# EavnJeong/IEF-VAD

Hardware: AMD Instinct MI355X
Metric: snippets/sec at [B,T=256,d=768] (higher is better)
Workload: dtype f32 emulated: exact 3-term bf16 split of both fp32 operands, 6 bf16 MFMA products, fp32 accumulate

## Files before the change

### ief-vad_amd/csrc/iefvad.hip

```cpp
#include "../../include/iefvad.h"

#include <hip/hip_runtime.h>
#include <math.h>
#include <stdarg.h>
#include <stdio.h>
#include <stdlib.h>
#include <string.h>

#include <algorithm>
#include <exception>
#include <new>
#include <thread>
#include <vector>

#include "attention_f32.h"
#include "attention_bf16.h"
#include "attention_pbf16.h"
#include "attention_split.h"
#include "common.h"
#include "gather.h"
#include "gemm_f32.h"
#include "gemm_bf16.h"
#include "gemm_split.h"
#include "rowops.h"
#include "refine_chain_bf16.h"
#include "outproj_ln_chain_bf16.h"
#include "outproj_ln_pchain_bf16.h"
#include "inproj_chain_bf16.h"
#include "heads_chain_bf16.h"
#include "heads_pchain_bf16.h"
#include "ragged.h"
#include "resample.h"
#include "loss.h"
#include "gemm_split_tn.h"
#include "backward.h"
#include "metrics.h"
#include "similarity.h"

static thread_local char g_err[512] = "";

static int fail(const char* fmt, ...) {
    va_list ap;
    va_start(ap, fmt);
    vsnprintf(g_err, sizeof(g_err), fmt, ap);
    va_end(ap);
    return 1;
}

#define HIP_TRY(expr)                                                                            \
    do {                                                                                         \
        hipError_t e_ = (expr);                                                                  \
        if (e_ != hipSuccess) return fail("%s failed: %s (%s:%d)", #expr, hipGetErrorString(e_), \
                                          __FILE__, __LINE__);                                   \
    } while (0)

struct ProjW {
    int N;
    float* w;
    float* b;
    bf16_t* wb;
    bf16_t* ws;
    _Float16* wh;
    const float* wa;
    bf16_t* wst;
};

struct iefvad_handle {
    iefvad_config cfg;
    int D, DH;
    int device;
    bool weights_set;
    bool no_heads_fusion, no_ln_fusion;
    char* iproj_stream[2][IEFVAD_MAX_LAYERS];
    char* heads_stream;
    int chain_min_blocks;
    int rowblock_min_wgs;
    bool no_inproj_chain;
    char* oproj_stream[2][IEFVAD_MAX_LAYERS];
    bool dense_encoder;
    bool persist;
    bool train_attn_unfused;
    bool hostpipe_trace;
    bool no_chain;
    char* chain_stream;
    float* arena;
    size_t arena_floats;
    ProjW in[2][IEFVAD_MAX_LAYERS], out[2][IEFVAD_MAX_LAYERS], head[2], ref1[IEFVAD_MAX_STEPS], ref2[IEFVAD_MAX_STEPS];
    float* norm_w[2][IEFVAD_MAX_LAYERS];
    float* norm_b[2][IEFVAD_MAX_LAYERS];
    float* whiten_w[2];
    float* whiten_b[2];
    float* cls_w;
    float* cls_b;
    float* score_fold;
    bf16_t* arena_b;
    bf16_t* arena_s;
    _Float16* arena_h;
    float* amax_dev;
    struct EventPool* events;
    struct GraphCache* graphs;
    struct MetaRing* meta;
    int num_cus;
    bf16_t* arena_st; float* zero_bias; bool tplanes_valid;
    struct HostPipe* hostpipe;
    struct TrainState* train;
    const float* row_scale[2];
};
static const int kAmaxActBase = 256;
static int amax_act_tensors(int L, int K) { return 2 + 6 * L + 2 * K + 1; }
static size_t amax_words(int L, int K, int mb_chunks) {
    return (size_t)kAmaxActBase * IEF_AMAX_FLOATS + (size_t)amax_act_tensors(L, K) * mb_chunks * IEF_AMAX_PARTS;
}

static const int kDefaultMicroBatchF32 = 256;
static const int kDefaultMicroBatchBF16 = 1024;

static int micro_batch(const iefvad_handle* h) {
    if (h->cfg.micro_batch > 0) return h->cfg.micro_batch < 16384 ? h->cfg.micro_batch : 16384;
    return h->cfg.compute == IEFVAD_COMPUTE_F32 ? kDefaultMicroBatchF32 : kDefaultMicroBatchBF16;
}

template <typename F>
static int for_each_proj(iefvad_handle* h, F f) {
    for (int m = 0; m < 2; ++m) {
        for (int l = 0; l < h->cfg.num_layers; ++l) {
            if (int rc = f(h->in[m][l])) return rc;
            if (int rc = f(h->out[m][l])) return rc;
        }
        if (int rc = f(h->head[m])) return rc;
    }
    for (int k = 0; k < h->cfg.num_steps; ++k) {
        if (int rc = f(h->ref1[k])) return rc;
        if (int rc = f(h->ref2[k])) return rc;
    }
    return 0;
}
static size_t proj_elems(const iefvad_handle* h) {
    const size_t DD = (size_t)h->D * h->D;
    return 2 * (size_t)h->cfg.num_layers * (3 * DD + DD) + 2 * (2 * DD) + (size_t)h->cfg.num_steps * 2 * DD;
}

extern "C" int iefvad_abi_version(void) { return IEFVAD_ABI_VERSION; }

extern "C" const char* iefvad_last_error(void) { return g_err; }

#define IEF_D512 512

static int create_impl(const char* who, bool allow_512, const iefvad_config* cfg, iefvad_handle** out) {
    if (!cfg || !out) return fail("%s: null argument", who);
    *out = nullptr;
    if (cfg->abi_version != IEFVAD_ABI_VERSION)
        return fail("%s: abi_version %d, library is %d", who, cfg->abi_version, IEFVAD_ABI_VERSION);
    const bool d512 = allow_512 && cfg->embed_dim == IEF_D512;
    if (d512) {
        if (cfg->seq_len != IEF_T || cfg->num_heads != IEF_D512 / 64)
            return fail("%s: D=512 is built for T=256, H=8 (head dim 64) (got T=%d H=%d)", who, cfg->seq_len, cfg->num_heads);
        if (cfg->compute != IEFVAD_COMPUTE_F32)
            return fail("%s: D=512 runs in the f32 arithmetic only (compute = %d; bf16, bf16x6 and fp16x3 are built for D=768)", who,
                        cfg->compute);
    } else if (cfg->embed_dim != IEF_D || cfg->seq_len != IEF_T || cfg->num_heads != IEF_H) {
        if (allow_512)
            return fail("%s: kernels are built for D=768, T=256, H=8, or D=512, T=256, H=8 in the f32 arithmetic (got D=%d T=%d H=%d)", who,
                        cfg->embed_dim, cfg->seq_len, cfg->num_heads);
        return fail("iefvad_create: kernels are built for D=768, T=256, H=8 (got D=%d T=%d H=%d)",
                    cfg->embed_dim, cfg->seq_len, cfg->num_heads);
    }
    if (cfg->num_layers < 1 || cfg->num_layers > IEFVAD_MAX_LAYERS)
        return fail("%s: num_layers %d outside 1..%d", who, cfg->num_layers, IEFVAD_MAX_LAYERS);
    if (cfg->num_steps < 0 || cfg->num_steps > IEFVAD_MAX_STEPS)
        return fail("%s: num_steps %d outside 0..%d", who, cfg->num_steps, IEFVAD_MAX_STEPS);
    if (cfg->noise_model != IEFVAD_NOISE_GAUSSIAN && cfg->noise_model != IEFVAD_NOISE_STUDENT_T)
        return fail("Unsupported noise_model. Choose 'Gaussian' or 'StudentT'.");
    if (cfg->compute != IEFVAD_COMPUTE_F32 && cfg->compute != IEFVAD_COMPUTE_BF16 && cfg->compute != IEFVAD_COMPUTE_BF16X6 &&
        cfg->compute != IEFVAD_COMPUTE_FP16X3)
        return fail("%s: unknown compute mode %d", who, cfg->compute);
    if (cfg->noise_model == IEFVAD_NOISE_STUDENT_T && !(cfg->nu != 0.f))
        return fail("%s: nu must be non-zero for StudentT", who);
    int ndev = 0;
    HIP_TRY(hipGetDeviceCount(&ndev));
    if (ndev <= 0) return fail("%s: no HIP device", who);
    iefvad_handle* h = new (std::nothrow) iefvad_handle();
    if (!h) return fail("%s: out of host memory", who);
    memset(h, 0, sizeof(*h));
    h->cfg = *cfg;
    h->D = d512 ? IEF_D512 : IEF_D;
    h->DH = h->D / IEF_H;
    {
        const char* v = getenv("IEFVAD_ROWBLOCK_OFF");
        const int off = v ? atoi(v) : 0;
        h->no_inproj_chain = off & 1; h->no_ln_fusion = off & 2; h->no_heads_fusion = off & 4; h->no_chain = off & 8;
    }
    { const char* v = getenv("IEFVAD_ROWBLOCK_MIN_WGS"); h->rowblock_min_wgs = (v && atoi(v) > 0) ? atoi(v) : 128; }
    { const char* v = getenv("IEFVAD_CHAIN_MIN_BLOCKS"); h->chain_min_blocks = (v && atoi(v) > 0) ? atoi(v) : 4; }
    { const char* v = getenv("IEFVAD_PERSIST"); h->persist = !(v && v[0] == '0'); }
    { const char* v = getenv("IEFVAD_DENSE_ENCODER"); h->dense_encoder = v && v[0] == '1'; }
    { const char* v = getenv("IEFVAD_TRAIN_ATTN"); h->train_attn_unfused = v && v[0] == 'u'; }
    { const char* v = getenv("IEFVAD_HOSTPIPE_TRACE"); h->hostpipe_trace = v && v[0] == '1'; }
    hipError_t e = hipGetDevice(&h->device);
    if (e == hipSuccess)
        e = hipFuncSetAttribute((const void*)iefvad_gemm_bf16_kernel, hipFuncAttributeMaxDynamicSharedMemorySize,
                                GB2_LDS_BYTES);
    if (e == hipSuccess)
        e = hipFuncSetAttribute((const void*)iefvad_gemm_bf16_pipe_kernel, hipFuncAttributeMaxDynamicSharedMemorySize,
                                GB2_LDS_BYTES);
    if (e == hipSuccess)
        e = hipFuncSetAttribute((const void*)iefvad_gemm_bf16_w256_kernel, hipFuncAttributeMaxDynamicSharedMemorySize,
                                GB3_LDS_BYTES);
    if (e == hipSuccess)
        e = hipFuncSetAttribute((const void*)iefvad_refine_chain_bf16_kernel, hipFuncAttributeMaxDynamicSharedMemorySize,
                                RC_LDS_BYTES);
    if (e == hipSuccess)
        e = hipFuncSetAttribute((const void*)iefvad_outproj_ln_chain_bf16_kernel, hipFuncAttributeMaxDynamicSharedMemorySize,
                                OC_LDS_BYTES);
    if (e == hipSuccess)
        e = hipFuncSetAttribute((const void*)iefvad_outproj_ln_pchain_bf16_kernel<true, true>, hipFuncAttributeMaxDynamicSharedMemorySize,
                                OP_LDS_BYTES);
    if (e == hipSuccess)
        e = hipFuncSetAttribute((const void*)iefvad_outproj_ln_pchain_bf16_kernel<true, false>, hipFuncAttributeMaxDynamicSharedMemorySize,
                                OP_LDS_BYTES);
    if (e == hipSuccess)
        e = hipFuncSetAttribute((const void*)iefvad_outproj_ln_pchain_bf16_kernel<false, true>, hipFuncAttributeMaxDynamicSharedMemorySize,
                                OP_LDS_BYTES);
    if (e == hipSuccess)
        e = hipFuncSetAttribute((const void*)iefvad_heads_pchain_bf16_kernel, hipFuncAttributeMaxDynamicSharedMemorySize,
                                HP_LDS_BYTES);
    if (e == hipSuccess)
        e = hipFuncSetAttribute((const void*)iefvad_gemm_split_tn256_kernel, hipFuncAttributeMaxDynamicSharedMemorySize, TN_LDS_BYTES_OF(4));
    if (e == hipSuccess)
        e = hipFuncSetAttribute((const void*)iefvad_attention_pbf16_kernel, hipFuncAttributeMaxDynamicSharedMemorySize, APB_LDS_BYTES);
    if (e == hipSuccess)
        e = hipFuncSetAttribute((const void*)iefvad_attention_pbf16_rows_kernel, hipFuncAttributeMaxDynamicSharedMemorySize, APB_LDS_BYTES);
    if (e == hipSuccess) {
        hipDeviceProp_t prop;
        e = hipGetDeviceProperties(&prop, h->device);
        h->num_cus = e == hipSuccess ? prop.multiProcessorCount : 256;
        g_num_cus = h->num_cus;
    }
    if (e == hipSuccess)
        e = hipFuncSetAttribute((const void*)iefvad_gemm_f32_t256_kernel, hipFuncAttributeMaxDynamicSharedMemorySize,
                                GB2_LDS_BYTES);
    if (e == hipSuccess)
        e = hipFuncSetAttribute((const void*)iefvad_gemm_split_n128_kernel, hipFuncAttributeMaxDynamicSharedMemorySize,
                                GS_LDS_BYTES_OF(2));
    if (e == hipSuccess)
        e = hipFuncSetAttribute((const void*)iefvad_attention_split_kernel, hipFuncAttributeMaxDynamicSharedMemorySize,
                                ATS_LDS_BYTES);
    if (e == hipSuccess)
        e = hipFuncSetAttribute((const void*)iefvad_attention_split_rows_kernel, hipFuncAttributeMaxDynamicSharedMemorySize,
                                ATS_LDS_BYTES);
    if (e == hipSuccess)
        e = hipFuncSetAttribute((const void*)iefvad_attention_split_train_kernel, hipFuncAttributeMaxDynamicSharedMemorySize,
                                ATS_LDS_BYTES);
    if (e == hipSuccess)
        e = hipFuncSetAttribute((const void*)iefvad_attention_split_ds_kernel, hipFuncAttributeMaxDynamicSharedMemorySize,
                                ATS_LDS_BYTES);
    if (e == hipSuccess)
        e = hipFuncSetAttribute((const void*)iefvad_attention_split_train_mask_kernel, hipFuncAttributeMaxDynamicSharedMemorySize,
                                ATS_LDS_BYTES);
    if (e == hipSuccess)
        e = hipFuncSetAttribute((const void*)iefvad_heads_chain_bf16_kernel, hipFuncAttributeMaxDynamicSharedMemorySize,
                                HC_LDS_BYTES);
    if (e == hipSuccess)
        e = hipFuncSetAttribute((const void*)iefvad_inproj_chain_bf16_kernel, hipFuncAttributeMaxDynamicSharedMemorySize,
                                IC_LDS_BYTES);
    if (e == hipSuccess)
        e = hipFuncSetAttribute((const void*)iefvad_inproj_chain_f32in_kernel, hipFuncAttributeMaxDynamicSharedMemorySize,
                                IC_LDS_BYTES);
    if (e == hipSuccess)
        e = hipFuncSetAttribute((const void*)iefvad_attention_split_f16_kernel, hipFuncAttributeMaxDynamicSharedMemorySize,
                                ATS_LDS_BYTES);
    if (e == hipSuccess)
        e = hipFuncSetAttribute((const void*)iefvad_gemm_split_f16_n128_kernel, hipFuncAttributeMaxDynamicSharedMemorySize,
                                GS_LDS_BYTES_OF(2));
    if (e == hipSuccess && cfg->compute == IEFVAD_COMPUTE_FP16X3) e = hipMalloc((void**)&h->amax_dev, amax_words(cfg->num_layers, cfg->num_steps, micro_batch(h)) * sizeof(float));
    if (e != hipSuccess) {
        delete h;
        return fail("%s: %s", who, hipGetErrorString(e));
    }
    *out = h;
    return 0;
}

extern "C" int iefvad_create(const iefvad_config* cfg, iefvad_handle** out) { return create_impl("iefvad_create", false, cfg, out); }

extern "C" int iefvad_create_ex(const iefvad_config* cfg, iefvad_handle** out) { return create_impl("iefvad_create_ex", true, cfg, out); }

static void release_events(iefvad_handle* h);
static void release_graphs(iefvad_handle* h);
static void release_meta(iefvad_handle* h);
static void release_train(iefvad_handle* h);
static void release_hostpipe(iefvad_handle* h);

extern "C" void iefvad_destroy(iefvad_handle* h) {
    if (!h) return;
    if (h->arena) (void)hipFree(h->arena);
    if (h->arena_b) (void)hipFree(h->arena_b);
    if (h->chain_stream) (void)hipFree(h->chain_stream);
    if (h->heads_stream) (void)hipFree(h->heads_stream);
    for (int m = 0; m < 2; ++m)
        for (int l = 0; l < IEFVAD_MAX_LAYERS; ++l) {
            if (h->oproj_stream[m][l]) (void)hipFree(h->oproj_stream[m][l]);
            if (h->iproj_stream[m][l]) (void)hipFree(h->iproj_stream[m][l]);
        }
    if (h->arena_s) (void)hipFree(h->arena_s);
    if (h->arena_st) (void)hipFree(h->arena_st);
    if (h->zero_bias) (void)hipFree(h->zero_bias);
    if (h->arena_h) (void)hipFree(h->arena_h);
    if (h->amax_dev) (void)hipFree(h->amax_dev);
    release_events(h);
    release_graphs(h);
    release_meta(h);
    release_train(h);
    release_hostpipe(h);
    delete h;
}

template <typename T> struct InType { using type = T; };
template <int W> struct RowWidth { static constexpr int value = W; };
template <typename F>
static void dispatch_d(bool d512, F&& f) {
    if (d512) f(RowWidth<IEF_D512>{});
    else f(RowWidth<IEF_D>{});
}
template <typename F>
static int dispatch_in(int in_dtype, bool d512, F&& f) {
    int rc = 0;
    dispatch_d(d512, [&](auto w) {
        rc = in_dtype == IEFVAD_IN_F32 ? f(InType<float>{}, w) : in_dtype == IEFVAD_IN_F16 ? f(InType<__half>{}, w) : f(InType<__hip_bfloat16>{}, w);
    });
    return rc;
}

template <typename T>
static int launch_cast(const void* in0, const void* in1, float* o0, float* o1, bf16_t* b0, bf16_t* b1, size_t n, int nsrc,
                       hipStream_t stream) {
    size_t blocks = (n / 4 + 255) / 256;
    if (blocks > 4096) blocks = 4096;
    hipLaunchKernelGGL(iefvad_cast_kernel<T>, dim3((unsigned)blocks, nsrc), dim3(256), 0, stream, (const T*)in0,
                       (const T*)in1, o0, o1, b0, b1, n);
    HIP_TRY(hipGetLastError());
    return 0;
}

template <typename T, int W>
static int launch_cast_scaled(const void* in0, const void* in1, float* o0, float* o1, bf16_t* b0, bf16_t* b1, size_t n, const float* s0,
                              const float* s1, hipStream_t stream) {
    size_t blocks = (n / 4 + 255) / 256;
    if (blocks > 4096) blocks = 4096;
    hipLaunchKernelGGL((iefvad_cast_scaled_kernel<T, W>), dim3((unsigned)blocks, 2), dim3(256), 0, stream, (const T*)in0, (const T*)in1, o0, o1, b0, b1,
                       n, s0, s1);
    HIP_TRY(hipGetLastError());
    return 0;
}

static int launch_split_planes(const float* src, bf16_t* planes, size_t n, hipStream_t stream) {
    if (n % 4) return fail("split_bf16x3: n = %zu is not a multiple of 4", n);
    size_t blocks = (n / 4 + 255) / 256;
    if (blocks > 4096) blocks = 4096;
    hipLaunchKernelGGL(iefvad_split_planes_kernel, dim3((unsigned)blocks), dim3(256), 0, stream, src, planes, n);
    HIP_TRY(hipGetLastError());
    return 0;
}

struct SplitMany {
    SplitManyArgs a;
    hipStream_t stream;
    explicit SplitMany(hipStream_t s) : stream(s) { a.count = 0; }
    int flush() {
        if (a.count == 0) return 0;
        hipLaunchKernelGGL(iefvad_split_planes_many_kernel, dim3(96, a.count), dim3(256), 0, stream, a);
        a.count = 0;
        HIP_TRY(hipGetLastError());
        return 0;
    }
    int add(const float* src, bf16_t* dst, size_t n, int rows) {
        if (n % 4 || n > 0xffffffffu) return fail("split_bf16x3: n = %zu is not a multiple of 4 below 2^32", n);
        if (rows && (rows % 64 || (n / rows) % 32 || n % rows)) return fail("split_bf16x3: transposed split of a [%d, %zu] matrix", rows, n / rows);
        a.src[a.count] = src; a.dst[a.count] = dst; a.n[a.count] = (unsigned)n; a.rows[a.count] = rows;
        if (++a.count == SPLIT_MANY_MAX) return flush();
        return 0;
    }
};

extern "C" int iefvad_split_bf16x3_many(const float* const* src, void* const* planes, const size_t* n, const int32_t* rows, int32_t count,
                                        void* stream) {
    if (!src || !planes || !n || !rows || count < 0) return fail("iefvad_split_bf16x3_many: null argument");
    SplitMany sm((hipStream_t)stream);
    for (int i = 0; i < count; ++i) {
        if (!src[i] || !planes[i] || rows[i] < 0) return fail("iefvad_split_bf16x3_many: entry %d is null or has negative rows", i);
        if (((uintptr_t)src[i] | (uintptr_t)planes[i]) & 15) return fail("iefvad_split_bf16x3_many: entry %d is not 16-byte aligned", i);
        if (int rc = sm.add(src[i], (bf16_t*)planes[i], n[i], rows[i])) return rc;
    }
    return sm.flush();
}

// ... 165 lines not shown
                q += 2 * n;
                float* word = h->amax_dev + IEF_AMAX_FLOATS * widx++;
                r.wa = word;
                size_t blocks = (n / 4 + 255) / 256;
                if (blocks > 1024) blocks = 1024;
                hipLaunchKernelGGL(iefvad_amax_kernel, dim3((unsigned)blocks, 1), dim3(256), 0, stream, r.w, r.w, word, word, n);
                hipLaunchKernelGGL(iefvad_split_planes_f16_kernel, dim3((unsigned)blocks), dim3(256), 0, stream, r.w, r.wh, n,
                                   (const float*)word);
                HIP_TRY(hipGetLastError());
                return 0;
            })) return rc;
    }
    h->weights_set = true;
    h->tplanes_valid = false;
    return 0;
}

static size_t ws_floats_per_row(const iefvad_handle* h) { return 14 * (size_t)h->D + 4; }

extern "C" size_t iefvad_workspace_bytes(const iefvad_handle* h, int32_t B) {
    if (!h || B <= 0) return 0;
    const int mb = micro_batch(h);
    const size_t rows = (size_t)(B < mb ? B : mb) * IEF_T;
    return rows * ws_floats_per_row(h) * sizeof(float) + 256;
}

enum Stage { ST_QKV = 0, ST_ATT, ST_OUT, ST_LN, ST_HEAD, ST_FUSION, ST_REFINE, ST_SCORER, ST_CAST, ST_COUNT };

struct EventPool {
    std::vector<hipEvent_t> ev;
    size_t used = 0;
    hipError_t err = hipSuccess;
    hipEvent_t take() {
        if (used == ev.size()) {
            hipEvent_t e = nullptr;
            hipError_t r = hipEventCreate(&e);
            if (r != hipSuccess) {
                if (err == hipSuccess) err = r;
                return nullptr;
            }
            ev.push_back(e);
        }
        return ev[used++];
    }
    void release_all() {
        for (hipEvent_t e : ev) (void)hipEventDestroy(e);
        ev.clear();
        used = 0;
    }
};

struct Timer {
    bool on = false;
    hipStream_t stream = nullptr;
    EventPool* pool = nullptr;
    struct Span { int stage; hipEvent_t a, b; };
    std::vector<Span> spans;
    int gemm_launches = 0;
    hipEvent_t begin(int stage) {
        if (!on) return nullptr;
        Span s;
        s.stage = stage;
        s.a = pool->take();
        s.b = pool->take();
        if (!s.a || !s.b) return nullptr;
        (void)hipEventRecord(s.a, stream);
        spans.push_back(s);
        return s.b;
    }
    void end(hipEvent_t b) {
        if (on && b) (void)hipEventRecord(b, stream);
    }
};

static void release_events(iefvad_handle* h) {
    if (h->events) {
        h->events->release_all();
        delete h->events;
        h->events = nullptr;
    }
}

static const int kF32TinyMaxBlocks64 = 320;
static const int kF32T256MinBlocks = 1536;
static const int kF32SmallMaxBlocks128 = 1024;

static int launch_gemm(const GemmArgs& a, int nz, hipStream_t stream, Timer& tm, int stage) {
    if (a.M % GEMM_BM || a.N % GEMM_BN || a.K % GEMM_BK)
        return fail("gemm: shape M=%d N=%d K=%d not a multiple of the %dx%dx%d tile", a.M, a.N, a.K, GEMM_BM, GEMM_BN,
                    GEMM_BK);
    const int blocks128 = (a.M / GEMM_BM) * (a.N / GEMM_BN) * nz;
    const int blocks64 = (a.M / GEMS_BM) * (a.N / GEMS_BN) * nz;
    const bool t256_ok = (a.N % GB2_BN == 0) && (a.K % 16 == 0) && (a.K >= 32);
    const int blocks256 = t256_ok ? (a.M / GB2_BM) * (a.N / GB2_BN) * nz : 0;
    const bool tiny = blocks64 < kF32TinyMaxBlocks64 && a.K % 64 == 0;
    hipEvent_t e = tm.begin(stage);
    if (tiny) {
        dim3 grid((a.M / GEMT_BM) * (a.N / GEMT_BN), 1, nz);
        hipLaunchKernelGGL(iefvad_gemm_f32_tiny_kernel, grid, dim3(256), 0, stream, a);
    } else if (blocks256 >= kF32T256MinBlocks) {
        GemmBArgs b;
        memset(&b, 0, sizeof(b));
        b.M = a.M; b.N = a.N; b.K = a.K; b.lda = a.lda; b.ldc = a.ldc; b.epi = a.epi; b.alpha = a.alpha; b.qcols = a.qcols;
        for (int m = 0; m < nz; ++m) {
            b.p[m].A = (const bf16_t*)a.p[m].A; b.p[m].W = (const bf16_t*)a.p[m].W;
            b.p[m].bias = a.p[m].bias; b.p[m].C = a.p[m].C; b.p[m].R = a.p[m].R; b.p[m].C2 = a.p[m].C2;
        }
        dim3 grid((a.M / GB2_BM) * (a.N / GB2_BN), 1, nz);
        hipLaunchKernelGGL(iefvad_gemm_f32_t256_kernel, grid, dim3(256), GB2_LDS_BYTES, stream, b);
    } else if (blocks128 < kF32SmallMaxBlocks128) {
        dim3 grid((a.M / GEMS_BM) * (a.N / GEMS_BN), 1, nz);
        hipLaunchKernelGGL(iefvad_gemm_f32_small_kernel, grid, dim3(256), 0, stream, a);
    } else {
        dim3 grid((a.M / GEMM_BM) * (a.N / GEMM_BN), 1, nz);
        hipLaunchKernelGGL(iefvad_gemm_f32_kernel, grid, dim3(256), 0, stream, a);
    }
    tm.end(e);
    tm.gemm_launches += 1;
    HIP_TRY(hipGetLastError());
    return 0;
}

static int launch_gemm_b(const GemmBArgs& a, int nz, hipStream_t stream, Timer& tm, int stage) {
    hipEvent_t e;
    if (a.N % GB2_BN == 0 && a.M % GB2_BM == 0 && a.K % GB2_BK == 0 && a.K >= 2 * GB2_BK) {
        e = tm.begin(stage);
        if (a.M % GB3_BM == 0 && a.epi != EPI_REFINE && (a.M / GB3_BM) * (a.N / GB2_BN) * nz >= 256) {
            dim3 grid((a.M / GB3_BM) * (a.N / GB2_BN), 1, nz);
            hipLaunchKernelGGL(iefvad_gemm_bf16_w256_kernel, grid, dim3(512), GB3_LDS_BYTES, stream, a);
        } else {
            dim3 grid((a.M / GB2_BM) * (a.N / GB2_BN), 1, nz);
            hipLaunchKernelGGL(iefvad_gemm_bf16_pipe_kernel, grid, dim3(256), GB2_LDS_BYTES, stream, a);
        }
    } else {
        if (a.M % GEMM_BM || a.N % GEMM_BN || a.K % GEMMB_BK)
            return fail("gemm(bf16): shape M=%d N=%d K=%d not a multiple of the %dx%dx%d tile", a.M, a.N, a.K, GEMM_BM,
                        GEMM_BN, GEMMB_BK);
        dim3 grid((a.M / GEMM_BM) * (a.N / GEMM_BN), 1, nz);
        e = tm.begin(stage);
        hipLaunchKernelGGL(iefvad_gemm_bf16_v1_kernel, grid, dim3(256), 0, stream, a);
    }
    tm.end(e);
    tm.gemm_launches += 1;
    HIP_TRY(hipGetLastError());
    return 0;
}

static const int kSplitBN = GS_BN_OF(2);
static const int kSplitMinWgs = 72;
static bool split_eligible(int M, int N, int K, int nz) {
    return M % GS_BM == 0 && N % kSplitBN == 0 && K % 64 == 0 && K >= 64 && (M / GS_BM) * (N / kSplitBN) * nz >= kSplitMinWgs;
}

static int launch_gemm_split(const GemmBArgs& a, int nz, hipStream_t stream, Timer& tm, int stage, bool f16 = false) {
    if (a.M % GS_BM || a.N % kSplitBN || a.K % 64 || a.K < 64)
        return fail("gemm(bf16x6): shape M=%d N=%d K=%d not a multiple of the %dx%dx64 tile", a.M, a.N, a.K, GS_BM, kSplitBN);
    if (a.epi == EPI_BIAS_RELU_DOT && (f16 || nz != 1 || !a.p[0].R || !a.p[0].C2))
        return fail("gemm(bf16x6): the dot-product epilogue takes one bf16x6 problem with its vector (R) and its partial sums (C2)");
    dim3 grid((a.M / GS_BM) * (a.N / kSplitBN), 1, nz);
    hipEvent_t e = tm.begin(stage);
    if (f16) hipLaunchKernelGGL(iefvad_gemm_split_f16_n128_kernel, grid, dim3(256), GS_LDS_BYTES_OF(2), stream, a);
    else hipLaunchKernelGGL(iefvad_gemm_split_n128_kernel, grid, dim3(256), GS_LDS_BYTES_OF(2), stream, a);
    tm.end(e);
    tm.gemm_launches += 1;
    HIP_TRY(hipGetLastError());
    return 0;
}

static size_t in_elem_bytes(int in_dtype) { return in_dtype == IEFVAD_IN_F32 ? 4 : 2; }

struct Proj {
    const float* A32[2];
    const bf16_t* A16[2];
    const float* W32[2];
    const bf16_t* W16[2];
    const bf16_t* Ws[2];
    const _Float16* Wh[2];
    const float* amaxW[2];
    const float* amaxA[2];
    float* amaxC[2];
    const float* bias[2];
    float* C[2];
    bf16_t* Cb[2];
    const float* R[2];
    float* C2[2];
    int N, ldc, epi, nz;
    float alpha;
    int qcols;
    void set_w(int m, const ProjW& r) {
        W32[m] = r.w; W16[m] = r.wb; Ws[m] = r.ws; Wh[m] = r.wh; amaxW[m] = r.wa; bias[m] = r.b;
    }
};

static int launch_proj(const Proj& p, int compute, bool use_split, int D, int rows, hipStream_t stream, Timer& tm, int stage) {
    const bool bf16 = (compute == IEFVAD_COMPUTE_BF16);
    if (p.epi == EPI_BIAS_RELU_DOT && !(use_split && compute == IEFVAD_COMPUTE_BF16X6))
        return fail("gemm: the dot-product epilogue exists in the bf16x6 split kernel only");
    if (use_split) {
        const bool f16 = (compute == IEFVAD_COMPUTE_FP16X3);
        GemmBArgs g;
        memset(&g, 0, sizeof(g));
        g.M = rows; g.N = p.N; g.K = IEF_D; g.lda = IEF_D; g.ldc = p.ldc; g.epi = p.epi; g.alpha = p.alpha; g.qcols = p.qcols;
        g.wplane = p.N * IEF_D * 2;
        for (int m = 0; m < p.nz; ++m) {
            g.p[m].A = (const bf16_t*)p.A32[m];
            g.p[m].W = f16 ? (const bf16_t*)p.Wh[m] : p.Ws[m];
            g.p[m].bias = p.bias[m]; g.p[m].C = p.C[m]; g.p[m].R = p.R[m]; g.p[m].C2 = p.C2[m];
            if (f16) {
                if (!p.amaxA[m] || !p.amaxW[m]) return fail("gemm(fp16x3): missing running-max word");
                g.p[m].amaxA = p.amaxA[m]; g.p[m].amaxW = p.amaxW[m]; g.p[m].amaxC = p.amaxC[m];
            }
        }
        return launch_gemm_split(g, p.nz, stream, tm, stage, f16);
    }
    if (!bf16) {
        GemmArgs g;
        memset(&g, 0, sizeof(g));
        g.M = rows; g.N = p.N; g.K = D; g.lda = D; g.ldc = p.ldc; g.epi = p.epi; g.alpha = p.alpha; g.qcols = p.qcols;
        for (int m = 0; m < p.nz; ++m) {
            g.p[m].A = p.A32[m]; g.p[m].W = p.W32[m]; g.p[m].bias = p.bias[m]; g.p[m].C = p.C[m]; g.p[m].R = p.R[m];
            g.p[m].C2 = p.C2[m];
        }
        return launch_gemm(g, p.nz, stream, tm, stage);
    }
    GemmBArgs g;
    memset(&g, 0, sizeof(g));
    g.M = rows; g.N = p.N; g.K = IEF_D; g.lda = IEF_D; g.ldc = p.ldc; g.epi = p.epi; g.alpha = p.alpha; g.qcols = p.qcols;
    for (int m = 0; m < p.nz; ++m) {
        g.p[m].A = p.A16[m]; g.p[m].W = p.W16[m]; g.p[m].bias = p.bias[m]; g.p[m].C = p.C[m]; g.p[m].Cb = p.Cb[m];
        g.p[m].R = p.R[m]; g.p[m].C2 = p.C2[m];
    }
    return launch_gemm_b(g, p.nz, stream, tm, stage);
}

static int launch_inproj_chain(iefvad_handle* h, int l, const void* const A[2], bool a_fp32, bf16_t* const C[2], int rows, hipStream_t stream, Timer& tm) {
    InProjChainArgs ia;
    memset(&ia, 0, sizeof(ia));
    for (int m = 0; m < 2; ++m) {
        ia.p[m].A = A[m];
        ia.p[m].stream = h->iproj_stream[m][l]; ia.p[m].bias = h->in[m][l].b; ia.p[m].C = C[m];
    }
    ia.M = rows; ia.alpha = (1.0f / sqrtf((float)IEF_DH)) * 1.4426950408889634f; ia.wave_stride = (unsigned)wstream_wave_stride_bytes(IC_NPASS);
    hipEvent_t e = tm.begin(ST_QKV);
    if (a_fp32) hipLaunchKernelGGL(iefvad_inproj_chain_f32in_kernel, dim3(rows / IC_BM, 2), dim3(512), IC_LDS_BYTES, stream, ia);
    else hipLaunchKernelGGL(iefvad_inproj_chain_bf16_kernel, dim3(rows / IC_BM, 2), dim3(512), IC_LDS_BYTES, stream, ia);
    tm.end(e);
    tm.gemm_launches += 1;
    HIP_TRY(hipGetLastError());
    return 0;
}

static int launch_outproj_ln_chain(iefvad_handle* h, int l, bool whiten, const bf16_t* const A[2], const float* const R[2], float* const y[2],
                                   bf16_t* const yb[2], int rows, hipStream_t stream, Timer& tm) {
    OutLnChainArgs oa;
    memset(&oa, 0, sizeof(oa));
    for (int m = 0; m < 2; ++m) {
        OutLnChainProblem& q = oa.p[m];
        q.A = A[m]; q.stream = h->oproj_stream[m][l]; q.bias = h->out[m][l].b; q.R = R[m];
        q.g1 = h->norm_w[m][l]; q.b1 = h->norm_b[m][l];
        if (whiten) { q.g2 = h->whiten_w[m]; q.b2 = h->whiten_b[m]; }
        q.y = y[m];
        q.yb = yb[m];
    }
    oa.M = rows; oa.eps = 1e-5f; oa.wave_stride = (unsigned)wstream_wave_stride_bytes();
    const int gx = h->num_cus / 2;
    const int nblk = rows / OC_BM;
    hipEvent_t e = tm.begin(ST_OUT);
    if (h->persist && nblk >= 2 * gx && (y[0] != nullptr) == (y[1] != nullptr) && (yb[0] != nullptr) == (yb[1] != nullptr) && (y[0] || yb[0])) {
        if (y[0] && yb[0]) hipLaunchKernelGGL((iefvad_outproj_ln_pchain_bf16_kernel<true, true>), dim3(gx, 2), dim3(512), OP_LDS_BYTES, stream, oa);
        else if (y[0]) hipLaunchKernelGGL((iefvad_outproj_ln_pchain_bf16_kernel<true, false>), dim3(gx, 2), dim3(512), OP_LDS_BYTES, stream, oa);
        else hipLaunchKernelGGL((iefvad_outproj_ln_pchain_bf16_kernel<false, true>), dim3(gx, 2), dim3(512), OP_LDS_BYTES, stream, oa);
    } else
        hipLaunchKernelGGL(iefvad_outproj_ln_chain_bf16_kernel, dim3(rows / OC_BM, 2), dim3(512), OC_LDS_BYTES, stream, oa);
    tm.end(e);
    tm.gemm_launches += 1;
    HIP_TRY(hipGetLastError());
    return 0;
}

static void launch_attention_bf16(iefvad_handle* h, const bf16_t* const qkv[2], bf16_t* const out[2], int nb, const RaggedChunk* chunks,
                                  bool head_major, int rows, hipStream_t stream) {
    AttnBArgs ab;
    for (int m = 0; m < 2; ++m) { ab.qkv[m] = qkv[m]; ab.out[m] = out[m]; }
    ab.nchunks = nb;
    ab.chunks = chunks;
    ab.head_major = head_major ? 1 : 0;
    ab.nrows = rows;
    const int items = 2 * nb * IEF_H;
    if (h->persist && items >= 2 * h->num_cus) {
        if (chunks) hipLaunchKernelGGL(iefvad_attention_pbf16_rows_kernel, dim3(h->num_cus), dim3(512), APB_LDS_BYTES, stream, ab);
        else hipLaunchKernelGGL(iefvad_attention_pbf16_kernel, dim3(h->num_cus), dim3(512), APB_LDS_BYTES, stream, ab);
    } else if (chunks) hipLaunchKernelGGL(iefvad_attention_bf16_rows_kernel, dim3(IEF_H, 2, 2 * nb), dim3(256), 0, stream, ab);
    else hipLaunchKernelGGL(iefvad_attention_bf16_kernel, dim3(IEF_H, 2, 2 * nb), dim3(256), 0, stream, ab);
}

static int launch_heads_chain(iefvad_handle* h, HeadsChainArgs& ha, int rows, float factor, hipStream_t stream, Timer& tm) {
    for (int m = 0; m < 2; ++m) ha.bias[m] = h->head[m].b;
    ha.stream = h->heads_stream;
    ha.M = rows; ha.factor = factor; ha.eps = h->cfg.epsilon; ha.wave_stride = (unsigned)heads_stream_wave_stride_bytes();
    const int gx = h->num_cus / HC_THIRDS;
    hipEvent_t e = tm.begin(ST_HEAD);
    if (h->persist && rows / HC_BM >= 2 * gx)
        hipLaunchKernelGGL(iefvad_heads_pchain_bf16_kernel, dim3(gx, HC_THIRDS), dim3(512), HP_LDS_BYTES, stream, ha);
    else
        hipLaunchKernelGGL(iefvad_heads_chain_bf16_kernel, dim3(rows / HC_BM, HC_THIRDS), dim3(512), HC_LDS_BYTES, stream, ha);
    tm.end(e);
    tm.gemm_launches += 1;
    HIP_TRY(hipGetLastError());
    return 0;
}

static int launch_refine_chain(iefvad_handle* h, const float* z_in, float* z_out, float* logits, int rows, hipStream_t stream, Timer& tm) {
    const int K = h->cfg.num_steps;
    ChainArgs ca;
    memset(&ca, 0, sizeof(ca));
    ca.z_in = z_in; ca.stream = h->chain_stream; ca.cls_w = h->cls_w; ca.cls_b = h->cls_b;
    ca.z_out = z_out;
    ca.logits = logits;
    ca.M = rows; ca.K = K; ca.lambda = h->cfg.lambda_ref; ca.wave_stride = (unsigned)chain_wave_stride_bytes(K);
    hipEvent_t e = tm.begin(ST_REFINE);
    hipLaunchKernelGGL(iefvad_refine_chain_bf16_kernel, dim3(rows / RC_BM), dim3(64 * RC_NW), RC_LDS_BYTES, stream, ca);
    tm.end(e);
    tm.gemm_launches += 1;
    HIP_TRY(hipGetLastError());
    return 0;
}

struct RaggedPass {
    const void* img_rows;
    const void* ev_rows;
    const RaggedChunk* d_chunks;
    const int* d_flags;
    int valid_rows;
    int enc_used_rows;
    int enc_rows;
    float* logits;
    float* w_i_mean;
    float* w_e_mean;
};

struct PassBuffers {
    int nb, rows;
    size_t R;
    bool enc_rows_mode;
    bool ip_chain;
    bool need_xb0;
    bool splitmb, f16mb;
    bool compacted, tail_split;
    float *xin[2], *qkv[2], *att[2], *ybuf[2], *xbuf[2];
    bf16_t *qkvb[2], *attb[2], *xb[2];
    float* lg_scratch;
    float *mu_i, *lv_i, *mu_e, *lv_e, *z, *hbuf, *n_i, *n_e, *logits, *wim_out, *wem_out;
    bf16_t *hb, *zb;
    const float* cur[2];
    const float* xt[2];
    const bf16_t* xtb[2];
    float* am; size_t mbs; int L, K;
    float* am_t(int t) const { return f16mb ? am + mbs * t : nullptr; }
    float* am_in(int m) const { return am_t(m); }
    float* am_att(int l, int m) const { return am_t(2 + 6 * l + m); }
    float* am_x(int l, int m) const { return am_t(2 + 6 * l + 2 + m); }
    float* am_qkv(int l, int m) const { return am_t(2 + 6 * l + 4 + m); }
    float* am_z(int k) const { return am_t(2 + 6 * L + k); }
    float* am_h(int k) const { return am_t(2 + 6 * L + (K + 1) + k); }
};

static PassBuffers pass_buffers(const iefvad_handle* h, int nb, size_t row0, void* workspace, const iefvad_outputs* out, const RaggedPass* rg) {
    const iefvad_config& c = h->cfg;
    const size_t D = h->D, R = (size_t)nb * IEF_T;
    PassBuffers b;
    memset(&b, 0, sizeof(b));
    b.nb = nb; b.R = R;
    b.enc_rows_mode = rg && rg->enc_rows > 0;
    b.rows = b.enc_rows_mode ? rg->enc_rows : nb * IEF_T;
    float* ws = (float*)workspace;
    float* t0 = ws + 2 * R * D;
    for (int m = 0; m < 2; ++m) {
        b.xin[m] = ws + m * R * D;
        b.qkv[m] = t0 + 3 * m * R * D;
        b.qkvb[m] = (bf16_t*)t0 + 3 * m * R * D;
        b.att[m] = ws + (8 + m) * R * D;
        b.attb[m] = (bf16_t*)(ws + 8 * R * D) + m * R * D;
        b.xb[m] = (bf16_t*)(ws + 9 * R * D) + m * R * D;
        b.ybuf[m] = ws + (10 + m) * R * D;
        b.xbuf[m] = ws + (12 + m) * R * D;
        b.xt[m] = b.xbuf[m];
        b.xtb[m] = b.xb[m];
    }
    b.lg_scratch = ws + 14 * R * D;
    b.mu_i = out->image_mu ? out->image_mu + row0 * D : t0;
    b.lv_i = out->image_logvar ? out->image_logvar + row0 * D : t0 + R * D;
    b.mu_e = out->event_mu ? out->event_mu + row0 * D : t0 + 2 * R * D;
    b.lv_e = out->event_logvar ? out->event_logvar + row0 * D : t0 + 3 * R * D;
    b.z = out->fused ? out->fused + row0 * D : t0 + 4 * R * D;
    b.hbuf = t0 + 5 * R * D;
    b.hb = (bf16_t*)b.hbuf; b.zb = b.hb + R * D;
    b.n_i = out->w_i ? out->w_i + row0 * D : nullptr;
    b.n_e = out->w_e ? out->w_e + row0 * D : nullptr;
    b.logits = out->logits ? out->logits + row0 : b.lg_scratch;
    b.wim_out = out->w_i_mean ? out->w_i_mean + row0 : nullptr;
    b.wem_out = out->w_e_mean ? out->w_e_mean + row0 : nullptr;
    if (rg) {
        b.logits = b.lg_scratch;
        b.wim_out = rg->w_i_mean ? b.lg_scratch + R : nullptr;
        b.wem_out = rg->w_e_mean ? b.lg_scratch + 2 * R : nullptr;
    }
    b.ip_chain = c.compute == IEFVAD_COMPUTE_BF16 && !h->no_inproj_chain && b.rows % IC_BM == 0 && (b.rows / IC_BM) * 2 >= h->rowblock_min_wgs;
    b.need_xb0 = c.compute == IEFVAD_COMPUTE_BF16 && !b.ip_chain;
    b.splitmb = (c.compute == IEFVAD_COMPUTE_BF16X6 || c.compute == IEFVAD_COMPUTE_FP16X3) && split_eligible(b.rows, IEF_D, IEF_D, 1);
    b.f16mb = b.splitmb && c.compute == IEFVAD_COMPUTE_FP16X3;
    b.am = h->amax_dev ? h->amax_dev + kAmaxActBase * IEF_AMAX_FLOATS : nullptr;
    b.mbs = (size_t)micro_batch(h) * IEF_AMAX_PARTS;
    b.L = c.num_layers; b.K = c.num_steps;
    return b;
}

static int pass_load_inputs(iefvad_handle* h, PassBuffers& b, const void* pi, const void* pe, int32_t in_dtype, size_t row0, const RaggedPass* rg,
                            hipStream_t stream, Timer& tm) {
    const size_t D = h->D, n = b.R * D;
    const bool d512 = h->D == IEF_D512;
    bf16_t* const b0p = b.need_xb0 ? b.xb[0] : nullptr;
    bf16_t* const b1p = b.need_xb0 ? b.xb[1] : nullptr;
    b.cur[0] = b.xin[0]; b.cur[1] = b.xin[1];
    if (rg) {
        if (b.enc_rows_mode && rg->enc_used_rows < b.rows) {
            const size_t o = (size_t)rg->enc_used_rows * D, nz = (size_t)(b.rows - rg->enc_used_rows) * D;
            for (int m = 0; m < 2; ++m) {
                HIP_TRY(hipMemsetAsync(b.xin[m] + o, 0, nz * sizeof(float), stream));
                if (b.need_xb0) HIP_TRY(hipMemsetAsync(b.xb[m] + o, 0, nz * sizeof(bf16_t), stream));
            }
        }
        hipEvent_t e = tm.begin(ST_CAST);
        dispatch_in(in_dtype, d512, [&](auto t, auto w) {
            using T = typename decltype(t)::type;
            hipLaunchKernelGGL((iefvad_scatter_rows_kernel<T, decltype(w)::value>), dim3(b.nb, 2, IEF_RAGGED_SLICES), dim3(256), 0, stream,
                               (const T*)rg->img_rows, (const T*)rg->ev_rows, rg->d_chunks, rg->d_flags, b.xin[0], b.xin[1], b0p, b1p,
                               b.enc_rows_mode ? 0 : IEF_T);
            return 0;
        });
        tm.end(e);
        HIP_TRY(hipGetLastError());
    } else if (h->row_scale[0] || h->row_scale[1]) {
        hipEvent_t e = tm.begin(ST_CAST);
        const float* s0 = h->row_scale[0] ? h->row_scale[0] + row0 : nullptr;
        const float* s1 = h->row_scale[1] ? h->row_scale[1] + row0 : nullptr;
        const int rc = dispatch_in(in_dtype, d512, [&](auto t, auto w) {
            return launch_cast_scaled<typename decltype(t)::type, decltype(w)::value>(pi, pe, b.xin[0], b.xin[1], b0p, b1p, n, s0, s1, stream);
        });
        tm.end(e);
        if (rc) return rc;
    } else if (in_dtype == IEFVAD_IN_F32) {
        b.cur[0] = (const float*)pi; b.cur[1] = (const float*)pe;
        if (b.need_xb0) {
            hipEvent_t e = tm.begin(ST_CAST);
            const int rc = launch_cast<float>(pi, pe, nullptr, nullptr, b.xb[0], b.xb[1], n, 2, stream);
            tm.end(e);
            if (rc) return rc;
        }
    } else {
        hipEvent_t e = tm.begin(ST_CAST);
        const int rc = dispatch_in(in_dtype, d512, [&](auto t, auto) {
            return launch_cast<typename decltype(t)::type>(pi, pe, b.xin[0], b.xin[1], b0p, b1p, n, 2, stream);
        });
        tm.end(e);
        if (rc) return rc;
    }
    if (b.f16mb) {
        HIP_TRY(hipMemsetAsync(b.am, 0, (size_t)amax_act_tensors(b.L, b.K) * b.mbs * sizeof(float), stream));
        hipEvent_t e = tm.begin(ST_CAST);
        hipLaunchKernelGGL(iefvad_amax_chunk_kernel, dim3(b.nb, 2), dim3(256), 0, stream, b.cur[0], b.cur[1], b.am_in(0), b.am_in(1));
        tm.end(e);
        HIP_TRY(hipGetLastError());
    }
    return 0;
}

static int pass_encoder_layer(iefvad_handle* h, PassBuffers& b, int l, const RaggedPass* rg, hipStream_t stream, Timer& tm) {
    const iefvad_config& c = h->cfg;
    const bool bf = (c.compute == IEFVAD_COMPUTE_BF16);
    const int D = h->D, L = c.num_layers, rows = b.rows, nb = b.nb;
    const bool d512 = h->D == IEF_D512;
    const RaggedChunk* enc_chunks = b.enc_rows_mode ? rg->d_chunks : nullptr;
    Proj p;
    if (b.ip_chain) {
        const void* ipA[2] = {(l == 0) ? (const void*)b.cur[0] : (const void*)b.xb[0], (l == 0) ? (const void*)b.cur[1] : (const void*)b.xb[1]};
        if (int rc = launch_inproj_chain(h, l, ipA, l == 0, b.qkvb, rows, stream, tm)) return rc;
    } else {
        memset(&p, 0, sizeof(p));
        p.N = 3 * D; p.ldc = 3 * D; p.epi = EPI_QKV; p.qcols = D; p.nz = 2;
        p.alpha = 1.0f / sqrtf((float)h->DH) * 1.4426950408889634f;
        for (int m = 0; m < 2; ++m) {
            p.set_w(m, h->in[m][l]);
            p.A32[m] = b.cur[m]; p.A16[m] = b.xb[m]; p.amaxA[m] = l == 0 ? b.am_in(m) : b.am_x(l - 1, m);
            p.amaxC[m] = b.am_qkv(l, m);
            if (bf) p.Cb[m] = b.qkvb[m]; else p.C[m] = b.qkv[m];
        }
        if (int rc = launch_proj(p, c.compute, b.splitmb, D, rows, stream, tm, ST_QKV)) return rc;
    }

    hipEvent_t e = tm.begin(ST_ATT);
    if (bf) {
        launch_attention_bf16(h, b.qkvb, b.attb, nb, enc_chunks, b.ip_chain, rows, stream);
    } else {
        AttnArgs aa;
        memset(&aa, 0, sizeof(aa));
        for (int m = 0; m < 2; ++m) { aa.qkv[m] = b.qkv[m]; aa.out[m] = b.att[m]; }
        aa.nchunks = nb;
        aa.chunks = enc_chunks;
        for (int m = 0; m < 2; ++m) { aa.amax[m] = b.am_att(l, m); aa.amax_in[m] = b.am_qkv(l, m); }
        void (*const kernel)(AttnArgs) = b.f16mb    ? iefvad_attention_split_f16_kernel
                                         : b.splitmb ? (enc_chunks ? iefvad_attention_split_rows_kernel : iefvad_attention_split_kernel)
                                         : d512      ? (enc_chunks ? iefvad_attention_f32_rows_d64_kernel : iefvad_attention_f32_d64_kernel)
                                                     : (enc_chunks ? iefvad_attention_f32_rows_kernel : iefvad_attention_f32_kernel);
        hipLaunchKernelGGL(kernel, dim3(IEF_H, 2, 2 * nb), dim3(256), b.splitmb ? ATS_LDS_BYTES : 0, stream, aa);
    }
    tm.end(e);
    HIP_TRY(hipGetLastError());

    const bool ln_fused = bf && !h->no_ln_fusion && rows % OC_BM == 0 && (rows / OC_BM) * 2 >= h->rowblock_min_wgs;
    if (ln_fused) {
        float* oy[2] = {(l < L - 1) ? b.xbuf[0] : nullptr, (l < L - 1) ? b.xbuf[1] : nullptr};
        if (int rc = launch_outproj_ln_chain(h, l, l == L - 1, b.attb, b.cur, oy, b.xb, rows, stream, tm)) return rc;
    } else {
        memset(&p, 0, sizeof(p));
        p.N = D; p.ldc = D; p.epi = EPI_BIAS_RESID; p.nz = 2;
        for (int m = 0; m < 2; ++m) {
            p.set_w(m, h->out[m][l]);
            p.A32[m] = b.att[m]; p.A16[m] = b.attb[m]; p.amaxA[m] = b.am_att(l, m);
            p.C[m] = b.ybuf[m]; p.R[m] = b.cur[m];
        }
        if (int rc = launch_proj(p, c.compute, b.splitmb, D, rows, stream, tm, ST_OUT)) return rc;

        LnArgs la;
        memset(&la, 0, sizeof(la));
        la.nrows = rows; la.eps = 1e-5f;
        for (int m = 0; m < 2; ++m) {
            la.x[m] = b.ybuf[m]; la.g1[m] = h->norm_w[m][l]; la.b1[m] = h->norm_b[m][l];
            if (l == L - 1) { la.g2[m] = h->whiten_w[m]; la.b2[m] = h->whiten_b[m]; }
            la.y[m] = (!bf || l < L - 1) ? b.xbuf[m] : nullptr;
            la.yb[m] = bf ? b.xb[m] : nullptr;
            la.amax[m] = b.am_x(l, m);
        }
        e = tm.begin(ST_LN);
        dispatch_d(d512, [&](auto w) {
            hipLaunchKernelGGL(iefvad_layernorm_kernel<decltype(w)::value>, dim3((rows + ROW_WAVES - 1) / ROW_WAVES, 2), dim3(256), 0, stream, la);
        });
        tm.end(e);
        HIP_TRY(hipGetLastError());
    }
    b.cur[0] = b.xbuf[0]; b.cur[1] = b.xbuf[1];
    return 0;
}

static int pass_compact_rows(iefvad_handle* h, PassBuffers& b, const RaggedPass* rg, hipStream_t stream, Timer& tm) {
    const bool bf = (h->cfg.compute == IEFVAD_COMPUTE_BF16);
    const size_t D = h->D;
    if (rg && !b.enc_rows_mode && h->cfg.compute != IEFVAD_COMPUTE_FP16X3) {
        const int mc = (rg->valid_rows + 255) / 256 * 256;
        if (mc < b.rows) {
            CompactArgs ca;
            memset(&ca, 0, sizeof(ca));
            for (int m = 0; m < 2; ++m) {
                if (bf) { ca.xb[m] = b.xb[m]; ca.xcb[m] = b.attb[m]; b.xtb[m] = b.attb[m]; }
                else { ca.x[m] = b.xbuf[m]; ca.xc[m] = b.att[m]; b.xt[m] = b.att[m]; }
            }
            ca.chunks = rg->d_chunks;
            const size_t tail0 = (size_t)rg->valid_rows * D, tailn = (size_t)(mc - rg->valid_rows) * D;
            if (tailn)
                for (int m = 0; m < 2; ++m)
                    HIP_TRY(bf ? hipMemsetAsync(b.attb[m] + tail0, 0, tailn * sizeof(bf16_t), stream)
                               : hipMemsetAsync(b.att[m] + tail0, 0, tailn * sizeof(float), stream));
            hipEvent_t e = tm.begin(ST_CAST);
            dispatch_d(h->D == IEF_D512, [&](auto w) {
                hipLaunchKernelGGL(iefvad_compact_rows_kernel<decltype(w)::value>, dim3(b.nb, 2), dim3(256), 0, stream, ca);
            });
            tm.end(e);
            HIP_TRY(hipGetLastError());
            b.rows = mc;
            b.compacted = true;
        }
    }
    b.tail_split = b.splitmb && (!b.compacted || split_eligible(b.rows, IEF_D, IEF_D, 1));
    return 0;
}

static int pass_tail(iefvad_handle* h, PassBuffers& b, const iefvad_outputs* out, const RaggedPass* rg, hipStream_t stream, Timer& tm) {
    const iefvad_config& c = h->cfg;
    const bool bf = (c.compute == IEFVAD_COMPUTE_BF16);
    const int D = h->D, L = c.num_layers, K = c.num_steps, rows = b.rows;
    const bool d512 = h->D == IEF_D512;
    const float factor = (c.noise_model == IEFVAD_NOISE_STUDENT_T) ? (c.nu + 1.0f) / c.nu : 1.0f;
    const dim3 row_grid((rows + ROW_WAVES - 1) / ROW_WAVES);
    float* const z = b.z;

    const bool heads_rows = bf && !h->no_heads_fusion && h->heads_stream && rows % HC_BM == 0 && (rows / HC_BM) * HC_THIRDS >= h->rowblock_min_wgs;
    const bool chain = bf && K > 0 && !h->no_chain && h->chain_stream && rows % RC_BM == 0 && rows / RC_BM >= h->chain_min_blocks;
    if (heads_rows) {
        HeadsChainArgs ha;
        memset(&ha, 0, sizeof(ha));
        for (int m = 0; m < 2; ++m) ha.A[m] = b.xtb[m];
        ha.mu[0] = out->image_mu ? b.mu_i : nullptr; ha.lv[0] = out->image_logvar ? b.lv_i : nullptr;
        ha.mu[1] = out->event_mu ? b.mu_e : nullptr; ha.lv[1] = out->event_logvar ? b.lv_e : nullptr;
        ha.n[0] = b.n_i; ha.n[1] = b.n_e;
        ha.z = z;
        ha.zb = chain ? nullptr : b.zb;
        const bool means = b.wim_out || b.wem_out;
        ha.nsum_part = means ? b.ybuf[0] : nullptr;
        if (int rc = launch_heads_chain(h, ha, rows, factor, stream, tm)) return rc;
        if (means) {
            hipEvent_t e = tm.begin(ST_FUSION);
            hipLaunchKernelGGL(iefvad_rowmean_finish_kernel, dim3((2 * rows + 255) / 256), dim3(256), 0, stream, ha.nsum_part,
                               b.wim_out, b.wem_out, rows, HC_NPART);
            tm.end(e);
            HIP_TRY(hipGetLastError());
        }
    } else {
        Proj p;
        memset(&p, 0, sizeof(p));
        p.N = 2 * D; p.ldc = D; p.epi = EPI_HEADS; p.nz = 2;
        for (int m = 0; m < 2; ++m) {
            p.set_w(m, h->head[m]);
            p.A32[m] = b.xt[m]; p.A16[m] = b.xtb[m]; p.amaxA[m] = b.am_x(L - 1, m);
        }
        p.C[0] = b.mu_i; p.C2[0] = b.lv_i; p.C[1] = b.mu_e; p.C2[1] = b.lv_e;
        if (int rc = launch_proj(p, c.compute, b.tail_split, D, rows, stream, tm, ST_HEAD)) return rc;

        FusionArgs fa;
        memset(&fa, 0, sizeof(fa));
        fa.mu_i = b.mu_i; fa.lv_i = b.lv_i; fa.mu_e = b.mu_e; fa.lv_e = b.lv_e;
        fa.n_i = b.n_i; fa.n_e = b.n_e; fa.n_i_mean = b.wim_out; fa.n_e_mean = b.wem_out;
        fa.z = z;
        fa.zb = (bf && !chain) ? b.zb : nullptr;
        fa.nrows = rows; fa.factor = factor; fa.eps = c.epsilon;
        fa.z_amax = b.am_z(0);
        hipEvent_t e = tm.begin(ST_FUSION);
        dispatch_d(d512, [&](auto w) { hipLaunchKernelGGL(iefvad_fusion_kernel<decltype(w)::value>, row_grid, dim3(256), 0, stream, fa); });
        tm.end(e);
        HIP_TRY(hipGetLastError());
    }

    if (chain)
        if (int rc = launch_refine_chain(h, z, out->fused ? z : nullptr, b.logits, rows, stream, tm)) return rc;

    const bool fold = b.tail_split && c.compute == IEFVAD_COMPUTE_BF16X6 && K >= 1;
    float* const fold_part = b.ybuf[0];

    for (int k = 0; k < K && !chain; ++k) {
        const bool dot = fold && k == K - 1;
        Proj p;
        memset(&p, 0, sizeof(p));
        p.N = D; p.ldc = D; p.epi = EPI_BIAS_RELU; p.nz = 1;
        p.set_w(0, h->ref1[k]);
        p.A32[0] = z; p.A16[0] = b.zb; p.amaxA[0] = b.am_z(k); p.amaxC[0] = b.am_h(k);
        p.C[0] = bf ? nullptr : b.hbuf; p.Cb[0] = bf ? b.hb : nullptr;
        if (dot) {
            p.epi = EPI_BIAS_RELU_DOT; p.R[0] = h->score_fold; p.C2[0] = fold_part;
            if (!out->fused) p.C[0] = nullptr;
        }
        if (int rc = launch_proj(p, c.compute, b.tail_split, D, rows, stream, tm, ST_REFINE)) return rc;
        if (dot) {
            hipEvent_t e = tm.begin(ST_SCORER);
            hipLaunchKernelGGL((iefvad_scorer_fold_kernel<IEF_D, IEF_D / kSplitBN>), row_grid, dim3(256), 0, stream, z, h->cls_w, fold_part,
                               h->score_fold, b.logits, rows);
            tm.end(e);
            HIP_TRY(hipGetLastError());
            if (!out->fused) break;
        }
        memset(&p, 0, sizeof(p));
        p.N = D; p.ldc = D; p.epi = EPI_REFINE; p.alpha = c.lambda_ref; p.nz = 1;
        p.set_w(0, h->ref2[k]);
        p.A32[0] = b.hbuf; p.A16[0] = b.hb; p.amaxA[0] = b.am_h(k); p.amaxC[0] = b.am_z(k + 1);
        p.C[0] = z; p.R[0] = z; p.Cb[0] = (bf && k + 1 < K) ? b.zb : nullptr;
        if (int rc = launch_proj(p, c.compute, b.tail_split, D, rows, stream, tm, ST_REFINE)) return rc;
    }

    if (!chain && !fold) {
        hipEvent_t e = tm.begin(ST_SCORER);
        dispatch_d(d512, [&](auto w) {
            hipLaunchKernelGGL(iefvad_scorer_kernel<decltype(w)::value>, row_grid, dim3(256), 0, stream, z, h->cls_w, h->cls_b, b.logits, rows);
        });
        tm.end(e);
        HIP_TRY(hipGetLastError());
    }

    if (rg) {
        hipEvent_t e = tm.begin(ST_SCORER);
        hipLaunchKernelGGL(iefvad_rows_out_kernel, dim3(b.compacted ? (rg->valid_rows + 255) / 256 : b.nb), dim3(256), 0, stream, b.logits, b.wim_out,
                           b.wem_out, rg->logits, rg->w_i_mean, rg->w_e_mean, b.compacted ? nullptr : rg->d_chunks, rg->valid_rows);
        tm.end(e);
        HIP_TRY(hipGetLastError());
    }
    return 0;
}

static int forward_pass(iefvad_handle* h, const void* pi, const void* pe, int32_t in_dtype, int nb, size_t row0, void* workspace,
                        const iefvad_outputs* out, const RaggedPass* rg, hipStream_t stream, Timer& tm) {
    PassBuffers b = pass_buffers(h, nb, row0, workspace, out, rg);
    if (int rc = pass_load_inputs(h, b, pi, pe, in_dtype, row0, rg, stream, tm)) return rc;
    for (int l = 0; l < h->cfg.num_layers; ++l)
        if (int rc = pass_encoder_layer(h, b, l, rg, stream, tm)) return rc;
    if (int rc = pass_compact_rows(h, b, rg, stream, tm)) return rc;
    return pass_tail(h, b, out, rg, stream, tm);
}

static int forward_impl(iefvad_handle* h, const void* img, const void* ev, int32_t in_dtype, int32_t B, void* workspace,
                        size_t workspace_bytes, const iefvad_outputs* out, hipStream_t stream, Timer& tm) {
    if (!h || !img || !ev || !out) return fail("iefvad_forward: null argument");
    if (!h->weights_set) return fail("iefvad_forward: weights not set");
    if (B <= 0) return fail("iefvad_forward: B must be positive (got %d)", B);
    if (in_dtype != IEFVAD_IN_F32 && in_dtype != IEFVAD_IN_F16 && in_dtype != IEFVAD_IN_BF16)
        return fail("iefvad_forward: unknown in_dtype %d", in_dtype);
    if (!workspace || workspace_bytes < iefvad_workspace_bytes(h, B))
        return fail("iefvad_forward: workspace too small (%zu < %zu bytes)", workspace_bytes, iefvad_workspace_bytes(h, B));
    if (((uintptr_t)workspace & 15) || ((uintptr_t)img & 15) || ((uintptr_t)ev & 15))
        return fail("iefvad_forward: buffers must be 16-byte aligned");
    const int mb = micro_batch(h);
    for (int b0 = 0; b0 < B; b0 += mb) {
        const int nb = (B - b0 < mb) ? (B - b0) : mb;
        const size_t row0 = (size_t)b0 * IEF_T;
        const size_t in_off = row0 * (size_t)h->D * in_elem_bytes(in_dtype);
        if (int rc = forward_pass(h, (const char*)img + in_off, (const char*)ev + in_off, in_dtype, nb, row0, workspace, out, nullptr,
                                  stream, tm))
            return rc;
    }
    return 0;
}

static int video_chunks(int n) { return n < IEF_T ? 1 : n / IEF_T + (n % IEF_T ? 1 : 0); }

struct MetaRing {
    static const int kSlots = 4;
    void* host[kSlots] = {nullptr, nullptr, nullptr, nullptr};
    void* dev[kSlots] = {nullptr, nullptr, nullptr, nullptr};
    size_t cap[kSlots] = {0, 0, 0, 0};
    hipEvent_t done[kSlots] = {nullptr, nullptr, nullptr, nullptr};
    int turn = 0;
};

static void release_meta(iefvad_handle* h) {
    if (!h->meta) return;
    for (int i = 0; i < MetaRing::kSlots; ++i) {
        if (h->meta->host[i]) (void)hipHostFree(h->meta->host[i]);
        if (h->meta->dev[i]) (void)hipFree(h->meta->dev[i]);
        if (h->meta->done[i]) (void)hipEventDestroy(h->meta->done[i]);
    }
    delete h->meta;
    h->meta = nullptr;
}

static int videos_layout(const int32_t* lengths, int32_t nvideos, long long* total_rows, long long* total_chunks) {
    long long rows = 0, chunks = 0;
    for (int v = 0; v < nvideos; ++v) {
        if (lengths[v] <= 0) return fail("iefvad_forward_videos: lengths[%d] = %d", v, lengths[v]);
        rows += lengths[v];
        chunks += video_chunks(lengths[v]);
    }
    *total_rows = rows;
    *total_chunks = chunks;
    return 0;
}

extern "C" size_t iefvad_videos_workspace_bytes(const iefvad_handle* h, const int32_t* lengths, int32_t nvideos) {
    if (!h || !lengths || nvideos <= 0) return 0;
    long long rows, chunks;
    if (videos_layout(lengths, nvideos, &rows, &chunks) || chunks > 0x7fffffffLL) return 0;
    return iefvad_workspace_bytes(h, (int32_t)chunks);
}

static int forward_videos_impl(iefvad_handle* h, const void* img_rows, const void* ev_rows, int32_t in_dtype, const int32_t* lengths,
                               int32_t nvideos, int32_t nan_to_num, void* workspace, size_t workspace_bytes, float* logits,
                               float* w_i_mean, float* w_e_mean, hipStream_t stream, Timer& tm) {
    if (!h || !img_rows || !ev_rows || !lengths || !logits) return fail("iefvad_forward_videos: null argument");
    if (!h->weights_set) return fail("iefvad_forward_videos: weights not set");
    if (nvideos <= 0) return fail("iefvad_forward_videos: nvideos must be positive (got %d)", nvideos);
    if (in_dtype != IEFVAD_IN_F32 && in_dtype != IEFVAD_IN_F16 && in_dtype != IEFVAD_IN_BF16)
        return fail("iefvad_forward_videos: unknown in_dtype %d", in_dtype);
    long long total_rows, total_chunks;
    if (int rc = videos_layout(lengths, nvideos, &total_rows, &total_chunks)) return rc;
    if (total_chunks > 0x7fffffffLL / IEF_T) return fail("iefvad_forward_videos: too many chunks");
    const size_t need = iefvad_workspace_bytes(h, (int32_t)total_chunks);
    if (!workspace || workspace_bytes < need) return fail("iefvad_forward_videos: workspace too small (%zu < %zu bytes)", workspace_bytes, need);
    if (((uintptr_t)workspace & 15) || ((uintptr_t)img_rows & 15) || ((uintptr_t)ev_rows & 15))
        return fail("iefvad_forward_videos: buffers must be 16-byte aligned");

    const size_t chunk_bytes = (size_t)total_chunks * sizeof(RaggedChunk);
    const size_t flag_off = (chunk_bytes + 255) & ~(size_t)255;
    const size_t flag_bytes = nan_to_num ? (size_t)nvideos * 2 * sizeof(int) : 0;
    const size_t meta_bytes = flag_off + flag_bytes;
    if (!h->meta) {
        h->meta = new (std::nothrow) MetaRing();
        if (!h->meta) return fail("iefvad_forward_videos: out of host memory");
    }
    MetaRing& mr = *h->meta;
    const int slot = mr.turn;
    mr.turn = (mr.turn + 1) % MetaRing::kSlots;
    HIP_TRY(hipSetDevice(h->device));
    if (mr.done[slot]) HIP_TRY(hipEventSynchronize(mr.done[slot]));
    else HIP_TRY(hipEventCreateWithFlags(&mr.done[slot], hipEventDisableTiming));
    if (mr.cap[slot] < meta_bytes) {
        if (mr.host[slot]) (void)hipHostFree(mr.host[slot]);
        if (mr.dev[slot]) (void)hipFree(mr.dev[slot]);
        mr.host[slot] = mr.dev[slot] = nullptr;
        mr.cap[slot] = 0;
        const size_t cap = meta_bytes * 2 + 4096;
        HIP_TRY(hipHostMalloc(&mr.host[slot], cap, hipHostMallocDefault));
        HIP_TRY(hipMalloc(&mr.dev[slot], cap));
        mr.cap[slot] = cap;
    }
    RaggedChunk* hc = (RaggedChunk*)mr.host[slot];
    const int mb = micro_batch(h);
    const bool enc_rows_mode = !h->dense_encoder && h->cfg.compute != IEFVAD_COMPUTE_FP16X3;
    {
        long long row = 0, pass_row0 = 0;
        long long ci = 0;
        int enc = 0;
        for (int v = 0; v < nvideos; ++v) {
            const int n = lengths[v], nch = video_chunks(n);
            for (int j = 0; j < nch; ++j, ++ci) {
                if (ci % mb == 0) { pass_row0 = row; enc = 0; }
                const int valid = (n - j * IEF_T) < IEF_T ? (n - j * IEF_T) : IEF_T;
                hc[ci].src_row = (int)(row - pass_row0);
                hc[ci].valid = valid;
                hc[ci].video = v;
                hc[ci].enc_row = enc;
                enc += enc_rows_mode ? ragged_rows(valid) : IEF_T;
                row += valid;
// ... 640 lines not shown
        table[v].out = v;
        row += lengths[v];
    }
    std::stable_sort(table.begin(), table.end(), [](const ResampleVideo& a, const ResampleVideo& b) { return a.n > b.n; });
    hipStream_t stream = (hipStream_t)stream_;
    HIP_TRY(hipMemcpyAsync(workspace, table.data(), (size_t)nvideos * sizeof(ResampleVideo), hipMemcpyHostToDevice, stream));
    HIP_TRY(hipStreamSynchronize(stream));
    const dim3 grid((unsigned)((long long)nvideos * groups));
    if (in_dtype == IEFVAD_IN_F32)
        hipLaunchKernelGGL(iefvad_resample_rows_kernel<float>, grid, dim3(256), 0, stream, (const float*)rows, (const ResampleVideo*)workspace, (int)D, out,
                           (int*)out_lengths);
    else
        hipLaunchKernelGGL(iefvad_resample_rows_kernel<__half>, grid, dim3(256), 0, stream, (const __half*)rows, (const ResampleVideo*)workspace, (int)D, out,
                           (int*)out_lengths);
    HIP_TRY(hipGetLastError());
    return 0;
}

extern "C" int iefvad_gather_windows(const float* img_set, const float* ev_set, const int32_t* set_lengths, int32_t nset, const int32_t* index,
                                     int32_t B, int32_t T, int32_t D, float* img_out, float* ev_out, int32_t* len_out, void* stream_) {
    if (!img_set || !ev_set || !set_lengths || !index || !img_out || !ev_out || !len_out) return fail("iefvad_gather_windows: null argument");
    if (nset <= 0 || B <= 0) return fail("iefvad_gather_windows: nset = %d, B = %d must be positive", nset, B);
    if (B > 65535) return fail("iefvad_gather_windows: B = %d exceeds one launch (65535 windows)", B);
    if (T != IEF_T) return fail("iefvad_gather_windows: T = %d, the window is %d segments", T, IEF_T);
    if (D <= 0 || D % 8) return fail("iefvad_gather_windows: D = %d must be a positive multiple of 8", D);
    if (((uintptr_t)img_set & 15) || ((uintptr_t)ev_set & 15) || ((uintptr_t)img_out & 15) || ((uintptr_t)ev_out & 15) ||
        ((uintptr_t)set_lengths & 3) || ((uintptr_t)index & 3) || ((uintptr_t)len_out & 3))
        return fail("iefvad_gather_windows: the window tensors must be 16-byte aligned, the int32 vectors 4-byte");
    const int nvec = IEF_T * D / 4, per_wg = 256 * IEF_GW_VEC;
    hipLaunchKernelGGL(iefvad_gather_windows_kernel, dim3((nvec + per_wg - 1) / per_wg, B, 2), dim3(256), 0, (hipStream_t)stream_, img_set, ev_set,
                       (const int*)set_lengths, (int)nset, (const int*)index, (int)D, img_out, ev_out, (int*)len_out);
    HIP_TRY(hipGetLastError());
    return 0;
}

extern "C" int iefvad_similarity_rows(const float* fused, const float* image_mu, const float* event_mu, int64_t rows, int32_t D,
                                      const int32_t* src_rows, int64_t nout, float* out, void* stream_) {
    if (!fused || !image_mu || !event_mu) return fail("iefvad_similarity_rows: null tensor (fused, image_mu, event_mu)");
    if (!out) return fail("iefvad_similarity_rows: null out");
    if (rows <= 0) return fail("iefvad_similarity_rows: rows = %lld must be positive", (long long)rows);
    if (nout < 0) return fail("iefvad_similarity_rows: nout = %lld is negative", (long long)nout);
    if (D != 768 && D != 512) return fail("iefvad_similarity_rows: D = %d (768 and 512 are built)", D);
    if (!src_rows && nout > rows) return fail("iefvad_similarity_rows: nout = %lld exceeds rows = %lld without src_rows", (long long)nout, (long long)rows);
    if (nout > 0x7fffffffLL) return fail("iefvad_similarity_rows: nout = %lld exceeds one launch (2^31 - 1 rows)", (long long)nout);
    if (((uintptr_t)fused & 15) || ((uintptr_t)image_mu & 15) || ((uintptr_t)event_mu & 15) || ((uintptr_t)out & 15) || ((uintptr_t)src_rows & 3))
        return fail("iefvad_similarity_rows: misaligned pointer (the tensors and out 16-byte, src_rows 4-byte)");
    if (nout == 0) return 0;
    const dim3 grid((unsigned)((nout + ROW_WAVES - 1) / ROW_WAVES));
    if (D == 768)
        hipLaunchKernelGGL(iefvad_similarity_rows_kernel<768>, grid, dim3(256), 0, (hipStream_t)stream_, fused, image_mu, event_mu, (long long)rows,
                           (const int*)src_rows, (long long)nout, out);
    else
        hipLaunchKernelGGL(iefvad_similarity_rows_kernel<512>, grid, dim3(256), 0, (hipStream_t)stream_, fused, image_mu, event_mu, (long long)rows,
                           (const int*)src_rows, (long long)nout, out);
    HIP_TRY(hipGetLastError());
    return 0;
}

#include "vadclip.h"
#include "hostgather.h"
#include "hostpipe.h"

extern "C" int iefvad_rowblock_unit(iefvad_handle* h, int32_t stage, int32_t layer, int32_t rows, const iefvad_unit_io* io, void* stream_) {
    if (!h || !io) return fail("iefvad_rowblock_unit: null argument");
    if (!h->weights_set) return fail("iefvad_rowblock_unit: weights not set");
    if (h->D != IEF_D) return fail("iefvad_rowblock_unit: the row-block kernels are built for D=768 (this handle has D=%d)", h->D);
    if (h->cfg.compute != IEFVAD_COMPUTE_BF16) return fail("iefvad_rowblock_unit: the row-block kernels belong to compute = BF16 (got %d)", h->cfg.compute);
    if (rows <= 0 || rows % 64) return fail("iefvad_rowblock_unit: rows = %d must be a positive multiple of 64", rows);
    if (stage == IEFVAD_UNIT_ATTENTION && rows % IEF_T) return fail("iefvad_rowblock_unit: ATTENTION runs whole chunks, rows = %d must be a multiple of %d", rows, IEF_T);
    hipStream_t stream = (hipStream_t)stream_;
    const int L = h->cfg.num_layers, K = h->cfg.num_steps;
    Timer tm;
    auto aligned = [](const void* p) { return (((uintptr_t)p) & 15) == 0; };
    switch (stage) {
    case IEFVAD_UNIT_INPROJ: {
        if (layer < 0 || layer >= L) return fail("iefvad_rowblock_unit: layer %d of %d", layer, L);
        if (!h->iproj_stream[0][layer]) return fail("iefvad_rowblock_unit: in_proj streams are not packed on this handle");
        const void* A[2] = {io->x[0], io->x[1]};
        bf16_t* C[2] = {(bf16_t*)io->y[0], (bf16_t*)io->y[1]};
        for (int m = 0; m < 2; ++m)
            if (!A[m] || !C[m] || !aligned(A[m]) || !aligned(C[m])) return fail("iefvad_rowblock_unit: INPROJ needs x[m] and y[m], 16-byte aligned");
        return launch_inproj_chain(h, layer, A, layer == 0, C, rows, stream, tm);
    }
    case IEFVAD_UNIT_OUTPROJ_LN: {
        if (layer < 0 || layer >= L) return fail("iefvad_rowblock_unit: layer %d of %d", layer, L);
        if (!h->oproj_stream[0][layer]) return fail("iefvad_rowblock_unit: out_proj streams are not packed on this handle");
        const bf16_t* A[2] = {(const bf16_t*)io->x[0], (const bf16_t*)io->x[1]};
        const float* R[2] = {io->resid[0], io->resid[1]};
        float* y[2] = {(float*)io->y[0], (float*)io->y[1]};
        bf16_t* yb[2] = {(bf16_t*)io->yb[0], (bf16_t*)io->yb[1]};
        for (int m = 0; m < 2; ++m)
            if (!A[m] || !R[m] || (!y[m] && !yb[m]) || !aligned(A[m]) || !aligned(R[m]) || !aligned(y[m]) || !aligned(yb[m]))
                return fail("iefvad_rowblock_unit: OUTPROJ_LN needs x[m], resid[m] and y[m] or yb[m], 16-byte aligned");
        return launch_outproj_ln_chain(h, layer, layer == L - 1, A, R, y, yb, rows, stream, tm);
    }
    case IEFVAD_UNIT_HEADS: {
        if (!h->heads_stream) return fail("iefvad_rowblock_unit: the heads stream is not packed on this handle");
        if (!io->x[0] || !io->x[1] || !io->z || !aligned(io->x[0]) || !aligned(io->x[1]) || !aligned(io->z))
            return fail("iefvad_rowblock_unit: HEADS needs x[0], x[1] and z, 16-byte aligned");
        HeadsChainArgs ha;
        memset(&ha, 0, sizeof(ha));
        for (int m = 0; m < 2; ++m) {
            ha.A[m] = (const bf16_t*)io->x[m];
            ha.mu[m] = io->mu[m]; ha.lv[m] = io->logvar[m]; ha.n[m] = io->w[m];
        }
        ha.z = io->z;
        const float factor = (h->cfg.noise_model == IEFVAD_NOISE_STUDENT_T) ? (h->cfg.nu + 1.0f) / h->cfg.nu : 1.0f;
        return launch_heads_chain(h, ha, rows, factor, stream, tm);
    }
    case IEFVAD_UNIT_REFINE: {
        if (K < 1 || !h->chain_stream) return fail("iefvad_rowblock_unit: the refinement chain needs K >= 1 (K = %d)", K);
        if (!io->x[0] || !io->logits || !aligned(io->x[0]) || !aligned(io->z)) return fail("iefvad_rowblock_unit: REFINE needs x[0] (z_0) and logits");
        return launch_refine_chain(h, (const float*)io->x[0], io->z, io->logits, rows, stream, tm);
    }
    case IEFVAD_UNIT_ATTENTION: {
        const bf16_t* qkv[2] = {(const bf16_t*)io->x[0], (const bf16_t*)io->x[1]};
        bf16_t* out[2] = {(bf16_t*)io->yb[0], (bf16_t*)io->yb[1]};
        for (int m = 0; m < 2; ++m)
            if (!qkv[m] || !out[m] || !aligned(qkv[m]) || !aligned(out[m])) return fail("iefvad_rowblock_unit: ATTENTION needs x[m] and yb[m], 16-byte aligned");
        launch_attention_bf16(h, qkv, out, rows / IEF_T, nullptr, true, rows, stream);
        HIP_TRY(hipGetLastError());
        return 0;
    }
    default:
        return fail("iefvad_rowblock_unit: unknown stage %d", stage);
    }
}

extern "C" int iefvad_gemm_bias(const void* A, const void* W, const float* bias, float* C, int32_t M, int32_t N, int32_t K,
                                int32_t compute, void* stream) {
    if (!A || !W || !bias || !C) return fail("iefvad_gemm_bias: null argument");
    Timer tm;
    if (compute == IEFVAD_COMPUTE_F32) {
        GemmArgs g;
        memset(&g, 0, sizeof(g));
        g.M = M; g.N = N; g.K = K; g.lda = K; g.ldc = N; g.epi = EPI_BIAS;
        g.p[0].A = (const float*)A; g.p[0].W = (const float*)W; g.p[0].bias = bias; g.p[0].C = C;
        return launch_gemm(g, 1, (hipStream_t)stream, tm, ST_QKV);
    }
    if (compute == IEFVAD_COMPUTE_BF16) {
        GemmBArgs g;
        memset(&g, 0, sizeof(g));
        g.M = M; g.N = N; g.K = K; g.lda = K; g.ldc = N; g.epi = EPI_BIAS;
        g.p[0].A = (const bf16_t*)A; g.p[0].W = (const bf16_t*)W; g.p[0].bias = bias; g.p[0].C = C;
        return launch_gemm_b(g, 1, (hipStream_t)stream, tm, ST_QKV);
    }
    if (compute == IEFVAD_COMPUTE_BF16X6) {
        GemmBArgs g;
        memset(&g, 0, sizeof(g));
        g.M = M; g.N = N; g.K = K; g.lda = K; g.ldc = N; g.epi = EPI_BIAS; g.wplane = N * K * 2;
        g.p[0].A = (const bf16_t*)A; g.p[0].W = (const bf16_t*)W; g.p[0].bias = bias; g.p[0].C = C;
        hipError_t e = hipFuncSetAttribute((const void*)iefvad_gemm_split_n128_kernel, hipFuncAttributeMaxDynamicSharedMemorySize,
                                           GS_LDS_BYTES_OF(2));
        if (e != hipSuccess) return fail("iefvad_gemm_bias: %s", hipGetErrorString(e));
        return launch_gemm_split(g, 1, (hipStream_t)stream, tm, ST_QKV);
    }
    return fail("iefvad_gemm_bias: unknown compute mode %d", compute);
}
```

### ief-vad_amd/csrc/train.h

```cpp
#pragma once

struct TrainLayout {
    size_t U;
    size_t PU;
    size_t x[2][IEFVAD_MAX_LAYERS + 1], qkv[2][IEFVAD_MAX_LAYERS], att[2][IEFVAD_MAX_LAYERS], s[2][IEFVAD_MAX_LAYERS];
    size_t P[2][IEFVAD_MAX_LAYERS];
    size_t E[2], mu[2], lv[2];
    size_t z[IEFVAD_MAX_STEPS + 1], hid[IEFVAD_MAX_STEPS];
    size_t logits;
    size_t g, da, dh[2], gx, datt, dqkv, dP, part, cpart, rpart;
    size_t part_floats, cpart_floats, rpart_floats;
    size_t total;
};

static const int kColsumRows = 128;

static int splitk_splits(int rows, int n_out) {
    const int tiles = (n_out / 128) * (IEF_D / 128);
    int want = (1024 + tiles - 1) / tiles, s = 1;
    while (s < want && s < 64) s <<= 1;
    while (s > 1 && ((rows / 16) % s)) s >>= 1;
    return s;
}

static bool train_attn_fused(const iefvad_handle* h) { return h->cfg.compute == IEFVAD_COMPUTE_BF16X6 && !h->train_attn_unfused; }

static TrainLayout train_layout(int L, int K, int B) {
    TrainLayout t;
    memset(&t, 0, sizeof(t));
    const size_t rows = (size_t)B * IEF_T;
    t.U = rows * IEF_D;
    t.PU = (size_t)B * IEF_H * IEF_T * IEF_T;
    size_t o = 0;
    auto take = [&](size_t n) { const size_t r = o; o += (n + 63) & ~(size_t)63; return r; };
    for (int m = 0; m < 2; ++m) {
        for (int l = 0; l <= L; ++l) t.x[m][l] = take(t.U);
        for (int l = 0; l < L; ++l) {
            t.qkv[m][l] = take(3 * t.U);
            t.att[m][l] = take(t.U);
            t.s[m][l] = take(t.U);
            t.P[m][l] = take(t.PU);
        }
        t.E[m] = take(t.U);
        t.mu[m] = take(t.U);
        t.lv[m] = take(t.U);
    }
    for (int k = 0; k <= K; ++k) t.z[k] = take(t.U);
    for (int k = 0; k < K; ++k) t.hid[k] = take(t.U);
    t.logits = take(rows);
    t.g = take(t.U);
    t.da = take(t.U);
    {
        size_t dead = t.z[0];
        const size_t dead_end = t.z[0] + (size_t)(2 * K + 1) * t.U;
        auto place = [&](size_t n) {
            const size_t n64 = (n + 63) & ~(size_t)63;
            if (dead + n64 <= dead_end) { const size_t r = dead; dead += n64; return r; }
            return take(n);
        };
        t.dqkv = place(3 * t.U);
        t.dP = place(t.PU);
        t.dh[0] = place(2 * t.U);
        t.dh[1] = place(2 * t.U);
        t.gx = place(t.U);
        t.datt = place(t.U);
    }
    size_t pf = 0;
    const int nouts[3] = {IEF_D, 2 * IEF_D, 3 * IEF_D};
    for (int n : nouts) {
        const size_t f = (size_t)splitk_splits((int)rows, n) * n * IEF_D;
        if (f > pf) pf = f;
    }
    t.part_floats = pf;
    t.part = take(pf);
    t.cpart_floats = ((rows + kColsumRows - 1) / kColsumRows) * 3 * IEF_D;
    t.cpart = take(t.cpart_floats);
    t.rpart_floats = ((rows + BWD_ROWS_PER_BLOCK - 1) / BWD_ROWS_PER_BLOCK) * (2 * IEF_D + 1);
    t.rpart = take(t.rpart_floats);
    t.total = o;
    return t;
}

extern "C" size_t iefvad_train_workspace_bytes(const iefvad_handle* h, int32_t B) {
    if (!h || B <= 0 || B > 4096) return 0;
    if (h->D != IEF_D) { fail("iefvad_train_workspace_bytes: training is built for D=768 (this handle has D=%d)", h->D); return 0; }
    return train_layout(h->cfg.num_layers, h->cfg.num_steps, B).total * sizeof(float) + 256;
}

static int launch_bgemm(const BgemmArgs& a, bool akc, bool bkc, int nz, hipStream_t stream) {
    const int bn = (a.N % 128 == 0) ? 128 : 96;
    if (a.M % BG_BM || a.N % bn || a.K % BG_BK || a.M <= 0 || a.N <= 0 || a.K <= 0 || nz <= 0 || a.nz2 <= 0)
        return fail("bgemm: shape M=%d N=%d K=%d is not a multiple of the 128 x %d x 16 tile", a.M, a.N, a.K, bn);
    if ((a.lda | a.ldb) & 3) return fail("bgemm: leading dimensions must be multiples of 4 floats");
    dim3 grid((unsigned)((a.M / BG_BM) * (a.N / bn) * nz));
#define BG_LAUNCH(AK, BK_, BN_) hipLaunchKernelGGL((iefvad_bgemm_f32_kernel<AK, BK_, BN_>), grid, dim3(256), 0, stream, a)
    if (bn == 128) {
        if (akc && bkc) BG_LAUNCH(true, true, 128);
        else if (akc) BG_LAUNCH(true, false, 128);
        else if (bkc) BG_LAUNCH(false, true, 128);
        else BG_LAUNCH(false, false, 128);
    } else {
        if (akc && bkc) BG_LAUNCH(true, true, 96);
        else if (akc) BG_LAUNCH(true, false, 96);
        else if (bkc) BG_LAUNCH(false, true, 96);
        else BG_LAUNCH(false, false, 96);
    }
#undef BG_LAUNCH
    HIP_TRY(hipGetLastError());
    return 0;
}

static int ensure_train_planes(iefvad_handle* h, hipStream_t stream) {
    if (h->cfg.compute != IEFVAD_COMPUTE_BF16X6 || h->tplanes_valid) return 0;
    if (!h->arena_st) HIP_TRY(hipMalloc((void**)&h->arena_st, 3 * proj_elems(h) * sizeof(bf16_t)));
    if (!h->zero_bias) {
        HIP_TRY(hipMalloc((void**)&h->zero_bias, 3 * IEF_D * sizeof(float)));
        HIP_TRY(hipMemsetAsync(h->zero_bias, 0, 3 * IEF_D * sizeof(float), stream));
    }
    bf16_t* q = h->arena_st;
    SplitMany sm(stream);
    if (int rc = for_each_proj(h, [&](ProjW& r) {
            const size_t n = (size_t)r.N * IEF_D;
            r.wst = q;
            q += 3 * n;
            return sm.add(r.w, r.wst, n, r.N);
        })) return rc;
    if (int rc = sm.flush()) return rc;
    h->tplanes_valid = true;
    return 0;
}

static int launch_dx(iefvad_handle* h, const bf16_t* planes_t, const float* dY, int ldy, const float* W, int n_out, int n_in, float* dX,
                     const float* R, const float* G, float alpha, int rows, hipStream_t stream) {
    if (planes_t && n_in == IEF_D && ldy == n_out && split_eligible(rows, IEF_D, n_out, 1) && (!R || !G) && (G || alpha == 1.f)) {
        GemmBArgs g;
        memset(&g, 0, sizeof(g));
        g.M = rows; g.N = IEF_D; g.K = n_out; g.lda = n_out; g.ldc = IEF_D; g.alpha = alpha;
        g.epi = G ? EPI_GATE : (R ? EPI_BIAS_RESID : EPI_BIAS);
        g.wplane = IEF_D * n_out * 2;
        g.p[0].A = (const bf16_t*)dY;
        g.p[0].W = planes_t; g.p[0].bias = h->zero_bias; g.p[0].C = dX; g.p[0].R = G ? G : R;
        Timer tm;
        return launch_gemm_split(g, 1, stream, tm, ST_REFINE);
    }
    BgemmArgs a;
    memset(&a, 0, sizeof(a));
    a.A = dY; a.B = W; a.C = dX; a.R = R; a.G = G;
    a.M = rows; a.N = n_in; a.K = n_out; a.lda = ldy; a.ldb = n_in; a.ldc = n_in; a.nz2 = 1; a.alpha = alpha;
    (void)h;
    return launch_bgemm(a, true, false, 1, stream);
}

struct ReduceBatch {
    ReduceJobs j;
    ReduceBatch() { memset(&j, 0, sizeof(j)); }
    void add(const float* part, size_t stride, int nparts, size_t n, float* out, float alpha) {
        if (!out || n == 0 || j.count == 4) return;
        const int c = j.count++;
        j.part[c] = part; j.stride[c] = stride; j.nparts[c] = nparts; j.n[c] = n; j.out[c] = out; j.alpha[c] = alpha;
        j.first[c + 1] = j.first[c] + (unsigned)((n + RED_STRIP - 1) / RED_STRIP);
    }
    void launch(hipStream_t stream) {
        if (j.count == 0) return;
        hipLaunchKernelGGL(iefvad_reduce_parts_multi_kernel, dim3(j.first[j.count]), dim3(256), 0, stream, j);
    }
};

static int launch_dw(const float* dY, int ldy, int n_out, const float* X, float* dW, float* dW2, int n_split, float alpha, int rows,
                     float* part, size_t part_floats, hipStream_t stream, bool split_tn = false, float* db = nullptr, float* db2 = nullptr,
                     float* cpart = nullptr, size_t cpart_floats = 0, bool* db_done = nullptr) {
    if (db_done) *db_done = false;
    if (!dW && !dW2) return 0;
    const int splits = splitk_splits(rows, n_out);
    const size_t per = (size_t)n_out * IEF_D;
    if ((size_t)splits * per > part_floats) return fail("train_backward: split-K scratch too small");
    const int ms = rows / splits;
    if (split_tn && ms % TN_BK == 0 && n_out % 128 == 0 && (ldy & 3) == 0) {
        TnArgs g;
        memset(&g, 0, sizeof(g));
        g.A = dY; g.B = X; g.C = part; g.M = n_out; g.N = IEF_D; g.lda = ldy; g.ldb = IEF_D; g.ldc = IEF_D;
        g.nk_total = rows / TN_BK;
        const int tiles = (n_out / 128) * (IEF_D / 256);
        int slices = (2 * g_num_cus) / tiles;
        if (slices > g.nk_total / 8) slices = g.nk_total / 8;
        if (slices > splits) slices = splits;
        if (slices < 1) slices = 1;
        g.slices = slices;
        g.tiles_n = IEF_D / 256;
        const bool with_db = (db || db2) && cpart && db_done && (size_t)slices * n_out <= cpart_floats;
        g.colsum = with_db ? cpart : nullptr;
        hipLaunchKernelGGL(iefvad_gemm_split_tn256_kernel, dim3((unsigned)((n_out / 128) * g.tiles_n * slices)), dim3(256), TN_LDS_BYTES_OF(4), stream, g);
        HIP_TRY(hipGetLastError());
        ReduceBatch rb;
        rb.add(part, per, slices, (size_t)(n_split > 0 ? n_split : n_out) * IEF_D, dW, alpha);
        if (dW2) rb.add(part + (size_t)n_split * IEF_D, per, slices, (size_t)(n_out - n_split) * IEF_D, dW2, alpha);
        if (with_db) {
            rb.add(cpart, (size_t)n_out, slices, (size_t)(n_split > 0 ? n_split : n_out), db, alpha);
            if (db2) rb.add(cpart + n_split, (size_t)n_out, slices, (size_t)(n_out - n_split), db2, alpha);
            *db_done = true;
        }
        rb.launch(stream);
        HIP_TRY(hipGetLastError());
        return 0;
    }
    BgemmArgs a;
    memset(&a, 0, sizeof(a));
    a.A = dY; a.B = X; a.C = part;
    a.M = n_out; a.N = IEF_D; a.K = ms; a.lda = ldy; a.ldb = IEF_D; a.ldc = IEF_D;
    a.a1 = (long long)ms * ldy; a.b1 = (long long)ms * IEF_D; a.c1 = (long long)per; a.nz2 = 1; a.alpha = 1.f;
    if (int rc = launch_bgemm(a, false, false, splits, stream)) return rc;
    if (dW) {
        const size_t n = (size_t)(n_split > 0 ? n_split : n_out) * IEF_D;
        hipLaunchKernelGGL(iefvad_reduce_parts_kernel, dim3((unsigned)((n + RED_STRIP - 1) / RED_STRIP)), dim3(256), 0, stream, part, per, splits, n, dW, alpha);
    }
    if (dW2) {
        const size_t n = (size_t)(n_out - n_split) * IEF_D;
        hipLaunchKernelGGL(iefvad_reduce_parts_kernel, dim3((unsigned)((n + RED_STRIP - 1) / RED_STRIP)), dim3(256), 0, stream, part + (size_t)n_split * IEF_D,
                           per, splits, n, dW2, alpha);
    }
    HIP_TRY(hipGetLastError());
    return 0;
}

static int launch_db(const float* Y, int ld, int ncols, float* db, float* db2, int n_split, float alpha, int rows, float* cpart,
                     hipStream_t stream) {
    if (!db && !db2) return 0;
    const int nblk = (rows + kColsumRows - 1) / kColsumRows;
    hipLaunchKernelGGL(iefvad_colsum_kernel, dim3((ncols + 255) / 256, nblk), dim3(256), 0, stream, Y, ld, rows, ncols, kColsumRows, cpart);
    if (db) {
        const size_t n = n_split > 0 ? n_split : ncols;
        hipLaunchKernelGGL(iefvad_reduce_parts_kernel, dim3((unsigned)((n + RED_STRIP - 1) / RED_STRIP)), dim3(256), 0, stream, cpart, (size_t)ncols, nblk, n, db, alpha);
    }
    if (db2) {
        const size_t n = ncols - n_split;
        hipLaunchKernelGGL(iefvad_reduce_parts_kernel, dim3((unsigned)((n + RED_STRIP - 1) / RED_STRIP)), dim3(256), 0, stream, cpart + n_split, (size_t)ncols, nblk,
                           n, db2, alpha);
    }
    HIP_TRY(hipGetLastError());
    return 0;
}

struct TrainRecord {
    const void* ws; int B; bool drop[2][IEFVAD_MAX_LAYERS]; float drop_p[2][IEFVAD_MAX_LAYERS]; bool fused; unsigned long long stamp;
    const float* x0[2]; float* mu[2]; float* lv[2]; float* zK;
};
struct TrainState { TrainRecord rec[8]; unsigned long long clock = 0; };

static void release_train(iefvad_handle* h) {
    delete h->train;
    h->train = nullptr;
}

static int train_check(const iefvad_handle* h, int32_t B, const void* ws, size_t ws_bytes, const char* who) {
    if (!h) return fail("%s: null handle", who);
    if (!h->weights_set) return fail("%s: weights not set", who);
    if (h->cfg.compute != IEFVAD_COMPUTE_F32 && h->cfg.compute != IEFVAD_COMPUTE_BF16X6)
        return fail("%s: training runs in the fp32-accurate arithmetics only (compute f32 or bf16x6)", who);
    if (B <= 0 || B > 4096) return fail("%s: B = %d outside 1..4096", who, B);
    const size_t need = iefvad_train_workspace_bytes(h, B);
    if (!ws || ws_bytes < need) return fail("%s: training buffer too small (%zu < %zu bytes)", who, ws_bytes, need);
    if ((uintptr_t)ws & 255) return fail("%s: the training buffer must be 256-byte aligned", who);
    return 0;
}

__global__ __launch_bounds__(256) void iefvad_nan_scan_kernel(const float* __restrict__ a, const float* __restrict__ b, size_t n4, unsigned* flags) {
    const float* x = blockIdx.y ? b : a;
    bool bad = false;
    for (size_t i = (size_t)blockIdx.x * 256 + threadIdx.x; i < n4; i += (size_t)gridDim.x * 256) {
        const f32x4 v = ((const f32x4*)x)[i];
        bad |= (v[0] != v[0]) | (v[1] != v[1]) | (v[2] != v[2]) | (v[3] != v[3]);
    }
    if (__any(bad) && (threadIdx.x & 63) == 0) flags[blockIdx.y] = 1u;
}
__global__ __launch_bounds__(256) void iefvad_nan_fix_kernel(float* a, float* b, size_t n4, const unsigned* flags) {
    if (!flags[blockIdx.y]) return;
    float* x = blockIdx.y ? b : a;
    for (size_t i = (size_t)blockIdx.x * 256 + threadIdx.x; i < n4; i += (size_t)gridDim.x * 256) {
        f32x4 v = ((f32x4*)x)[i];
#pragma unroll
        for (int e = 0; e < 4; ++e) {
            const float f = v[e];
            v[e] = f != f ? 0.f : f == __builtin_inff() ? 3.402823466e+38f : f == -__builtin_inff() ? -3.402823466e+38f : f;
        }
        ((f32x4*)x)[i] = v;
    }
}
extern "C" int iefvad_nan_rule(float* a, float* b, size_t n, void* flags_ws, void* stream_) {
    if (!a || !b || !flags_ws) return fail("iefvad_nan_rule: null argument");
    if (n % 4 || (((uintptr_t)a | (uintptr_t)b) & 15) || ((uintptr_t)flags_ws & 7)) return fail("iefvad_nan_rule: n %% 4 == 0 and 16-byte aligned tensors, please");
    hipStream_t stream = (hipStream_t)stream_;
    HIP_TRY(hipMemsetAsync(flags_ws, 0, 8, stream));
    hipLaunchKernelGGL(iefvad_nan_scan_kernel, dim3(2048, 2), dim3(256), 0, stream, a, b, n / 4, (unsigned*)flags_ws);
    hipLaunchKernelGGL(iefvad_nan_fix_kernel, dim3(2048, 2), dim3(256), 0, stream, a, b, n / 4, (const unsigned*)flags_ws);
    HIP_TRY(hipGetLastError());
    return 0;
}

extern "C" int iefvad_train_forward(iefvad_handle* h, const void* img, const void* ev, int32_t in_dtype, int32_t B,
                                    const iefvad_train_options* opt, void* train_ws, size_t train_ws_bytes, const iefvad_outputs* out,
                                    void* stream_) {
    if (!h) return fail("iefvad_train_forward: null handle");
    if (h->D != IEF_D) return fail("iefvad_train_forward: training is built for D=768 (this handle has D=%d)", h->D);
    const bool fused = train_attn_fused(h);
    if (int rc = train_check(h, B, train_ws, train_ws_bytes, "iefvad_train_forward")) return rc;
    if (!img || !ev || !out || !opt) return fail("iefvad_train_forward: null argument");
    if (in_dtype != IEFVAD_IN_F32 && in_dtype != IEFVAD_IN_F16 && in_dtype != IEFVAD_IN_BF16)
        return fail("iefvad_train_forward: unknown in_dtype %d", in_dtype);
    if (((uintptr_t)img | (uintptr_t)ev) & 15) return fail("iefvad_train_forward: buffers must be 16-byte aligned");
    if (((uintptr_t)out->fused | (uintptr_t)out->image_mu | (uintptr_t)out->event_mu | (uintptr_t)out->image_logvar | (uintptr_t)out->event_logvar) & 15)
        return fail("iefvad_train_forward: output buffers must be 16-byte aligned");
    const iefvad_config& c = h->cfg;
    const int L = c.num_layers, K = c.num_steps;
    for (int m = 0; m < 2; ++m)
        for (int l = 0; l < L; ++l)
            if (!(opt->dropout_p[m][l] >= 0.f && opt->dropout_p[m][l] < 1.f))
                return fail("iefvad_train_forward: dropout_p[%d][%d] = %g outside [0, 1)", m, l, (double)opt->dropout_p[m][l]);
    hipStream_t stream = (hipStream_t)stream_;
    const TrainLayout t = train_layout(L, K, B);
    float* ws = (float*)train_ws;
    const int rows = B * IEF_T;
    Timer tm;
    if (!h->train) {
        h->train = new (std::nothrow) TrainState();
        if (!h->train) return fail("iefvad_train_forward: out of host memory");
        memset(h->train->rec, 0, sizeof(h->train->rec));
    }
    TrainRecord* rec = nullptr;
    {
        TrainState& ts = *h->train;
        int slot = 0;
        for (int i = 0; i < 8; ++i) {
            if (ts.rec[i].ws == train_ws) { slot = i; break; }
            if (ts.rec[i].stamp < ts.rec[slot].stamp) slot = i;
        }
        TrainRecord& r = ts.rec[slot];
        rec = &r;
        r.ws = train_ws; r.B = B; r.fused = fused; r.stamp = ++ts.clock;
        const bool f32in = in_dtype == IEFVAD_IN_F32;
        r.x0[0] = f32in ? (const float*)img : ws + t.x[0][0];
        r.x0[1] = f32in ? (const float*)ev : ws + t.x[1][0];
        r.mu[0] = out->image_mu ? out->image_mu : ws + t.mu[0];
        r.mu[1] = out->event_mu ? out->event_mu : ws + t.mu[1];
        r.lv[0] = out->image_logvar ? out->image_logvar : ws + t.lv[0];
        r.lv[1] = out->event_logvar ? out->event_logvar : ws + t.lv[1];
        r.zK = out->fused ? out->fused : ws + t.z[K];
        for (int m = 0; m < 2; ++m)
            for (int l = 0; l < IEFVAD_MAX_LAYERS; ++l) {
                r.drop[m][l] = l < L && (opt->dropout_p[m][l] > 0.f || opt->keep_mask);
                r.drop_p[m][l] = l < L ? opt->dropout_p[m][l] : 0.f;
            }
    }
    const bool splitmb = c.compute == IEFVAD_COMPUTE_BF16X6 && split_eligible(rows, IEF_D, IEF_D, 1);
    const float qscale = 1.0f / sqrtf((float)IEF_DH);
    const float factor = (c.noise_model == IEFVAD_NOISE_STUDENT_T) ? (c.nu + 1.0f) / c.nu : 1.0f;

    auto xin = [&](int m, int l) -> const float* { return l == 0 ? rec->x0[m] : ws + t.x[m][l]; };
    auto zst = [&](int k) -> float* { return k == K ? rec->zK : ws + t.z[k]; };
    if (in_dtype != IEFVAD_IN_F32) {
        if (int rc = dispatch_in(in_dtype, false, [&](auto ty, auto) {
                return launch_cast<typename decltype(ty)::type>(img, ev, ws + t.x[0][0], ws + t.x[1][0], nullptr, nullptr, t.U, 2, stream);
            })) return rc;
    }

    for (int l = 0; l < L; ++l) {
        Proj p;
        memset(&p, 0, sizeof(p));
        p.N = 3 * IEF_D; p.ldc = 3 * IEF_D; p.epi = EPI_QKV; p.qcols = IEF_D; p.nz = 2;
        p.alpha = qscale;
        for (int m = 0; m < 2; ++m) {
            p.set_w(m, h->in[m][l]);
            p.A32[m] = xin(m, l); p.C[m] = ws + t.qkv[m][l];
        }
        if (int rc = launch_proj(p, c.compute, splitmb, IEF_D, rows, stream, tm, ST_QKV)) return rc;

        if (fused) {
            AttnArgs aa;
            AttnTrainArgs tx;
            memset(&aa, 0, sizeof(aa));
            memset(&tx, 0, sizeof(tx));
            aa.nchunks = B;
            for (int m = 0; m < 2; ++m) {
                const float pdrop = opt->dropout_p[m][l];
                const bool drop = pdrop > 0.f || opt->keep_mask;
                aa.qkv[m] = ws + t.qkv[m][l];
                aa.out[m] = ws + t.att[m][l];
                tx.P[m] = ws + t.P[m][l];
                tx.drop[m] = drop ? 1 : 0;
                tx.keep[m] = opt->keep_mask ? opt->keep_mask + ((size_t)m * L + l) * t.PU : nullptr;
                tx.seed[m] = opt->seed * 0x100000001B3ull + (unsigned long long)(m * IEFVAD_MAX_LAYERS + l + 1) * 0x9E3779B97F4A7C15ull;
                tx.drop_p[m] = pdrop;
            }
            if (opt->keep_mask)
                hipLaunchKernelGGL(iefvad_attention_split_train_mask_kernel, dim3(IEF_H, 2, 2 * B), dim3(256), ATS_LDS_BYTES, stream, aa, tx);
            else
                hipLaunchKernelGGL(iefvad_attention_split_train_kernel, dim3(IEF_H, 2, 2 * B), dim3(256), ATS_LDS_BYTES, stream, aa, tx);
            HIP_TRY(hipGetLastError());
        } else
        for (int m = 0; m < 2; ++m) {
            float* qkv = ws + t.qkv[m][l];
            const float pdrop = opt->dropout_p[m][l];
            const bool drop = pdrop > 0.f || opt->keep_mask;
            BgemmArgs a;
            memset(&a, 0, sizeof(a));
            a.A = qkv; a.B = qkv + IEF_D; a.C = ws + t.P[m][l];
            a.M = IEF_T; a.N = IEF_T; a.K = IEF_DH; a.lda = a.ldb = 3 * IEF_D; a.ldc = IEF_T;
            a.a1 = a.b1 = (long long)IEF_T * 3 * IEF_D; a.a2 = a.b2 = IEF_DH;
            a.c1 = (long long)IEF_H * IEF_T * IEF_T; a.c2 = (long long)IEF_T * IEF_T; a.nz2 = IEF_H; a.alpha = 1.f;
            if (int rc = launch_bgemm(a, true, true, B * IEF_H, stream)) return rc;
            SoftmaxDropArgs sa;
            sa.S = ws + t.P[m][l];
            sa.drop = drop ? 1 : 0;
            sa.keep = opt->keep_mask ? opt->keep_mask + ((size_t)m * L + l) * t.PU : nullptr;
            sa.seed = opt->seed * 0x100000001B3ull + (unsigned long long)(m * IEFVAD_MAX_LAYERS + l + 1) * 0x9E3779B97F4A7C15ull;
            sa.p = pdrop;
            sa.rows = (long long)B * IEF_H * IEF_T;
            hipLaunchKernelGGL(iefvad_softmax_dropout_kernel, dim3((unsigned)((sa.rows + 3) / 4)), dim3(256), 0, stream, sa);
            HIP_TRY(hipGetLastError());
            memset(&a, 0, sizeof(a));
            a.A = ws + t.P[m][l]; a.B = qkv + 2 * IEF_D; a.C = ws + t.att[m][l];
            if (drop) a.a_drop = (float)(1.0 / (1.0 - (double)pdrop));
            a.M = IEF_T; a.N = IEF_DH; a.K = IEF_T; a.lda = IEF_T; a.ldb = 3 * IEF_D; a.ldc = IEF_D;
            a.a1 = (long long)IEF_H * IEF_T * IEF_T; a.a2 = (long long)IEF_T * IEF_T;
            a.b1 = (long long)IEF_T * 3 * IEF_D; a.b2 = IEF_DH; a.c1 = (long long)IEF_T * IEF_D; a.c2 = IEF_DH; a.nz2 = IEF_H; a.alpha = 1.f;
            if (int rc = launch_bgemm(a, true, false, B * IEF_H, stream)) return rc;
        }

        memset(&p, 0, sizeof(p));
        p.N = IEF_D; p.ldc = IEF_D; p.epi = EPI_BIAS_RESID; p.nz = 2;
        for (int m = 0; m < 2; ++m) {
            p.set_w(m, h->out[m][l]);
            p.A32[m] = ws + t.att[m][l]; p.C[m] = ws + t.s[m][l]; p.R[m] = xin(m, l);
        }
        if (int rc = launch_proj(p, c.compute, splitmb, IEF_D, rows, stream, tm, ST_OUT)) return rc;

        LnArgs la;
        memset(&la, 0, sizeof(la));
        la.nrows = rows; la.eps = 1e-5f;
        for (int m = 0; m < 2; ++m) {
            la.x[m] = ws + t.s[m][l]; la.g1[m] = h->norm_w[m][l]; la.b1[m] = h->norm_b[m][l]; la.y[m] = ws + t.x[m][l + 1];
        }
        hipLaunchKernelGGL(iefvad_layernorm_kernel<IEF_D>, dim3((rows + ROW_WAVES - 1) / ROW_WAVES, 2), dim3(256), 0, stream, la);
        HIP_TRY(hipGetLastError());
    }
    {
        LnArgs la;
        memset(&la, 0, sizeof(la));
        la.nrows = rows; la.eps = 1e-5f;
        for (int m = 0; m < 2; ++m) {
            la.x[m] = ws + t.x[m][L]; la.g1[m] = h->whiten_w[m]; la.b1[m] = h->whiten_b[m]; la.y[m] = ws + t.E[m];
        }
        hipLaunchKernelGGL(iefvad_layernorm_kernel<IEF_D>, dim3((rows + ROW_WAVES - 1) / ROW_WAVES, 2), dim3(256), 0, stream, la);
        HIP_TRY(hipGetLastError());
    }
    {
        Proj p;
        memset(&p, 0, sizeof(p));
        p.N = 2 * IEF_D; p.ldc = IEF_D; p.epi = EPI_HEADS; p.nz = 2;
        for (int m = 0; m < 2; ++m) {
            p.set_w(m, h->head[m]);
            p.A32[m] = ws + t.E[m]; p.C[m] = rec->mu[m]; p.C2[m] = rec->lv[m];
        }
        if (int rc = launch_proj(p, c.compute, splitmb, IEF_D, rows, stream, tm, ST_HEAD)) return rc;
    }
    {
        FusionArgs fa;
        memset(&fa, 0, sizeof(fa));
        fa.mu_i = rec->mu[0]; fa.lv_i = rec->lv[0]; fa.mu_e = rec->mu[1]; fa.lv_e = rec->lv[1];
        fa.n_i = out->w_i; fa.n_e = out->w_e; fa.z = zst(0);
        fa.n_i_mean = out->w_i_mean; fa.n_e_mean = out->w_e_mean;
        fa.nrows = rows; fa.factor = factor; fa.eps = c.epsilon;
        hipLaunchKernelGGL(iefvad_fusion_kernel<IEF_D>, dim3((rows + ROW_WAVES - 1) / ROW_WAVES), dim3(256), 0, stream, fa);
        HIP_TRY(hipGetLastError());
    }
    for (int k = 0; k < K; ++k) {
        Proj p;
        memset(&p, 0, sizeof(p));
        p.N = IEF_D; p.ldc = IEF_D; p.epi = EPI_BIAS_RELU; p.nz = 1;
        p.set_w(0, h->ref1[k]);
        p.A32[0] = zst(k); p.C[0] = ws + t.hid[k];
        if (int rc = launch_proj(p, c.compute, splitmb, IEF_D, rows, stream, tm, ST_REFINE)) return rc;
        memset(&p, 0, sizeof(p));
        p.N = IEF_D; p.ldc = IEF_D; p.epi = EPI_REFINE; p.alpha = c.lambda_ref; p.nz = 1;
        p.set_w(0, h->ref2[k]);
        p.A32[0] = ws + t.hid[k]; p.C[0] = zst(k + 1); p.R[0] = zst(k);
        if (int rc = launch_proj(p, c.compute, splitmb, IEF_D, rows, stream, tm, ST_REFINE)) return rc;
    }
    float* logits = out->logits ? out->logits : ws + t.logits;
    hipLaunchKernelGGL(iefvad_scorer_kernel<IEF_D>, dim3((rows + ROW_WAVES - 1) / ROW_WAVES), dim3(256), 0, stream, rec->zK, h->cls_w, h->cls_b,
                       logits, rows);
    HIP_TRY(hipGetLastError());
    return 0;
}

extern "C" int iefvad_train_backward(iefvad_handle* h, int32_t B, void* train_ws, size_t train_ws_bytes, const iefvad_output_grads* dout,
                                     const iefvad_weight_grads* dw, void* stream_) {
    if (!h) return fail("iefvad_train_backward: null handle");
    if (h->D != IEF_D) return fail("iefvad_train_backward: training is built for D=768 (this handle has D=%d)", h->D);
    if (!dout || !dw) return fail("iefvad_train_backward: null argument");
    const TrainRecord* rec = nullptr;
    if (h->train)
        for (int i = 0; i < 8; ++i)
            if (h->train->rec[i].ws == train_ws && h->train->rec[i].stamp) rec = &h->train->rec[i];
    if (!rec || rec->B != B) return fail("iefvad_train_backward: no iefvad_train_forward with B = %d has filled this training buffer", B);
    if (int rc = train_check(h, B, train_ws, train_ws_bytes, "iefvad_train_backward")) return rc;
    const iefvad_config& c = h->cfg;
    const int L = c.num_layers, K = c.num_steps;
    hipStream_t stream = (hipStream_t)stream_;
    const TrainLayout t = train_layout(L, K, B);
    float* ws = (float*)train_ws;
    const int rows = B * IEF_T;
    const int nblk = (rows + BWD_ROWS_PER_BLOCK - 1) / BWD_ROWS_PER_BLOCK;
    const float factor = (c.noise_model == IEFVAD_NOISE_STUDENT_T) ? (c.nu + 1.0f) / c.nu : 1.0f;
    const float qscale = 1.0f / sqrtf((float)IEF_DH);
    float* part = ws + t.part;
    float* cpart = ws + t.cpart;
    float* rpart = ws + t.rpart;
    float* g = ws + t.g;
    float* da = ws + t.da;
    if (int rc = ensure_train_planes(h, stream)) return rc;
    const bool tp = h->cfg.compute == IEFVAD_COMPUTE_BF16X6 && h->tplanes_valid;
    const bool tn = h->cfg.compute == IEFVAD_COMPUTE_BF16X6;

    {
        ScorerBwdArgs sa;
        sa.dlogit = dout->logits; sa.dfused = dout->fused; sa.z = rec->zK; sa.w = h->cls_w; sa.g = g;
        sa.part_w = rpart; sa.part_b = rpart + (size_t)nblk * IEF_D; sa.rows = rows;
        hipLaunchKernelGGL(iefvad_scorer_bwd_kernel, dim3(nblk), dim3(256), 0, stream, sa);
        ReduceBatch rb;
        rb.add(rpart, (size_t)IEF_D, nblk, (size_t)IEF_D, dw->cls_w, 1.f);
        rb.add(rpart + (size_t)nblk * IEF_D, (size_t)1, nblk, (size_t)1, dw->cls_b, 1.f);
        rb.launch(stream);
        HIP_TRY(hipGetLastError());
    }
    for (int k = K - 1; k >= 0; --k) {
        const float nl = -c.lambda_ref;
        { bool db_done = false;
            if (int rc = launch_dw(g, IEF_D, IEF_D, ws + t.hid[k], dw->ref_w2[k], nullptr, 0, nl, rows, part, t.part_floats, stream, tn, dw->ref_b2[k], nullptr, cpart, t.cpart_floats, &db_done)) return rc;
            if (!db_done)
                if (int rc = launch_db(g, IEF_D, IEF_D, dw->ref_b2[k], nullptr, 0, nl, rows, cpart, stream)) return rc; }
        if (int rc = launch_dx(h, tp ? h->ref2[k].wst : nullptr, g, IEF_D, h->ref2[k].w, IEF_D, IEF_D, da, nullptr, ws + t.hid[k], nl, rows, stream)) return rc;
        { bool db_done = false;
            if (int rc = launch_dw(da, IEF_D, IEF_D, k == K ? rec->zK : ws + t.z[k], dw->ref_w1[k], nullptr, 0, 1.f, rows, part, t.part_floats, stream, tn, dw->ref_b1[k], nullptr, cpart, t.cpart_floats, &db_done)) return rc;
            if (!db_done)
                if (int rc = launch_db(da, IEF_D, IEF_D, dw->ref_b1[k], nullptr, 0, 1.f, rows, cpart, stream)) return rc; }
        if (int rc = launch_dx(h, tp ? h->ref1[k].wst : nullptr, da, IEF_D, h->ref1[k].w, IEF_D, IEF_D, g, g, nullptr, 1.f, rows, stream)) return rc;
    }
    {
        FusionBwdArgs fa;
        memset(&fa, 0, sizeof(fa));
        fa.mu_i = rec->mu[0]; fa.lv_i = rec->lv[0]; fa.mu_e = rec->mu[1]; fa.lv_e = rec->lv[1];
        fa.gz = g;
        fa.d_mu_i = dout->image_mu; fa.d_lv_i = dout->image_logvar; fa.d_mu_e = dout->event_mu; fa.d_lv_e = dout->event_logvar;
        fa.d_n_i = dout->w_i; fa.d_n_e = dout->w_e;
        fa.dh_i = ws + t.dh[0]; fa.dh_e = ws + t.dh[1];
        fa.rows = rows; fa.factor = factor; fa.eps = c.epsilon;
        hipLaunchKernelGGL(iefvad_fusion_bwd_kernel, dim3((rows + ROW_WAVES - 1) / ROW_WAVES), dim3(256), 0, stream, fa);
        HIP_TRY(hipGetLastError());
    }
    for (int m = 0; m < 2; ++m) {
        const float* dhm = ws + t.dh[m];
        float* gx = ws + t.gx;
        { bool db_done = false;
            if (int rc = launch_dw(dhm, 2 * IEF_D, 2 * IEF_D, ws + t.E[m], dw->mu_w[m], dw->logvar_w[m], IEF_D, 1.f, rows, part, t.part_floats, stream, tn, dw->mu_b[m], dw->logvar_b[m], cpart, t.cpart_floats, &db_done)) return rc;
            if (!db_done)
                if (int rc = launch_db(dhm, 2 * IEF_D, 2 * IEF_D, dw->mu_b[m], dw->logvar_b[m], IEF_D, 1.f, rows, cpart, stream)) return rc; }
        if (int rc = launch_dx(h, tp ? h->head[m].wst : nullptr, dhm, 2 * IEF_D, h->head[m].w, 2 * IEF_D, IEF_D, gx, nullptr, nullptr, 1.f, rows, stream)) return rc;
        auto ln_bwd = [&](const float* x, const float* gamma, float* dgamma, float* dbeta) -> int {
            LnBwdArgs la;
            la.x = x; la.dy = gx; la.g = gamma; la.dx = gx; la.part_g = rpart; la.part_b = rpart + (size_t)nblk * IEF_D; la.rows = rows; la.eps = 1e-5f;
            hipLaunchKernelGGL(iefvad_layernorm_bwd_kernel, dim3(nblk), dim3(256), 0, stream, la);
            ReduceBatch rb;
            rb.add(rpart, (size_t)IEF_D, nblk, (size_t)IEF_D, dgamma, 1.f);
            rb.add(rpart + (size_t)nblk * IEF_D, (size_t)IEF_D, nblk, (size_t)IEF_D, dbeta, 1.f);
            rb.launch(stream);
            HIP_TRY(hipGetLastError());
            return 0;
        };
        if (int rc = ln_bwd(ws + t.x[m][L], h->whiten_w[m], dw->whiten_w[m], dw->whiten_b[m])) return rc;
        for (int l = L - 1; l >= 0; --l) {
            if (int rc = ln_bwd(ws + t.s[m][l], h->norm_w[m][l], dw->norm_w[m][l], dw->norm_b[m][l])) return rc;
            float* datt = ws + t.datt;
            float* dqkv = ws + t.dqkv;
            float* dP = ws + t.dP;
            const float* qkv = ws + t.qkv[m][l];
            const float* P = ws + t.P[m][l];
            const bool signed_p = rec->drop[m][l];
            const float drop_scale = signed_p ? (float)(1.0 / (1.0 - (double)rec->drop_p[m][l])) : 1.0f;
            { bool db_done = false;
            if (int rc = launch_dw(gx, IEF_D, IEF_D, ws + t.att[m][l], dw->out_proj_w[m][l], nullptr, 0, 1.f, rows, part, t.part_floats, stream, tn, dw->out_proj_b[m][l], nullptr, cpart, t.cpart_floats, &db_done)) return rc;
            if (!db_done)
                if (int rc = launch_db(gx, IEF_D, IEF_D, dw->out_proj_b[m][l], nullptr, 0, 1.f, rows, cpart, stream)) return rc; }
            if (int rc = launch_dx(h, tp ? h->out[m][l].wst : nullptr, gx, IEF_D, h->out[m][l].w, IEF_D, IEF_D, datt, nullptr, nullptr, 1.f, rows, stream)) return rc;
            const long long sQ = (long long)IEF_T * 3 * IEF_D, sP1 = (long long)IEF_H * IEF_T * IEF_T, sP2 = (long long)IEF_T * IEF_T,
                            sA = (long long)IEF_T * IEF_D;
            BgemmArgs a;
            const bool ds_fused = rec->fused;
            if (ds_fused) {
                AttnArgs aa;
                AttnTrainArgs tx;
                memset(&aa, 0, sizeof(aa));
                memset(&tx, 0, sizeof(tx));
                aa.nchunks = B;
                aa.qkv[0] = qkv;
                tx.dO[0] = datt; tx.P[0] = const_cast<float*>(P); tx.drop[0] = signed_p ? 1 : 0; tx.drop_p[0] = rec->drop_p[m][l]; tx.dS[0] = dP;
                tx.dQ[0] = dqkv; tx.q_scale = qscale;
                hipLaunchKernelGGL(iefvad_attention_split_ds_kernel, dim3(IEF_H, 2, B), dim3(256), ATS_LDS_BYTES, stream, aa, tx);
                HIP_TRY(hipGetLastError());
            } else {
            memset(&a, 0, sizeof(a));
            a.A = datt; a.B = qkv + 2 * IEF_D; a.C = dP;
            a.M = IEF_T; a.N = IEF_T; a.K = IEF_DH; a.lda = IEF_D; a.ldb = 3 * IEF_D; a.ldc = IEF_T;
            a.a1 = sA; a.a2 = IEF_DH; a.b1 = sQ; a.b2 = IEF_DH; a.c1 = sP1; a.c2 = sP2; a.nz2 = IEF_H; a.alpha = 1.f;
            if (int rc = launch_bgemm(a, true, true, B * IEF_H, stream)) return rc;
            }
            memset(&a, 0, sizeof(a));
            a.A = P; a.B = datt; a.C = dqkv + 2 * IEF_D;
            a.M = IEF_T; a.N = IEF_DH; a.K = IEF_T; a.lda = IEF_T; a.ldb = IEF_D; a.ldc = 3 * IEF_D;
            a.a1 = sP1; a.a2 = sP2; a.b1 = sA; a.b2 = IEF_DH; a.c1 = sQ; a.c2 = IEF_DH; a.nz2 = IEF_H; a.alpha = 1.f;
            if (signed_p) a.a_drop = drop_scale;
            if (int rc = launch_bgemm(a, false, false, B * IEF_H, stream)) return rc;
            if (!ds_fused) {
                const long long srows = (long long)B * IEF_H * IEF_T;
                hipLaunchKernelGGL(iefvad_softmax_bwd_kernel, dim3((unsigned)((srows + 3) / 4)), dim3(256), 0, stream, P, drop_scale, dP, srows);
                HIP_TRY(hipGetLastError());
            }
            if (!ds_fused) {
            memset(&a, 0, sizeof(a));
            a.A = dP; a.B = qkv + IEF_D; a.C = dqkv;
            a.M = IEF_T; a.N = IEF_DH; a.K = IEF_T; a.lda = IEF_T; a.ldb = 3 * IEF_D; a.ldc = 3 * IEF_D;
            a.a1 = sP1; a.a2 = sP2; a.b1 = sQ; a.b2 = IEF_DH; a.c1 = sQ; a.c2 = IEF_DH; a.nz2 = IEF_H; a.alpha = qscale;
            if (int rc = launch_bgemm(a, true, false, B * IEF_H, stream)) return rc;
            }
            memset(&a, 0, sizeof(a));
            a.A = dP; a.B = qkv; a.C = dqkv + IEF_D;
            a.M = IEF_T; a.N = IEF_DH; a.K = IEF_T; a.lda = IEF_T; a.ldb = 3 * IEF_D; a.ldc = 3 * IEF_D;
            a.a1 = sP1; a.a2 = sP2; a.b1 = sQ; a.b2 = IEF_DH; a.c1 = sQ; a.c2 = IEF_DH; a.nz2 = IEF_H; a.alpha = 1.f;
            if (int rc = launch_bgemm(a, false, false, B * IEF_H, stream)) return rc;
            { bool db_done = false;
// ... 11 lines not shown
```

### ief-vad_amd/lib.py

```python
from __future__ import annotations

import ctypes as C
import os
import subprocess

_HERE = os.path.dirname(os.path.abspath(__file__))
LIB_PATH = os.environ.get("IEFVAD_LIB") or os.path.join(_HERE, "libiefvad.so")
CSRC_DIR = os.path.join(_HERE, "csrc")

ABI_VERSION = 8
MAX_LAYERS = 8
MAX_STEPS = 64
NOISE_GAUSSIAN, NOISE_STUDENT_T = 0, 1
IN_F32, IN_F16, IN_BF16 = 0, 1, 2
COMPUTE_F32, COMPUTE_BF16, COMPUTE_BF16X6, COMPUTE_FP16X3 = 0, 1, 2, 3
COMPUTE_CODES = {"f32": COMPUTE_F32, "bf16": COMPUTE_BF16, "bf16x6": COMPUTE_BF16X6, "fp16x3": COMPUTE_FP16X3}

SYMBOLS = ["iefvad_abi_version", "iefvad_create", "iefvad_create_ex", "iefvad_set_weights", "iefvad_workspace_bytes",
           "iefvad_forward", "iefvad_forward_timed", "iefvad_gemm_bias", "iefvad_split_bf16x3", "iefvad_split_bf16x3_many", "iefvad_last_error",
           "iefvad_destroy", "iefvad_comm_unique_id", "iefvad_comm_create", "iefvad_comm_nranks", "iefvad_comm_destroy",
           "iefvad_gather_scores", "iefvad_gather_plan", "iefvad_rccl_version", "iefvad_forward_videos",
           "iefvad_videos_workspace_bytes", "iefvad_host_gather", "iefvad_loss_forward", "iefvad_loss_backward", "iefvad_adamw_step",
           "iefvad_loss_workspace_bytes", "iefvad_train_workspace_bytes", "iefvad_train_forward", "iefvad_train_backward", "iefvad_nan_rule",
           "iefvad_forward_videos_host", "iefvad_host_gather_bf16", "iefvad_auc_ap", "iefvad_auc_ap_workspace_bytes", "iefvad_forward_scaled", "iefvad_rowblock_unit",
           "iefvad_similarity_adj", "iefvad_similarity_adj_workspace_bytes", "iefvad_distance_adj", "iefvad_gcn_forward",
           "iefvad_gcn_workspace_bytes", "iefvad_gat_forward", "iefvad_gat_workspace_bytes", "iefvad_resblock_forward",
           "iefvad_resblock_workspace_bytes", "iefvad_adamw_step_multi", "iefvad_resample_workspace_bytes", "iefvad_resample_videos",
           "iefvad_gather_windows", "iefvad_auc_ap_grouped", "iefvad_auc_ap_grouped_workspace_bytes", "iefvad_similarity_rows"]
COMM_ID_BYTES = 128

_fp = C.c_void_p


class Config(C.Structure):
    _fields_ = [("abi_version", C.c_int32), ("embed_dim", C.c_int32), ("seq_len", C.c_int32),
                ("num_heads", C.c_int32), ("num_layers", C.c_int32), ("num_steps", C.c_int32),
                ("noise_model", C.c_int32), ("compute", C.c_int32), ("lambda_ref", C.c_float),
                ("nu", C.c_float), ("epsilon", C.c_float), ("micro_batch", C.c_int32), ("graph_chunks", C.c_int32)]


class Weights(C.Structure):
    _fields_ = [("in_proj_w", (_fp * MAX_LAYERS) * 2), ("in_proj_b", (_fp * MAX_LAYERS) * 2),
                ("out_proj_w", (_fp * MAX_LAYERS) * 2), ("out_proj_b", (_fp * MAX_LAYERS) * 2),
                ("norm_w", (_fp * MAX_LAYERS) * 2), ("norm_b", (_fp * MAX_LAYERS) * 2),
                ("whiten_w", _fp * 2), ("whiten_b", _fp * 2),
                ("mu_w", _fp * 2), ("mu_b", _fp * 2), ("logvar_w", _fp * 2), ("logvar_b", _fp * 2),
                ("ref_w1", _fp * MAX_STEPS), ("ref_b1", _fp * MAX_STEPS),
                ("ref_w2", _fp * MAX_STEPS), ("ref_b2", _fp * MAX_STEPS),
                ("cls_w", _fp), ("cls_b", _fp)]


class WeightGrads(C.Structure):
    _fields_ = Weights._fields_


class TrainOptions(C.Structure):
    _fields_ = [("dropout_p", (C.c_float * MAX_LAYERS) * 2), ("seed", C.c_uint64), ("keep_mask", _fp)]


class OutputGrads(C.Structure):
    _fields_ = [("fused", _fp), ("logits", _fp), ("image_mu", _fp), ("event_mu", _fp),
                ("image_logvar", _fp), ("event_logvar", _fp), ("w_i", _fp), ("w_e", _fp)]


class Outputs(C.Structure):
    _fields_ = [("fused", _fp), ("logits", _fp), ("image_mu", _fp), ("event_mu", _fp),
                ("image_logvar", _fp), ("event_logvar", _fp), ("w_i", _fp), ("w_e", _fp),
                ("w_i_mean", _fp), ("w_e_mean", _fp)]


class StageTimes(C.Structure):
    _fields_ = [("total_ms", C.c_float), ("qkv_gemm_ms", C.c_float), ("attention_ms", C.c_float),
                ("out_gemm_ms", C.c_float), ("layernorm_ms", C.c_float), ("head_gemm_ms", C.c_float),
                ("fusion_ms", C.c_float), ("refine_gemm_ms", C.c_float), ("scorer_ms", C.c_float),
                ("cast_ms", C.c_float), ("gemm_launches", C.c_int32)]

    def as_dict(self):
        return {n: getattr(self, n) for n, _ in self._fields_}


_lib = None


def build_library(force: bool = False) -> str:
    cmd = ["make", "-C", CSRC_DIR] + (["-B"] if force else [])
    r = subprocess.run(cmd, capture_output=True, text=True)
    if r.returncode != 0:
        raise RuntimeError("building libiefvad.so failed:\n" + r.stdout + r.stderr)
    return LIB_PATH


class UnitIO(C.Structure):
    _fields_ = [("x", C.c_void_p * 2), ("resid", C.c_void_p * 2), ("y", C.c_void_p * 2), ("yb", C.c_void_p * 2), ("mu", C.c_void_p * 2),
                ("logvar", C.c_void_p * 2), ("w", C.c_void_p * 2), ("z", C.c_void_p), ("logits", C.c_void_p)]


UNIT_INPROJ, UNIT_OUTPROJ_LN, UNIT_HEADS, UNIT_REFINE, UNIT_ATTENTION = 0, 1, 2, 3, 4


class ResblockWeights(C.Structure):
    _fields_ = [(n, C.c_void_p) for n in ("in_proj_w", "in_proj_b", "out_proj_w", "out_proj_b", "ln_1_w", "ln_1_b", "ln_2_w", "ln_2_b", "c_fc_w",
                                          "c_fc_b", "c_proj_w", "c_proj_b")]


def load_library() -> C.CDLL:
    global _lib
    if _lib is not None:
        return _lib
    if not os.path.exists(LIB_PATH):
        raise RuntimeError(f"{LIB_PATH} not found: build it with `python -c 'import __graft_entry__ as g; g.build()'` "
                           f"(hipcc --offload-arch=gfx950); there is no CPU fallback for this path")
    lib = C.CDLL(LIB_PATH)
    for s in SYMBOLS:
        if not hasattr(lib, s):
            raise RuntimeError(f"libiefvad.so does not export {s}")
    lib.iefvad_abi_version.restype = C.c_int
    lib.iefvad_create.argtypes = [C.POINTER(Config), C.POINTER(C.c_void_p)]
    lib.iefvad_create.restype = C.c_int
    lib.iefvad_create_ex.argtypes = [C.POINTER(Config), C.POINTER(C.c_void_p)]
    lib.iefvad_create_ex.restype = C.c_int
    lib.iefvad_set_weights.argtypes = [C.c_void_p, C.POINTER(Weights), C.c_void_p]
    lib.iefvad_set_weights.restype = C.c_int
    lib.iefvad_workspace_bytes.argtypes = [C.c_void_p, C.c_int32]
    lib.iefvad_workspace_bytes.restype = C.c_size_t
    lib.iefvad_forward.argtypes = [C.c_void_p, C.c_void_p, C.c_void_p, C.c_int32, C.c_int32, C.c_void_p,
                                   C.c_size_t, C.POINTER(Outputs), C.c_void_p]
    lib.iefvad_forward.restype = C.c_int
    lib.iefvad_forward_scaled.argtypes = [C.c_void_p, C.c_void_p, C.c_void_p, C.c_int32, C.c_int32, C.c_void_p, C.c_void_p, C.c_void_p,
                                          C.c_size_t, C.POINTER(Outputs), C.c_void_p]
    lib.iefvad_forward_scaled.restype = C.c_int
    lib.iefvad_forward_timed.argtypes = lib.iefvad_forward.argtypes + [C.POINTER(StageTimes)]
    lib.iefvad_forward_timed.restype = C.c_int
    lib.iefvad_videos_workspace_bytes.argtypes = [C.c_void_p, C.POINTER(C.c_int32), C.c_int32]
    lib.iefvad_videos_workspace_bytes.restype = C.c_size_t
    lib.iefvad_forward_videos.argtypes = [C.c_void_p, C.c_void_p, C.c_void_p, C.c_int32, C.POINTER(C.c_int32), C.c_int32,
                                          C.c_int32, C.c_void_p, C.c_size_t, C.c_void_p, C.c_void_p, C.c_void_p, C.c_void_p]
    lib.iefvad_forward_videos.restype = C.c_int
    lib.iefvad_forward_videos_host.argtypes = [C.c_void_p, C.POINTER(C.c_void_p), C.POINTER(C.c_void_p), C.c_int32, C.c_int32, C.POINTER(C.c_int32),
                                               C.c_int32, C.c_int32, C.c_int32, C.c_int32, C.c_void_p, C.c_void_p, C.c_void_p, C.c_void_p]
    lib.iefvad_forward_videos_host.restype = C.c_int
    lib.iefvad_loss_workspace_bytes.argtypes = [C.c_int32, C.c_int32]
    lib.iefvad_loss_workspace_bytes.restype = C.c_size_t
    lib.iefvad_loss_forward.argtypes = [C.c_void_p] * 7 + [C.c_int32, C.c_int32, C.c_int32, C.c_float, C.c_float, C.c_float,
                                                          C.c_void_p, C.c_void_p, C.c_size_t, C.c_void_p]
    lib.iefvad_loss_forward.restype = C.c_int
    lib.iefvad_loss_backward.argtypes = [C.c_void_p] * 7 + [C.c_int32, C.c_int32, C.c_int32, C.c_float, C.c_float, C.c_float, C.c_float] + [C.c_void_p] * 7
    lib.iefvad_loss_backward.restype = C.c_int
    lib.iefvad_train_workspace_bytes.argtypes = [C.c_void_p, C.c_int32]
    lib.iefvad_train_workspace_bytes.restype = C.c_size_t
    lib.iefvad_train_forward.argtypes = [C.c_void_p, C.c_void_p, C.c_void_p, C.c_int32, C.c_int32, C.POINTER(TrainOptions), C.c_void_p,
                                         C.c_size_t, C.POINTER(Outputs), C.c_void_p]
    lib.iefvad_train_forward.restype = C.c_int
    lib.iefvad_train_backward.argtypes = [C.c_void_p, C.c_int32, C.c_void_p, C.c_size_t, C.POINTER(OutputGrads), C.POINTER(WeightGrads),
                                          C.c_void_p]
    lib.iefvad_train_backward.restype = C.c_int
    lib.iefvad_adamw_step.argtypes = [C.c_void_p] * 4 + [C.c_size_t] + [C.c_double] * 5 + [C.c_int32, C.c_void_p]
    lib.iefvad_adamw_step.restype = C.c_int
    lib.iefvad_adamw_step_multi.argtypes = [C.c_void_p, C.c_int32, C.c_uint64] + [C.c_double] * 5 + [C.c_int32, C.c_void_p]
    lib.iefvad_adamw_step_multi.restype = C.c_int
    lib.iefvad_host_gather.argtypes = [C.c_void_p, C.POINTER(C.c_void_p), C.POINTER(C.c_size_t), C.c_int64, C.c_int32]
    lib.iefvad_host_gather.restype = C.c_int
    lib.iefvad_host_gather_bf16.argtypes = [C.c_void_p, C.POINTER(C.c_void_p), C.POINTER(C.c_size_t), C.c_int64, C.c_int32]
    lib.iefvad_host_gather_bf16.restype = C.c_int
    lib.iefvad_auc_ap_workspace_bytes.argtypes = [C.c_int64]
    lib.iefvad_auc_ap_workspace_bytes.restype = C.c_size_t
    lib.iefvad_auc_ap.argtypes = [C.c_void_p, C.c_void_p, C.c_int64, C.c_int32, C.c_void_p, C.c_void_p, C.c_void_p, C.c_size_t, C.c_void_p]
    lib.iefvad_auc_ap.restype = C.c_int
    lib.iefvad_auc_ap_grouped_workspace_bytes.argtypes = [C.c_int64, C.c_int32]
    lib.iefvad_auc_ap_grouped_workspace_bytes.restype = C.c_size_t
    lib.iefvad_auc_ap_grouped.argtypes = [C.c_void_p, C.c_void_p, C.c_void_p, C.c_int64, C.c_int32, C.c_int32, C.c_void_p, C.c_void_p, C.c_void_p,
                                          C.c_void_p, C.c_size_t, C.c_void_p]
    lib.iefvad_auc_ap_grouped.restype = C.c_int
    lib.iefvad_rowblock_unit.argtypes = [C.c_void_p, C.c_int32, C.c_int32, C.c_int32, C.POINTER(UnitIO), C.c_void_p]
    lib.iefvad_rowblock_unit.restype = C.c_int
    i32, vp = C.c_int32, C.c_void_p
    lib.iefvad_similarity_adj_workspace_bytes.argtypes = [i32, i32, i32]
    lib.iefvad_similarity_adj_workspace_bytes.restype = C.c_size_t
    lib.iefvad_similarity_adj.argtypes = [vp, vp, vp, i32, i32, i32, i32, vp, vp, C.c_size_t, vp]
    lib.iefvad_similarity_adj.restype = C.c_int
    lib.iefvad_distance_adj.argtypes = [i32, i32, vp, vp]
    lib.iefvad_distance_adj.restype = C.c_int
    lib.iefvad_gcn_workspace_bytes.argtypes = [i32, i32, i32, i32, i32]
    lib.iefvad_gcn_workspace_bytes.restype = C.c_size_t
    lib.iefvad_gcn_forward.argtypes = [vp, vp, vp, vp, vp, vp, i32, i32, i32, i32, i32, i32, vp, vp, C.c_size_t, vp]
    lib.iefvad_gcn_forward.restype = C.c_int
    lib.iefvad_gat_workspace_bytes.argtypes = [i32, i32]
    lib.iefvad_gat_workspace_bytes.restype = C.c_size_t
    lib.iefvad_gat_forward.argtypes = [vp, vp, vp, vp, C.c_float, i32, i32, i32, i32, vp, vp, C.c_size_t, vp]
    lib.iefvad_gat_forward.restype = C.c_int
    lib.iefvad_resblock_workspace_bytes.argtypes = [i32, i32, i32]
    lib.iefvad_resblock_workspace_bytes.restype = C.c_size_t
    lib.iefvad_resblock_forward.argtypes = [vp, C.POINTER(ResblockWeights), vp, vp, i32, i32, i32, i32, vp, vp, C.c_size_t, vp]
    lib.iefvad_resblock_forward.restype = C.c_int
    lib.iefvad_resample_workspace_bytes.argtypes = [i32]
    lib.iefvad_resample_workspace_bytes.restype = C.c_size_t
    lib.iefvad_resample_videos.argtypes = [vp, i32, C.POINTER(C.c_int32), i32, i32, i32, vp, C.c_size_t, vp, vp, vp]
    lib.iefvad_resample_videos.restype = C.c_int
    lib.iefvad_gather_windows.argtypes = [vp, vp, vp, i32, vp, i32, i32, i32, vp, vp, vp, vp]
    lib.iefvad_gather_windows.restype = C.c_int
    lib.iefvad_similarity_rows.argtypes = [vp, vp, vp, C.c_int64, i32, vp, C.c_int64, vp, vp]
    lib.iefvad_similarity_rows.restype = C.c_int
    lib.iefvad_gemm_bias.argtypes = [C.c_void_p, C.c_void_p, C.c_void_p, C.c_void_p, C.c_int32, C.c_int32,
                                     C.c_int32, C.c_int32, C.c_void_p]
    lib.iefvad_gemm_bias.restype = C.c_int
    lib.iefvad_split_bf16x3.argtypes = [C.c_void_p, C.c_void_p, C.c_size_t, C.c_void_p]
    lib.iefvad_split_bf16x3.restype = C.c_int
    lib.iefvad_split_bf16x3_many.argtypes = [C.c_void_p, C.c_void_p, C.c_void_p, C.c_void_p, C.c_int32, C.c_void_p]
    lib.iefvad_split_bf16x3_many.restype = C.c_int
    lib.iefvad_nan_rule.argtypes = [C.c_void_p, C.c_void_p, C.c_size_t, C.c_void_p, C.c_void_p]
    lib.iefvad_nan_rule.restype = C.c_int
    lib.iefvad_comm_unique_id.argtypes = [C.c_void_p]
    lib.iefvad_comm_unique_id.restype = C.c_int
    lib.iefvad_comm_create.argtypes = [C.c_void_p, C.c_int32, C.c_int32, C.POINTER(C.c_void_p)]
    lib.iefvad_comm_create.restype = C.c_int
    lib.iefvad_comm_nranks.argtypes = [C.c_void_p]
    lib.iefvad_comm_nranks.restype = C.c_int32
    lib.iefvad_comm_destroy.argtypes = [C.c_void_p]
    lib.iefvad_comm_destroy.restype = None
    lib.iefvad_gather_scores.argtypes = [C.c_void_p, C.c_void_p, C.c_size_t, C.POINTER(C.c_int64), C.c_void_p, C.c_size_t,
                                         C.c_void_p]
    lib.iefvad_gather_scores.restype = C.c_int
    lib.iefvad_gather_plan.argtypes = [C.c_int32, C.c_int32, C.POINTER(C.c_int64), C.c_int64, C.POINTER(C.c_int64),
                                       C.POINTER(C.c_int64)]
    lib.iefvad_gather_plan.restype = C.c_int
    lib.iefvad_rccl_version.argtypes = []
    lib.iefvad_rccl_version.restype = C.c_int32
    lib.iefvad_last_error.restype = C.c_char_p
    lib.iefvad_destroy.argtypes = [C.c_void_p]
    lib.iefvad_destroy.restype = None
    if lib.iefvad_abi_version() != ABI_VERSION:
        raise RuntimeError(f"libiefvad.so ABI {lib.iefvad_abi_version()} != binding {ABI_VERSION}")
    _lib = lib
    return lib


def last_error() -> str:
    return load_library().iefvad_last_error().decode("utf-8", "replace")
```

### include/iefvad.h

```cpp
#ifndef IEFVAD_H
#define IEFVAD_H

#include <stddef.h>
#include <stdint.h>

#ifdef __cplusplus
extern "C" {
#endif

#define IEFVAD_ABI_VERSION 8
#define IEFVAD_MAX_LAYERS 8
#define IEFVAD_MAX_STEPS 64

enum { IEFVAD_NOISE_GAUSSIAN = 0, IEFVAD_NOISE_STUDENT_T = 1 };
enum { IEFVAD_IN_F32 = 0, IEFVAD_IN_F16 = 1, IEFVAD_IN_BF16 = 2 };
enum { IEFVAD_COMPUTE_F32 = 0, IEFVAD_COMPUTE_BF16 = 1, IEFVAD_COMPUTE_BF16X6 = 2, IEFVAD_COMPUTE_FP16X3 = 3 };

typedef struct iefvad_handle iefvad_handle;

typedef struct iefvad_config {
    int32_t abi_version;
    int32_t embed_dim;
    int32_t seq_len;
    int32_t num_heads;
// ... 70 lines not shown
                   void* workspace, size_t workspace_bytes, const iefvad_outputs* out, void* stream);

int iefvad_forward_timed(iefvad_handle* h, const void* img, const void* ev, int32_t in_dtype, int32_t B,
                         void* workspace, size_t workspace_bytes, const iefvad_outputs* out, void* stream,
                         iefvad_stage_times* times);

size_t iefvad_videos_workspace_bytes(const iefvad_handle* h, const int32_t* lengths, int32_t nvideos);
int iefvad_forward_videos(iefvad_handle* h, const void* img_rows, const void* ev_rows, int32_t in_dtype,
                          const int32_t* lengths, int32_t nvideos, int32_t nan_to_num, void* workspace,
                          size_t workspace_bytes, float* logits, float* w_i_mean, float* w_e_mean, void* stream);

int iefvad_forward_videos_host(iefvad_handle* h, const void* const* img_rows, const void* const* ev_rows, int32_t in_dtype,
                               int32_t wire_dtype, const int32_t* lengths, int32_t nvideos, int32_t nan_to_num, int32_t batch_chunks,
                               int32_t host_threads, float* logits, float* w_i_mean, float* w_e_mean, void* stream);

size_t iefvad_loss_workspace_bytes(int32_t B, int32_t T);
int iefvad_loss_forward(const float* logits, const float* image_mu, const float* event_mu, const float* image_logvar,
                        const float* event_logvar, const int32_t* lengths, const float* targets, int32_t B, int32_t T,
                        int32_t noise_model, float nu, float lambda_reg, float lambda_kl, float* out, void* workspace,
                        size_t workspace_bytes, void* stream);
int iefvad_loss_backward(const float* logits, const float* image_mu, const float* event_mu, const float* image_logvar,
                         const float* event_logvar, const int32_t* lengths, const float* targets, int32_t B, int32_t T,
                         int32_t noise_model, float nu, float lambda_reg, float lambda_kl, float grad_scale,
                         float* d_logits, float* d_image_mu, float* d_event_mu, float* d_image_logvar,
                         float* d_event_logvar, const float* grad_scale_dev, void* stream);

typedef struct iefvad_train_options {
    float dropout_p[2][IEFVAD_MAX_LAYERS];
    uint64_t seed;
    const uint8_t* keep_mask;
} iefvad_train_options;

typedef struct iefvad_output_grads {
    const float* fused;  const float* logits;  const float* image_mu;  const float* event_mu;
    const float* image_logvar;  const float* event_logvar;  const float* w_i;  const float* w_e;
} iefvad_output_grads;

typedef struct iefvad_weight_grads {
    float* in_proj_w[2][IEFVAD_MAX_LAYERS];
    float* in_proj_b[2][IEFVAD_MAX_LAYERS];
    float* out_proj_w[2][IEFVAD_MAX_LAYERS];
    float* out_proj_b[2][IEFVAD_MAX_LAYERS];
    float* norm_w[2][IEFVAD_MAX_LAYERS];
    float* norm_b[2][IEFVAD_MAX_LAYERS];
    float* whiten_w[2];
    float* whiten_b[2];
    float* mu_w[2];
    float* mu_b[2];
    float* logvar_w[2];
    float* logvar_b[2];
    float* ref_w1[IEFVAD_MAX_STEPS];
    float* ref_b1[IEFVAD_MAX_STEPS];
    float* ref_w2[IEFVAD_MAX_STEPS];
    float* ref_b2[IEFVAD_MAX_STEPS];
    float* cls_w;
    float* cls_b;
} iefvad_weight_grads;

size_t iefvad_train_workspace_bytes(const iefvad_handle* h, int32_t B);
int iefvad_train_forward(iefvad_handle* h, const void* img, const void* ev, int32_t in_dtype, int32_t B,
                         const iefvad_train_options* opt, void* train_ws, size_t train_ws_bytes, const iefvad_outputs* out,
                         void* stream);
int iefvad_train_backward(iefvad_handle* h, int32_t B, void* train_ws, size_t train_ws_bytes, const iefvad_output_grads* dout,
                          const iefvad_weight_grads* dw, void* stream);

int iefvad_nan_rule(float* a, float* b, size_t n, void* flags_ws, void* stream);

int iefvad_adamw_step(float* param, const float* grad, float* exp_avg, float* exp_avg_sq, size_t n, double lr, double beta1,
                      double beta2, double eps, double weight_decay, int32_t step, void* stream);

typedef struct iefvad_adamw_tensor {
    float* param;
    const float* grad;
    float* exp_avg;
    float* exp_avg_sq;
    uint64_t n;
    uint64_t first_chunk;
} iefvad_adamw_tensor;
int iefvad_adamw_step_multi(const iefvad_adamw_tensor* table, int32_t count, uint64_t total_chunks, double lr, double beta1, double beta2,
                            double eps, double weight_decay, int32_t step, void* stream);

int iefvad_host_gather(void* dst, const void* const* srcs, const size_t* nbytes, int64_t count, int32_t threads);
int iefvad_host_gather_bf16(void* dst, const void* const* srcs, const size_t* nbytes, int64_t count, int32_t threads);

int iefvad_forward_scaled(iefvad_handle* h, const void* img, const void* ev, int32_t in_dtype, int32_t B, const float* img_row_scale,
                          const float* ev_row_scale, void* workspace, size_t workspace_bytes, const iefvad_outputs* out, void* stream);

size_t iefvad_auc_ap_workspace_bytes(int64_t n);
int iefvad_auc_ap(const float* scores, const uint8_t* gt_frames, int64_t n, int32_t repeat, double* auc, double* ap,
                  void* workspace, size_t workspace_bytes, void* stream);

size_t iefvad_auc_ap_grouped_workspace_bytes(int64_t n, int32_t ngroups);
int iefvad_auc_ap_grouped(const float* scores, const uint8_t* gt_frames, const uint8_t* group, int64_t n, int32_t repeat, int32_t ngroups,
                          double* auc, double* ap, int64_t* frames, void* workspace, size_t workspace_bytes, void* stream);

int iefvad_similarity_rows(const float* fused, const float* image_mu, const float* event_mu, int64_t rows, int32_t D, const int32_t* src_rows,
                           int64_t nout, float* out, void* stream);

size_t iefvad_resample_workspace_bytes(int32_t nvideos);
int iefvad_resample_videos(const void* rows, int32_t in_dtype, const int32_t* lengths, int32_t nvideos, int32_t T, int32_t D,
                           void* workspace, size_t workspace_bytes, float* out, int32_t* out_lengths, void* stream);

int iefvad_gather_windows(const float* img_set, const float* ev_set, const int32_t* set_lengths, int32_t nset, const int32_t* index,
                          int32_t B, int32_t T, int32_t D, float* img_out, float* ev_out, int32_t* len_out, void* stream);

typedef struct iefvad_resblock_weights {
    const float* in_proj_w;
    const float* in_proj_b;
    const float* out_proj_w;
    const float* out_proj_b;
    const float* ln_1_w; const float* ln_1_b;
    const float* ln_2_w; const float* ln_2_b;
    const float* c_fc_w;
    const float* c_fc_b;
    const float* c_proj_w;
    const float* c_proj_b;
} iefvad_resblock_weights;
size_t iefvad_similarity_adj_workspace_bytes(int32_t B, int32_t T, int32_t d_out);
int iefvad_similarity_adj(const float* x, const float* weight0, const int32_t* seq_len, int32_t B, int32_t T, int32_t d_in, int32_t d_out,
                          float* adj, void* workspace, size_t workspace_bytes, void* stream);
int iefvad_distance_adj(int32_t B, int32_t T, float* adj, void* stream);
size_t iefvad_gcn_workspace_bytes(int32_t B, int32_t T, int32_t d_in, int32_t d_out, int32_t residual);
int iefvad_gcn_forward(const float* x, const float* adj, const float* weight, const float* bias, const float* conv_w, const float* conv_b,
                       int32_t residual, int32_t act, int32_t B, int32_t T, int32_t d_in, int32_t d_out, float* out, void* workspace,
                       size_t workspace_bytes, void* stream);
size_t iefvad_gat_workspace_bytes(int32_t N, int32_t f_out);
int iefvad_gat_forward(const float* input, const float* adj, const float* W, const float* a, float alpha, int32_t concat, int32_t N, int32_t f_in,
                       int32_t f_out, float* out, void* workspace, size_t workspace_bytes, void* stream);
size_t iefvad_resblock_workspace_bytes(int32_t T, int32_t B, int32_t n_head);
int iefvad_resblock_forward(const float* x, const iefvad_resblock_weights* w, const float* attn_mask, const uint8_t* key_padding_mask, int32_t T,
                            int32_t B, int32_t d_model, int32_t n_head, float* out, void* workspace, size_t workspace_bytes, void* stream);

#define IEFVAD_UNIT_INPROJ 0
#define IEFVAD_UNIT_OUTPROJ_LN 1
#define IEFVAD_UNIT_HEADS 2
#define IEFVAD_UNIT_REFINE 3
#define IEFVAD_UNIT_ATTENTION 4
typedef struct iefvad_unit_io {
    const void* x[2];
    const float* resid[2];
    void* y[2];
    void* yb[2];
    float* mu[2];
    float* logvar[2];
    float* w[2];
    float* z;
    float* logits;
} iefvad_unit_io;
int iefvad_rowblock_unit(iefvad_handle* h, int32_t stage, int32_t layer, int32_t rows, const iefvad_unit_io* io, void* stream);

int iefvad_gemm_bias(const void* A, const void* W, const float* bias, float* C,
                     int32_t M, int32_t N, int32_t K, int32_t compute, void* stream);

int iefvad_split_bf16x3(const float* src, void* planes, size_t n, void* stream);

int iefvad_split_bf16x3_many(const float* const* src, void* const* planes, const size_t* n, const int32_t* rows, int32_t count,
                             void* stream);

#define IEFVAD_COMM_ID_BYTES 128
typedef struct iefvad_comm iefvad_comm;

int iefvad_comm_unique_id(void* id_bytes );
int iefvad_comm_create(const void* id_bytes, int32_t nranks, int32_t rank, iefvad_comm** out);
int32_t iefvad_comm_nranks(const iefvad_comm* c);
void iefvad_comm_destroy(iefvad_comm* c);

int32_t iefvad_rccl_version(void);

int iefvad_gather_scores(iefvad_comm* c, const float* local, size_t count, const int64_t* counts, float* gathered,
                         size_t gathered_capacity, void* stream);

int iefvad_gather_plan(int32_t nranks, int32_t rank, const int64_t* counts, int64_t count, int64_t* summary, int64_t* steps);

const char* iefvad_last_error(void);
void iefvad_destroy(iefvad_handle* h);

#ifdef __cplusplus
}
#endif
#endif
```

Baseline: 4.211 million.

## Add wide 128x2 split-bf16 GEMM kernel reusing A splits across two N halves

Adds a split-precision GEMM kernel whose workgroup covers two 128-column halves of N. Each fp32 A tile is split into three bf16 planes once and reused for both halves, with the split work and W DMA spread across the two half-tile passes. The kernel is selectable per handle through IEFVAD_SPLIT_TILE and a new unit-test entry point. This halves the redundant A splitting and A loads per output column, at the cost of more accumulator registers and fewer workgroups.

```diff
diff --git a/ief-vad_amd/csrc/gemm_split_wide.h b/ief-vad_amd/csrc/gemm_split_wide.h
--- /dev/null
+++ b/ief-vad_amd/csrc/gemm_split_wide.h
@@ -0,0 +1,283 @@
+#pragma once
+#include <type_traits>
+#include "gemm_split.h"
+
+#ifndef GS_WIDE_SPREAD
+#define GS_WIDE_SPREAD 1
+#endif
+#undef GS_DIAG_STAMP
+
+__device__ __forceinline__ void gemm_split_wide_body(const GemmBArgs& args, float* smem) {
+    constexpr int NA = 2, NH = 2;
+    constexpr bool F16 = false;
+    constexpr int NP = F16 ? 2 : 3;
+    constexpr int NT = F16 ? 3 : 6;
+    constexpr int BN = GS_BN_OF(NA);
+    constexpr int BNB = BN * NH;
+    constexpr int W_PLANE = BN * 16;
+    constexpr int W_SLOT = NP * W_PLANE;
+    constexpr int W_BASE = 2 * GS_A_SLOT;
+    constexpr int WROWS = BN / 4;
+    constexpr int NM = NT * NA;
+#ifdef GB2_CLOCK_DIAG
+    const unsigned long long dg_entry = __builtin_amdgcn_s_memtime();
+#endif
+    const GemmBProblem& P = args.p[blockIdx.z];
+    const int ntn = args.N / BNB;
+    const int bid = xcd_remap(blockIdx.x, gridDim.x);
+    int tm, tn;
+    {
+        constexpr int PN = GS_PN / NH;
+        const int pn = (PN > 0 && ntn % PN == 0) ? PN : ntn;
+        const int ntm = args.M / GS_BM;
+        const int grp = bid / (ntm * pn), rem = bid - grp * (ntm * pn);
+        tm = rem / pn;
+        tn = grp * pn + (rem - tm * pn);
+    }
+    const int m0 = tm * GS_BM, n0 = tn * BNB;
+#ifdef GS_EXPERIMENT_A_ALIAS
+    const int m0a = (tm % GS_EXPERIMENT_A_ALIAS) * GS_BM;
+#else
+    const int m0a = m0;
+#endif
+    const int K = args.K, lda = args.lda;
+    const int wplane = args.wplane;
+    float ascale = 1.0f, cscale = 1.0f;
+    if constexpr (F16) {
+        if (P.amaxA && P.amaxW) {
+            const int ea = 13 - amax_exponent(amax_read_chunk(P.amaxA, m0 / IEF_T)), ew = 13 - amax_exponent(amax_read(P.amaxW));
+            ascale = __builtin_ldexpf(1.0f, ea);
+            cscale = __builtin_ldexpf(1.0f, -ea - ew);
+        }
+    }
+
+    const int t = threadIdx.x;
+    const int lane = t & 63, wave = t >> 6;
+    const int wrow0 = NA == 4 ? (wave >> 1) * 64 : wave * 32;
+    const int wcol0 = NA == 4 ? (wave & 1) * 128 : 0;
+    const int r16 = lane & 15, q16 = lane >> 4;
+    const int uwave = __builtin_amdgcn_readfirstlane(wave);
+
+    const int nrecA = (int)((GS_BM - 1) * lda + K) * 4, nrecW = (NP - 1) * wplane + (int)((BNB - 1) * K + K) * 2;
+    const auto rsA = __builtin_amdgcn_make_buffer_rsrc((void*)((const char*)P.A + (size_t)m0a * lda * 4), 0, nrecA, 0x00020000);
+    const auto rsW = __builtin_amdgcn_make_buffer_rsrc((void*)((const char*)P.W + (size_t)n0 * K * 2), 0, nrecW, 0x00020000);
+    const int arow = lane >> 3, achk = lane & 7;
+    int voA[2];
+#pragma unroll
+    for (int jj = 0; jj < 2; ++jj) voA[jj] = arow * lda * 4 + ((achk ^ (((arow >> 1) & 1) | (jj << 2))) << 4);
+    const int wrow = lane >> 2, wchk = lane & 3;
+    const int voW = wrow * K * 2 + ((wchk ^ ((0xD2 >> (2 * ((wrow >> 2) & 3))) & 3)) << 4);
+#define GLDS16(rs, vo, so, lp) \
+    __builtin_amdgcn_raw_ptr_buffer_load_lds(rs, (__attribute__((address_space(3))) void*)(lp), 16, vo, so, 0, 0)
+    auto stage_a = [&](int tile, int slot) {
+        float* Ad = smem + slot * GS_A_SLOT + uwave * 32 * 32;
+#pragma unroll
+        for (int j = 0; j < 4; ++j) GLDS16(rsA, voA[j & 1], ((uwave * 32 + j * 8) * lda + tile * GS_BK) * 4, Ad + j * 8 * 32);
+    };
+    auto stage_w = [&](int tile, int slot) {
+        float* Wd = smem + W_BASE + slot * W_SLOT + uwave * WROWS * 16;
+#pragma unroll
+        for (int p = 0; p < NP; ++p)
+#pragma unroll
+            for (int j = 0; j < WROWS / 16; ++j)
+                GLDS16(rsW, voW, p * wplane + ((uwave * WROWS + j * 16) * K + tile * GS_BK) * 2, Wd + p * W_PLANE + j * 16 * 16);
+    };
+
+    const int swa = (r16 >> 1) & 5;
+    const int a_lo = (wrow0 + r16) * 32 + (((2 * q16) ^ swa) << 2);
+    const int a_hi = (wrow0 + r16) * 32 + (((2 * q16 + 1) ^ swa) << 2);
+    const int b_of = (wcol0 + r16) * 16 + ((q16 ^ ((0xD2 >> (2 * ((r16 >> 2) & 3))) & 3)) << 2);
+
+    f32x4 acc16[NH][NA][8];
+#pragma unroll
+    for (int hh = 0; hh < NH; ++hh)
+#pragma unroll
+        for (int a = 0; a < NA; ++a)
+#pragma unroll
+            for (int b = 0; b < 8; ++b) acc16[hh][a][b] = f32x4{0.f, 0.f, 0.f, 0.f};
+
+    u32x4 ap[NA][NP], an[NA][NP];
+    auto mfma_row = [&](int hh, int b, int pa, const u32x4& wv) {
+#pragma unroll
+        for (int a = 0; a < NA; ++a) {
+            if constexpr (F16)
+                acc16[hh][a][b] = __builtin_amdgcn_mfma_f32_16x16x32_f16(__builtin_bit_cast(f16x8, ap[a][pa]),
+                                                                         __builtin_bit_cast(f16x8, wv), acc16[hh][a][b], 0, 0, 0);
+            else
+                acc16[hh][a][b] = __builtin_amdgcn_mfma_f32_16x16x32_bf16(__builtin_bit_cast(bf16x8, ap[a][pa]),
+                                                                          __builtin_bit_cast(bf16x8, wv), acc16[hh][a][b], 0, 0, 0);
+        }
+    };
+    auto split_half = [&](int hf, const f32x4& v) {
+        Split4 sp;
+        if constexpr (F16) {
+#pragma unroll
+            for (int e = 0; e < 4; ++e) sp.r[e] = v[e] * ascale;
+        } else {
+            sp.r = v;
+        }
+#pragma unroll
+        for (int p = 0; p < NP; ++p) {
+            unsigned d0, d1;
+            if constexpr (F16) sp.plane_f16(d0, d1, p < NP - 1); else sp.plane(d0, d1, p < NP - 1);
+            an[hf >> 1][p][2 * (hf & 1)] = d0;
+            an[hf >> 1][p][2 * (hf & 1) + 1] = d1;
+        }
+    };
+#define GS_FENCE() __builtin_amdgcn_sched_barrier(0)
+#define GS_PIPE(mask) __builtin_amdgcn_sched_group_barrier(mask, 1, 0)
+
+    const int nk = K / GS_BK;
+    stage_a(0, 0);
+    stage_a(1, 1);
+    stage_w(0, 0);
+    asm volatile("s_waitcnt vmcnt(0)" ::: "memory");
+    GB2_BARRIER();
+#pragma unroll
+    for (int hf = 0; hf < 2 * NA; ++hf)
+        split_half(hf, *(const f32x4*)(smem + (hf >> 1) * 16 * 32 + ((hf & 1) ? a_hi : a_lo)));
+#pragma unroll
+    for (int a = 0; a < NA; ++a)
+#pragma unroll
+        for (int p = 0; p < NP; ++p) ap[a][p] = an[a][p];
+#ifdef GB2_CLOCK_DIAG
+    const unsigned long long dg_c0 = __builtin_amdgcn_s_memtime(), dg_r0 = __builtin_amdgcn_s_memrealtime();
+    unsigned long long dg_last = dg_c0, dg_acc[3] = {0, 0, 0};
+#define GS_DIAG_STAMP(i) { const unsigned long long now = __builtin_amdgcn_s_memtime(); dg_acc[i] += now - dg_last; dg_last = now; }
+#else
+#define GS_DIAG_STAMP(i)
+#endif
+
+    for (int kt = 0; kt < nk; ++kt) {
+      auto half_tile = [&](auto hh_c) __attribute__((always_inline)) {
+        constexpr int HH = decltype(hh_c)::value;
+        const int it = kt * NH + HH, it1 = it + 1;
+        const auto rW = __builtin_amdgcn_make_buffer_rsrc((void*)((const char*)P.W + (size_t)n0 * K * 2), 0,
+                                                          (it1 < nk * NH) ? nrecW : 0, 0x00020000);
+        const auto rA = __builtin_amdgcn_make_buffer_rsrc((void*)((const char*)P.A + (size_t)m0a * lda * 4), 0,
+                                                          (kt + 2 < nk) ? nrecA : 0, 0x00020000);
+        float* Wd = smem + W_BASE + (it1 & 1) * W_SLOT + uwave * WROWS * 16;
+        float* Ad = smem + (kt & 1) * GS_A_SLOT + uwave * 32 * 32;
+        const int kW = (it1 % NH) * BN * K * 2 + (it1 / NH) * GS_BK * 2, kA = (kt + 2) * GS_BK * 4;
+        auto dma = [&](int d) {
+            if (GS_EXP_NODMA) return;
+            if (d < 4) {
+                GLDS16(rA, voA[d & 1], (uwave * 32 + d * 8) * lda * 4 + kA, Ad + d * 8 * 32);
+            } else {
+                const int p = (d - 4) / (WROWS / 16), j = (d - 4) % (WROWS / 16);
+                GLDS16(rW, voW, p * wplane + (uwave * WROWS + j * 16) * K * 2 + kW, Wd + p * W_PLANE + j * 16 * 16);
+            }
+        };
+        const float* Wv = smem + W_BASE + (it & 1) * W_SLOT + b_of;
+        const float* Av = smem + ((kt + 1) & 1) * GS_A_SLOT;
+        auto a_half = [&](int hf) { return *(const f32x4*)(Av + (hf >> 1) * 16 * 32 + ((hf & 1) ? a_hi : a_lo)); };
+#define GS_NSPLIT(B) (NA == 4 ? ((B) < 6 ? 1 : (B) == 6 ? 2 : 0) : NH == 2 ? (GS_WIDE_SPREAD ? ((B) < 2 ? 1 : 0) : (HH == 0 && (B) < 4 ? 1 : 0)) \
+                                                                           : ((B) < 4 ? 1 : 0))
+#define GS_HF(B) (NH == 2 && GS_WIDE_SPREAD ? 2 * HH + (B) : (B))
+#define GS_NAREAD(B) ((B) < 7 ? GS_NSPLIT((B) + 1) : 0)
+#define GS_NREAD(B) (((B) < 7 ? NP : 0) + GS_NAREAD(B))
+#define GS_NDMA(B) (NA == 4 ? ((B) < 4 ? (F16 ? 3 : 4) : 0) : (F16 ? ((B) < 4 ? 2 : 0) : HH > 0 ? ((B) < 3 ? 2 : 0) : ((B) < 5 ? 2 : 0)))
+#define GS_DMA0 (HH > 0 ? 4 : 0)
+#define GS_NVALU(B) ((B) == 7 ? (HH == NH - 1 ? 4 * NP * NA : 0) : GS_EXP_NOSPLIT ? 0 : (F16 ? 12 : 22) * GS_NSPLIT(B))
+        u32x4 w[NP];
+        f32x4 v0 = {0.f, 0.f, 0.f, 0.f}, v1 = {0.f, 0.f, 0.f, 0.f};
+#pragma unroll
+        for (int p = 0; p < NP; ++p) w[p] = *(const u32x4*)(Wv + p * W_PLANE);
+        if (GS_NSPLIT(0) > 0) v0 = a_half(GS_HF(0));
+        GS_FENCE();
+#define GS_VSLOT(B, g) (((g) + 1) * GS_NVALU(B) / NM - (g) * GS_NVALU(B) / NM)
+#define GS_SLOT(B, g)                                                                                           \
+        if ((g) < NM) {                                                                                         \
+            GS_PIPE(0x008);                                                                                     \
+            if (GS_VSLOT(B, g) > 0) __builtin_amdgcn_sched_group_barrier(0x002, GS_VSLOT(B, g) > 0 ? GS_VSLOT(B, g) : 1, 0); \
+            if (GS_NDMA(B) > 0 && !GS_EXP_NODMA && (g) % (NM / 4) == 2 && (g) / (NM / 4) < GS_NDMA(B)) GS_PIPE(0x020); \
+        }
+#define GS_STEP(B)                                                                                              \
+        {                                                                                                       \
+            u32x4 wn[NP];                                                                                       \
+            f32x4 vn0 = {0.f, 0.f, 0.f, 0.f}, vn1 = {0.f, 0.f, 0.f, 0.f};                                       \
+            if ((B) < 7) {                                                                                      \
+                _Pragma("unroll") for (int p = 0; p < NP; ++p) wn[p] = *(const u32x4*)(Wv + p * W_PLANE + ((B) + 1) * 16 * 16); \
+                if (GS_NAREAD(B) == 1) vn0 = a_half(GS_HF((B) + 1));                                            \
+                if (GS_NAREAD(B) == 2) { vn0 = a_half((B) + 1); vn1 = a_half((B) + 2); }                        \
+            }                                                                                                   \
+            if constexpr (!F16) {                                                                               \
+                mfma_row(HH, B, NP - 1, w[0]);                                                       \
+                mfma_row(HH, B, 0, w[NP - 1]);                                                       \
+                mfma_row(HH, B, 1, w[1]);                                                            \
+            }                                                                                                   \
+            mfma_row(HH, B, 1, w[0]);                                                                \
+            mfma_row(HH, B, 0, w[1]);                                                                \
+            mfma_row(HH, B, 0, w[0]);                                                                \
+            if (!GS_EXP_NOSPLIT) {                                                                              \
+                if (GS_NSPLIT(B) >= 1) split_half(GS_HF(B), v0);                                                 \
+                if (GS_NSPLIT(B) == 2) split_half((B) + 1, v1);                                                 \
+            }                                                                                                   \
+            if ((B) == 7 && HH == NH - 1) {                                                                     \
+                _Pragma("unroll") for (int a = 0; a < NA; ++a)                                                  \
+                    _Pragma("unroll") for (int p = 0; p < NP; ++p) ap[a][p] = an[a][p];                         \
+            }                                                                                                   \
+            _Pragma("unroll") for (int d = 0; d < GS_NDMA(B); ++d) dma(GS_DMA0 + GS_NDMA(B) * (B) + d);         \
+            if (GS_NREAD(B) > 0) __builtin_amdgcn_sched_group_barrier(0x100, GS_NREAD(B) > 0 ? GS_NREAD(B) : 1, 0); \
+            GS_SLOT(B, 0) GS_SLOT(B, 1) GS_SLOT(B, 2) GS_SLOT(B, 3) GS_SLOT(B, 4) GS_SLOT(B, 5)                 \
+            GS_SLOT(B, 6) GS_SLOT(B, 7) GS_SLOT(B, 8) GS_SLOT(B, 9) GS_SLOT(B, 10) GS_SLOT(B, 11)               \
+            GS_SLOT(B, 12) GS_SLOT(B, 13) GS_SLOT(B, 14) GS_SLOT(B, 15) GS_SLOT(B, 16) GS_SLOT(B, 17)           \
+            GS_SLOT(B, 18) GS_SLOT(B, 19) GS_SLOT(B, 20) GS_SLOT(B, 21) GS_SLOT(B, 22) GS_SLOT(B, 23)           \
+            GS_FENCE();                                                                                         \
+            if ((B) < 7) {                                                                                      \
+                _Pragma("unroll") for (int p = 0; p < NP; ++p) w[p] = wn[p];                                    \
+                if (GS_NAREAD(B) >= 1) v0 = vn0;                                                                \
+                if (GS_NAREAD(B) == 2) v1 = vn1;                                                                \
+            }                                                                                                   \
+        }
+        GS_STEP(0) GS_STEP(1) GS_STEP(2) GS_STEP(3) GS_STEP(4) GS_STEP(5) GS_STEP(6) GS_STEP(7)
+#undef GS_STEP
+#undef GS_SLOT
+#undef GS_VSLOT
+#undef GS_NVALU
+#undef GS_NDMA
+#undef GS_DMA0
+#undef GS_HF
+#undef GS_NREAD
+#undef GS_NAREAD
+#undef GS_NSPLIT
+        GS_DIAG_STAMP(0)
+        asm volatile("s_waitcnt vmcnt(0)" ::: "memory");
+        asm volatile("s_waitcnt lgkmcnt(0)" ::: "memory");
+        GS_DIAG_STAMP(1)
+        if (!GS_EXP_NOBAR) GB2_BARRIER();
+        GS_DIAG_STAMP(2)
+      };
+      half_tile(std::integral_constant<int, 0>{});
+      if constexpr (NH == 2) half_tile(std::integral_constant<int, 1>{});
+    }
+#ifdef GB2_CLOCK_DIAG
+    if (threadIdx.x == 0 && P.C2) {
+        unsigned long long* dg = (unsigned long long*)P.C2 + 2 * (blockIdx.x + gridDim.x * blockIdx.z);
+        dg[0] = __builtin_amdgcn_s_memtime() - dg_c0;
+        dg[1] = __builtin_amdgcn_s_memrealtime() - dg_r0;
+        unsigned long long* dx = (unsigned long long*)P.C2 + 2 * gridDim.x * gridDim.z + 3 * (blockIdx.x + gridDim.x * blockIdx.z);
+        dx[0] = dg_acc[0]; dx[1] = dg_acc[1]; dx[2] = dg_acc[2];
+    }
+    const unsigned long long dg_loop_end = __builtin_amdgcn_s_memtime();
+#endif
+#undef GS_PIPE
+#undef GS_FENCE
+#undef GLDS16
+    f32x16 unused[NA / 2][4];
+#pragma unroll
+    for (int hh = 0; hh < NH; ++hh)
+        gemm_wave_epilogue<true, NA / 2, !F16>(args, P, smem, m0, n0, wrow0, wcol0 + hh * BN, unused, acc16[hh], cscale, F16 ? P.amaxC : nullptr);
+#ifdef GB2_CLOCK_DIAG
+    if (threadIdx.x == 0 && P.C2) {
+        unsigned long long* dy = (unsigned long long*)P.C2 + 5 * gridDim.x * gridDim.z + 2 * (blockIdx.x + gridDim.x * blockIdx.z);
+        dy[0] = dg_c0 - dg_entry;
+        dy[1] = __builtin_amdgcn_s_memtime() - dg_loop_end;
+    }
+#endif
+}
+
+__global__ __launch_bounds__(256, 2) void iefvad_gemm_split_n128x2_kernel(GemmBArgs args) {
+    extern __shared__ __attribute__((aligned(16))) float smem[];
+    gemm_split_wide_body(args, smem);
+}
diff --git a/ief-vad_amd/csrc/iefvad.hip b/ief-vad_amd/csrc/iefvad.hip
--- a/ief-vad_amd/csrc/iefvad.hip
+++ b/ief-vad_amd/csrc/iefvad.hip
@@ -8,6 +8,7 @@
 #include <string.h>
 
 #include <algorithm>
+#include <atomic>
 #include <exception>
 #include <new>
 #include <thread>
@@ -22,6 +23,7 @@
 #include "gemm_f32.h"
 #include "gemm_bf16.h"
 #include "gemm_split.h"
+#include "gemm_split_wide.h"
 #include "rowops.h"
 #include "refine_chain_bf16.h"
 #include "outproj_ln_chain_bf16.h"
@@ -80,6 +82,7 @@
     bool dense_encoder;
     bool persist;
     bool train_attn_unfused;
+    int split_tile;
     bool hostpipe_trace;
     bool no_chain;
     char* chain_stream;
@@ -196,6 +199,7 @@
     { const char* v = getenv("IEFVAD_DENSE_ENCODER"); h->dense_encoder = v && v[0] == '1'; }
     { const char* v = getenv("IEFVAD_TRAIN_ATTN"); h->train_attn_unfused = v && v[0] == 'u'; }
     { const char* v = getenv("IEFVAD_HOSTPIPE_TRACE"); h->hostpipe_trace = v && v[0] == '1'; }
+    { const char* v = getenv("IEFVAD_SPLIT_TILE"); const int t = v ? atoi(v) : 0; h->split_tile = (t == 128 || t == 256) ? t : 0; }
     hipError_t e = hipGetDevice(&h->device);
     if (e == hipSuccess)
         e = hipFuncSetAttribute((const void*)iefvad_gemm_bf16_kernel, hipFuncAttributeMaxDynamicSharedMemorySize,
@@ -241,6 +245,9 @@
                                 GB2_LDS_BYTES);
     if (e == hipSuccess)
         e = hipFuncSetAttribute((const void*)iefvad_gemm_split_n128_kernel, hipFuncAttributeMaxDynamicSharedMemorySize,
+                                GS_LDS_BYTES_OF(2));
+    if (e == hipSuccess)
+        e = hipFuncSetAttribute((const void*)iefvad_gemm_split_n128x2_kernel, hipFuncAttributeMaxDynamicSharedMemorySize,
                                 GS_LDS_BYTES_OF(2));
     if (e == hipSuccess)
         e = hipFuncSetAttribute((const void*)iefvad_attention_split_kernel, hipFuncAttributeMaxDynamicSharedMemorySize,
@@ -712,14 +719,24 @@
     return M % GS_BM == 0 && N % kSplitBN == 0 && K % 64 == 0 && K >= 64 && (M / GS_BM) * (N / kSplitBN) * nz >= kSplitMinWgs;
 }
 
-static int launch_gemm_split(const GemmBArgs& a, int nz, hipStream_t stream, Timer& tm, int stage, bool f16 = false) {
+static const int kSplitWideMinWgs = 1536;
+static std::atomic<unsigned long long> g_split_wide_launches{0};
+static int launch_gemm_split(const GemmBArgs& a, int nz, hipStream_t stream, Timer& tm, int stage, bool f16 = false, int tile_n = 0) {
     if (a.M % GS_BM || a.N % kSplitBN || a.K % 64 || a.K < 64)
         return fail("gemm(bf16x6): shape M=%d N=%d K=%d not a multiple of the %dx%dx64 tile", a.M, a.N, a.K, GS_BM, kSplitBN);
+    if (tile_n != 0 && tile_n != 128 && tile_n != 256) return fail("gemm(bf16x6): tile_n = %d (128, 256 or 0 for the launch rule)", tile_n);
+    if (tile_n == 256 && (f16 || a.N % 256))
+        return fail("gemm(bf16x6): the 128 x 256 tiling takes bf16x6 problems with N %% 256 == 0 (N = %d%s)", a.N, f16 ? ", fp16x3" : "");
+    const bool wide = !f16 && a.N % 256 == 0 && (tile_n == 256 || (tile_n == 0 && (a.M / GS_BM) * (a.N / 256) * nz >= kSplitWideMinWgs));
     if (a.epi == EPI_BIAS_RELU_DOT && (f16 || nz != 1 || !a.p[0].R || !a.p[0].C2))
         return fail("gemm(bf16x6): the dot-product epilogue takes one bf16x6 problem with its vector (R) and its partial sums (C2)");
-    dim3 grid((a.M / GS_BM) * (a.N / kSplitBN), 1, nz);
+    dim3 grid((a.M / GS_BM) * (a.N / (wide ? 256 : kSplitBN)), 1, nz);
     hipEvent_t e = tm.begin(stage);
-    if (f16) hipLaunchKernelGGL(iefvad_gemm_split_f16_n128_kernel, grid, dim3(256), GS_LDS_BYTES_OF(2), stream, a);
+    if (wide) {
+        hipLaunchKernelGGL(iefvad_gemm_split_n128x2_kernel, grid, dim3(256), GS_LDS_BYTES_OF(2), stream, a);
+        g_split_wide_launches.fetch_add(1, std::memory_order_relaxed);
+    }
+    else if (f16) hipLaunchKernelGGL(iefvad_gemm_split_f16_n128_kernel, grid, dim3(256), GS_LDS_BYTES_OF(2), stream, a);
     else hipLaunchKernelGGL(iefvad_gemm_split_n128_kernel, grid, dim3(256), GS_LDS_BYTES_OF(2), stream, a);
     tm.end(e);
     tm.gemm_launches += 1;
@@ -752,7 +769,7 @@
     }
 };
 
-static int launch_proj(const Proj& p, int compute, bool use_split, int D, int rows, hipStream_t stream, Timer& tm, int stage) {
+static int launch_proj(const Proj& p, int compute, bool use_split, int D, int rows, hipStream_t stream, Timer& tm, int stage, int split_tile = 0) {
     const bool bf16 = (compute == IEFVAD_COMPUTE_BF16);
     if (p.epi == EPI_BIAS_RELU_DOT && !(use_split && compute == IEFVAD_COMPUTE_BF16X6))
         return fail("gemm: the dot-product epilogue exists in the bf16x6 split kernel only");
@@ -771,7 +788,7 @@
                 g.p[m].amaxA = p.amaxA[m]; g.p[m].amaxW = p.amaxW[m]; g.p[m].amaxC = p.amaxC[m];
             }
         }
-        return launch_gemm_split(g, p.nz, stream, tm, stage, f16);
+        return launch_gemm_split(g, p.nz, stream, tm, stage, f16, (f16 || (split_tile == 256 && p.N % 256)) ? (f16 ? 0 : 128) : split_tile);
     }
     if (!bf16) {
         GemmArgs g;
@@ -1055,7 +1072,7 @@
             p.amaxC[m] = b.am_qkv(l, m);
             if (bf) p.Cb[m] = b.qkvb[m]; else p.C[m] = b.qkv[m];
         }
-        if (int rc = launch_proj(p, c.compute, b.splitmb, D, rows, stream, tm, ST_QKV)) return rc;
+        if (int rc = launch_proj(p, c.compute, b.splitmb, D, rows, stream, tm, ST_QKV, h->split_tile)) return rc;
     }
 
     hipEvent_t e = tm.begin(ST_ATT);
@@ -1089,7 +1106,7 @@
             p.A32[m] = b.att[m]; p.A16[m] = b.attb[m]; p.amaxA[m] = b.am_att(l, m);
             p.C[m] = b.ybuf[m]; p.R[m] = b.cur[m];
         }
-        if (int rc = launch_proj(p, c.compute, b.splitmb, D, rows, stream, tm, ST_OUT)) return rc;
+        if (int rc = launch_proj(p, c.compute, b.splitmb, D, rows, stream, tm, ST_OUT, h->split_tile)) return rc;
 
         LnArgs la;
         memset(&la, 0, sizeof(la));
@@ -1183,7 +1200,7 @@
             p.A32[m] = b.xt[m]; p.A16[m] = b.xtb[m]; p.amaxA[m] = b.am_x(L - 1, m);
         }
         p.C[0] = b.mu_i; p.C2[0] = b.lv_i; p.C[1] = b.mu_e; p.C2[1] = b.lv_e;
-        if (int rc = launch_proj(p, c.compute, b.tail_split, D, rows, stream, tm, ST_HEAD)) return rc;
+        if (int rc = launch_proj(p, c.compute, b.tail_split, D, rows, stream, tm, ST_HEAD, h->split_tile)) return rc;
 
         FusionArgs fa;
         memset(&fa, 0, sizeof(fa));
@@ -1217,7 +1234,7 @@
             p.epi = EPI_BIAS_RELU_DOT; p.R[0] = h->score_fold; p.C2[0] = fold_part;
             if (!out->fused) p.C[0] = nullptr;
         }
-        if (int rc = launch_proj(p, c.compute, b.tail_split, D, rows, stream, tm, ST_REFINE)) return rc;
+        if (int rc = launch_proj(p, c.compute, b.tail_split, D, rows, stream, tm, ST_REFINE, h->split_tile)) return rc;
         if (dot) {
             hipEvent_t e = tm.begin(ST_SCORER);
             hipLaunchKernelGGL((iefvad_scorer_fold_kernel<IEF_D, IEF_D / kSplitBN>), row_grid, dim3(256), 0, stream, z, h->cls_w, fold_part,
@@ -1231,7 +1248,7 @@
         p.set_w(0, h->ref2[k]);
         p.A32[0] = b.hbuf; p.A16[0] = b.hb; p.amaxA[0] = b.am_h(k); p.amaxC[0] = b.am_z(k + 1);
         p.C[0] = z; p.R[0] = z; p.Cb[0] = (bf && k + 1 < K) ? b.zb : nullptr;
-        if (int rc = launch_proj(p, c.compute, b.tail_split, D, rows, stream, tm, ST_REFINE)) return rc;
+        if (int rc = launch_proj(p, c.compute, b.tail_split, D, rows, stream, tm, ST_REFINE, h->split_tile)) return rc;
     }
 
     if (!chain && !fold) {
@@ -2178,8 +2195,48 @@
         g.p[0].A = (const bf16_t*)A; g.p[0].W = (const bf16_t*)W; g.p[0].bias = bias; g.p[0].C = C;
         hipError_t e = hipFuncSetAttribute((const void*)iefvad_gemm_split_n128_kernel, hipFuncAttributeMaxDynamicSharedMemorySize,
                                            GS_LDS_BYTES_OF(2));
+        if (e == hipSuccess)
+            e = hipFuncSetAttribute((const void*)iefvad_gemm_split_n128x2_kernel, hipFuncAttributeMaxDynamicSharedMemorySize, GS_LDS_BYTES_OF(2));
         if (e != hipSuccess) return fail("iefvad_gemm_bias: %s", hipGetErrorString(e));
         return launch_gemm_split(g, 1, (hipStream_t)stream, tm, ST_QKV);
     }
     return fail("iefvad_gemm_bias: unknown compute mode %d", compute);
 }
+
+extern "C" uint64_t iefvad_gemm_split_wide_launches(void) { return g_split_wide_launches.load(std::memory_order_relaxed); }
+
+extern "C" int iefvad_gemm_split_unit(const iefvad_gemm_split_io* io, int32_t M, int32_t N, int32_t K, int32_t ldc, int32_t epilogue,
+                                      int32_t qcols, float alpha, int32_t nz, int32_t tile_n, void* stream) {
+    static const int epi_of[] = {EPI_BIAS, EPI_QKV, EPI_BIAS_RELU, EPI_BIAS_RESID, EPI_REFINE, EPI_HEADS, EPI_BIAS_RELU_DOT};
+    if (!io) return fail("iefvad_gemm_split_unit: null argument");
+    auto aligned = [](const void* p) { return (((uintptr_t)p) & 15) == 0; };
+    if (epilogue < 0 || epilogue >= (int)(sizeof(epi_of) / sizeof(epi_of[0]))) return fail("iefvad_gemm_split_unit: unknown epilogue %d", epilogue);
+    if (nz < 1 || nz > 2) return fail("iefvad_gemm_split_unit: nz = %d (1 or 2)", nz);
+    if (tile_n != 128 && tile_n != 256) return fail("iefvad_gemm_split_unit: tile_n = %d (128 or 256)", tile_n);
+    if (M <= 0 || N <= 0 || K < 64 || M % GS_BM || N % tile_n || K % 64)
+        return fail("iefvad_gemm_split_unit: shape M=%d N=%d K=%d not a multiple of the %dx%dx64 tile", M, N, K, GS_BM, tile_n);
+    const int epi = epi_of[epilogue];
+    const bool heads = epi == EPI_HEADS, dot = epi == EPI_BIAS_RELU_DOT;
+    const bool resid = epi == EPI_BIAS_RESID || epi == EPI_REFINE;
+    if (heads ? (N != 2 * ldc || ldc % 128) : (ldc < N || ldc % 4)) return fail("iefvad_gemm_split_unit: ldc = %d does not fit N = %d", ldc, N);
+    if (epi == EPI_QKV && (qcols < 0 || qcols > N || qcols % 8)) return fail("iefvad_gemm_split_unit: qcols = %d", qcols);
+    GemmBArgs g;
+    memset(&g, 0, sizeof(g));
+    g.M = M; g.N = N; g.K = K; g.lda = K; g.ldc = ldc; g.epi = epi; g.alpha = alpha; g.qcols = qcols;
+    g.wplane = N * K * 2;
+    for (int m = 0; m < nz; ++m) {
+        if (!io->A[m] || !io->W[m] || !io->bias[m] || (!io->C[m] && !dot) || ((resid || dot) && !io->R[m]) || ((heads || dot) && !io->C2[m]))
+            return fail("iefvad_gemm_split_unit: problem %d lacks an operand of epilogue %d", m, epilogue);
+        if (!aligned(io->A[m]) || !aligned(io->W[m]) || !aligned(io->bias[m]) || !aligned(io->C[m]) || !aligned(io->R[m]) || !aligned(io->C2[m]))
+            return fail("iefvad_gemm_split_unit: operands must be 16-byte aligned");
+        g.p[m].A = (const bf16_t*)io->A[m]; g.p[m].W = (const bf16_t*)io->W[m]; g.p[m].bias = io->bias[m]; g.p[m].C = io->C[m];
+        g.p[m].R = (resid || dot) ? io->R[m] : nullptr;
+        g.p[m].C2 = (heads || dot) ? io->C2[m] : nullptr;
+    }
+    hipError_t e = hipFuncSetAttribute((const void*)iefvad_gemm_split_n128_kernel, hipFuncAttributeMaxDynamicSharedMemorySize, GS_LDS_BYTES_OF(2));
+    if (e == hipSuccess)
+        e = hipFuncSetAttribute((const void*)iefvad_gemm_split_n128x2_kernel, hipFuncAttributeMaxDynamicSharedMemorySize, GS_LDS_BYTES_OF(2));
+    if (e != hipSuccess) return fail("iefvad_gemm_split_unit: %s", hipGetErrorString(e));
+    Timer tm;
+    return launch_gemm_split(g, nz, (hipStream_t)stream, tm, ST_QKV, false, tile_n);
+}
diff --git a/ief-vad_amd/csrc/train.h b/ief-vad_amd/csrc/train.h
--- a/ief-vad_amd/csrc/train.h
+++ b/ief-vad_amd/csrc/train.h
@@ -141,7 +141,7 @@
         g.p[0].A = (const bf16_t*)dY;
         g.p[0].W = planes_t; g.p[0].bias = h->zero_bias; g.p[0].C = dX; g.p[0].R = G ? G : R;
         Timer tm;
-        return launch_gemm_split(g, 1, stream, tm, ST_REFINE);
+        return launch_gemm_split(g, 1, stream, tm, ST_REFINE, false, h->split_tile);
     }
     BgemmArgs a;
     memset(&a, 0, sizeof(a));
@@ -371,7 +371,7 @@
             p.set_w(m, h->in[m][l]);
             p.A32[m] = xin(m, l); p.C[m] = ws + t.qkv[m][l];
         }
-        if (int rc = launch_proj(p, c.compute, splitmb, IEF_D, rows, stream, tm, ST_QKV)) return rc;
+        if (int rc = launch_proj(p, c.compute, splitmb, IEF_D, rows, stream, tm, ST_QKV, h->split_tile)) return rc;
 
         if (fused) {
             AttnArgs aa;
@@ -431,7 +431,7 @@
             p.set_w(m, h->out[m][l]);
             p.A32[m] = ws + t.att[m][l]; p.C[m] = ws + t.s[m][l]; p.R[m] = xin(m, l);
         }
-        if (int rc = launch_proj(p, c.compute, splitmb, IEF_D, rows, stream, tm, ST_OUT)) return rc;
+        if (int rc = launch_proj(p, c.compute, splitmb, IEF_D, rows, stream, tm, ST_OUT, h->split_tile)) return rc;
 
         LnArgs la;
         memset(&la, 0, sizeof(la));
@@ -460,7 +460,7 @@
             p.set_w(m, h->head[m]);
             p.A32[m] = ws + t.E[m]; p.C[m] = rec->mu[m]; p.C2[m] = rec->lv[m];
         }
-        if (int rc = launch_proj(p, c.compute, splitmb, IEF_D, rows, stream, tm, ST_HEAD)) return rc;
+        if (int rc = launch_proj(p, c.compute, splitmb, IEF_D, rows, stream, tm, ST_HEAD, h->split_tile)) return rc;
     }
     {
         FusionArgs fa;
@@ -478,12 +478,12 @@
         p.N = IEF_D; p.ldc = IEF_D; p.epi = EPI_BIAS_RELU; p.nz = 1;
         p.set_w(0, h->ref1[k]);
         p.A32[0] = zst(k); p.C[0] = ws + t.hid[k];
-        if (int rc = launch_proj(p, c.compute, splitmb, IEF_D, rows, stream, tm, ST_REFINE)) return rc;
+        if (int rc = launch_proj(p, c.compute, splitmb, IEF_D, rows, stream, tm, ST_REFINE, h->split_tile)) return rc;
         memset(&p, 0, sizeof(p));
         p.N = IEF_D; p.ldc = IEF_D; p.epi = EPI_REFINE; p.alpha = c.lambda_ref; p.nz = 1;
         p.set_w(0, h->ref2[k]);
         p.A32[0] = ws + t.hid[k]; p.C[0] = zst(k + 1); p.R[0] = zst(k);
-        if (int rc = launch_proj(p, c.compute, splitmb, IEF_D, rows, stream, tm, ST_REFINE)) return rc;
+        if (int rc = launch_proj(p, c.compute, splitmb, IEF_D, rows, stream, tm, ST_REFINE, h->split_tile)) return rc;
     }
     float* logits = out->logits ? out->logits : ws + t.logits;
     hipLaunchKernelGGL(iefvad_scorer_kernel<IEF_D>, dim3((rows + ROW_WAVES - 1) / ROW_WAVES), dim3(256), 0, stream, rec->zK, h->cls_w, h->cls_b,
diff --git a/ief-vad_amd/lib.py b/ief-vad_amd/lib.py
--- a/ief-vad_amd/lib.py
+++ b/ief-vad_amd/lib.py
@@ -26,7 +26,7 @@
            "iefvad_similarity_adj", "iefvad_similarity_adj_workspace_bytes", "iefvad_distance_adj", "iefvad_gcn_forward",
            "iefvad_gcn_workspace_bytes", "iefvad_gat_forward", "iefvad_gat_workspace_bytes", "iefvad_resblock_forward",
            "iefvad_resblock_workspace_bytes", "iefvad_adamw_step_multi", "iefvad_resample_workspace_bytes", "iefvad_resample_videos",
-           "iefvad_gather_windows", "iefvad_auc_ap_grouped", "iefvad_auc_ap_grouped_workspace_bytes", "iefvad_similarity_rows"]
+           "iefvad_gather_windows", "iefvad_auc_ap_grouped", "iefvad_auc_ap_grouped_workspace_bytes", "iefvad_similarity_rows", "iefvad_gemm_split_unit", "iefvad_gemm_split_wide_launches"]
 COMM_ID_BYTES = 128
 
 _fp = C.c_void_p
@@ -96,6 +96,14 @@
 
 
 UNIT_INPROJ, UNIT_OUTPROJ_LN, UNIT_HEADS, UNIT_REFINE, UNIT_ATTENTION = 0, 1, 2, 3, 4
+
+
+class GemmSplitIO(C.Structure):
+    _fields_ = [(n, C.c_void_p * 2) for n in ("A", "W", "bias", "R", "C", "C2")]
+
+
+(SPLIT_EPI_BIAS, SPLIT_EPI_QKV, SPLIT_EPI_BIAS_RELU, SPLIT_EPI_BIAS_RESID, SPLIT_EPI_REFINE, SPLIT_EPI_HEADS,
+ SPLIT_EPI_BIAS_RELU_DOT) = range(7)
 
 
 class ResblockWeights(C.Structure):
@@ -203,6 +211,11 @@
     lib.iefvad_gemm_bias.argtypes = [C.c_void_p, C.c_void_p, C.c_void_p, C.c_void_p, C.c_int32, C.c_int32,
                                      C.c_int32, C.c_int32, C.c_void_p]
     lib.iefvad_gemm_bias.restype = C.c_int
+    lib.iefvad_gemm_split_unit.argtypes = [C.POINTER(GemmSplitIO), C.c_int32, C.c_int32, C.c_int32, C.c_int32, C.c_int32, C.c_int32,
+                                           C.c_float, C.c_int32, C.c_int32, C.c_void_p]
+    lib.iefvad_gemm_split_unit.restype = C.c_int
+    lib.iefvad_gemm_split_wide_launches.argtypes = []
+    lib.iefvad_gemm_split_wide_launches.restype = C.c_uint64
     lib.iefvad_split_bf16x3.argtypes = [C.c_void_p, C.c_void_p, C.c_size_t, C.c_void_p]
     lib.iefvad_split_bf16x3.restype = C.c_int
     lib.iefvad_split_bf16x3_many.argtypes = [C.c_void_p, C.c_void_p, C.c_void_p, C.c_void_p, C.c_int32, C.c_void_p]
diff --git a/include/iefvad.h b/include/iefvad.h
--- a/include/iefvad.h
+++ b/include/iefvad.h
@@ -246,6 +246,25 @@
 int iefvad_gemm_bias(const void* A, const void* W, const float* bias, float* C,
                      int32_t M, int32_t N, int32_t K, int32_t compute, void* stream);
 
+#define IEFVAD_SPLIT_EPI_BIAS 0
+#define IEFVAD_SPLIT_EPI_QKV 1
+#define IEFVAD_SPLIT_EPI_BIAS_RELU 2
+#define IEFVAD_SPLIT_EPI_BIAS_RESID 3
+#define IEFVAD_SPLIT_EPI_REFINE 4
+#define IEFVAD_SPLIT_EPI_HEADS 5
+#define IEFVAD_SPLIT_EPI_BIAS_RELU_DOT 6
+typedef struct iefvad_gemm_split_io {
+    const float* A[2];
+    const void* W[2];
+    const float* bias[2];
+    const float* R[2];
+    float* C[2];
+    float* C2[2];
+} iefvad_gemm_split_io;
+uint64_t iefvad_gemm_split_wide_launches(void);
+int iefvad_gemm_split_unit(const iefvad_gemm_split_io* io, int32_t M, int32_t N, int32_t K, int32_t ldc, int32_t epilogue,
+                           int32_t qcols, float alpha, int32_t nz, int32_t tile_n, void* stream);
+
 int iefvad_split_bf16x3(const float* src, void* planes, size_t n, void* stream);
 
 int iefvad_split_bf16x3_many(const float* const* src, void* const* planes, const size_t* n, const int32_t* rows, int32_t count,
```

Result: faster. 4.498 million, median of 6 (+6.8%).
